# jspenmar/slowtv_monodepth

Measured on AMD Instinct MI355X. Metric: training images/sec (640×192, 3-frame) at 1/2/4/8 MI355X; warp+SSIM HBM GB/s, higher is better.
Workload: dtype f32

## Files before the change

### slowtv_monodepth_amd/csrc/smd_api.hip

```cpp
#include <limits.h>
#include <stdarg.h>
#include <stdio.h>
#include <stdlib.h>
#include <string.h>
#include <algorithm>

#include "smd_kernels.h"
#include "smd_smooth_dev.h"

namespace {

thread_local char g_err[512] = "";

int fail(int code, const char* fmt, ...) {
  va_list ap;
  va_start(ap, fmt);
  vsnprintf(g_err, sizeof(g_err), fmt, ap);
  va_end(ap);
  return code;
}

int check_launch(hipError_t e, const char* what) {
  if (e != hipSuccess) return fail(SMD_E_LAUNCH, "%s: %s", what, hipGetErrorString(e));
  return SMD_OK;
// ... 494 lines not shown
  if (int rc = fill_scales(sc, disp, g_disp, hs, ws, scale_keys, S)) return rc;
  for (int s = 0; s < S; ++s) if (!disp[s] || !g_disp[s]) return fail(SMD_E_INVALID, "null pointer for scale %d", s);
  int direct = -1;
  if (const char* why = loss_path_unsupported(sc, n, h, w, flags, &direct)) return fail(SMD_E_UNSUPPORTED, "the fused loss path does not serve %s", why);
  const size_t need = smd_loss_path_workspace_bytes(hs, ws, S, b, n, h, w);
  if (!need || workspace_bytes < need) return fail(SMD_E_WORKSPACE, "workspace %zu < %zu bytes", workspace_bytes, need);
  const size_t base = align256(smd_image_recon_workspace_bytes(b, n, S, h, w));
  float* g_depth = (float*)((char*)workspace + base);
  float* k0_tmp = (float*)((char*)workspace + base + align256((size_t)S*b*h*w*sizeof(float)));
  float a_scale = 1.f;
  if (min_depth > 0.f || max_depth > 0.f) a_scale = 1.f/min_depth - (max_depth > 0.f ? 1.f/max_depth : 0.f);
  const bool guests = knob("loss_path_guests", 1) != 0;
  smd::PoseFinJob job;
  memset(&job, 0, sizeof(job));
  job.chain.aa = aa; job.chain.t = t; job.chain.invert = invert; job.chain.g_aa = g_aa; job.chain.g_t = g_t;
  job.chain.fs = fs; job.chain.cs = cs; job.chain.g_fs = g_fs; job.chain.g_cs = g_cs; job.chain.h = h; job.chain.w = w;
  job.sm.stats = stats; job.sm.edge_w = edge_weights; job.sm.g_loss = g_loss; job.sm.g_scale = w_smooth; job.sm.accumulate_scale = direct;
  job.sm.blocks_per_sample = guests ? smd::smooth_bwd_blocks_per_sample(sc) : 0;
  const int rflags = flags & (SMD_USE_MIN | SMD_USE_AUTOMASK | SMD_NEED_K_GRAD | SMD_BWD_SKIP_DEAD_ROWS | SMD_BWD_NO_LIVE);
  if (int rc = recon_bwd_impl(depth_up, supp_packed, T, K, K_inv, sel, g_loss, nullptr, a_scale, g_depth, g_T, g_K, g_Kinv, workspace, base,
                              b, n, S, h, w, rflags, stream, &job, direct >= 0 ? g_disp[direct] : nullptr, direct, w_recon)) return rc;
  if (!guests) {
    if (int rc = check_launch(smd::launch_smooth_bwd(sc, b, nullptr, h, w, SMD_USE_EDGES, stats, g_loss, edge_weights, (hipStream_t)stream, w_smooth, direct), "loss_path smoothness adjoint")) return rc;
  }
  return check_launch(smd::launch_disp_to_depth_bwd(sc, b, h, w, min_depth, max_depth, depth_up, g_depth, k0_tmp, true, (hipStream_t)stream, &job, direct, true), "loss_path K0 adjoint");
}

static int smooth_chunks(const int* hs, const int* ws, int S) {
  int mx = 1;
  for (int s = 0; s < S; ++s) {
    const int u = smd::smooth_units_of(hs[s], ws[s]), p = smd::ceil_div(hs[s]*ws[s], 256);
    mx = (u > p ? u : p) > mx ? (u > p ? u : p) : mx;
  }
  return mx;
}

size_t smd_disp_smooth_workspace_bytes(const int* hs, const int* ws, int S, int b) {
  if (!hs || !ws || S < 1 || S > SMD_MAX_SCALES || b < 1) return 0;
  return align256((size_t)S*b*smooth_chunks(hs, ws, S)*2*sizeof(float) + (size_t)S*b*sizeof(double));
}

size_t smd_disp_smooth_edge_weight_bytes(const int* hs, const int* ws, int S, int b) {
  smd::ScaleSet sc;
  if (b < 1 || fill_scales(sc, nullptr, nullptr, hs, ws, nullptr, S)) return 0;
  return smd::smooth_edge_bytes(sc, b);
}

int smd_gaussian_blur3x3(const float* x, float* out, int planes, int h, int w, int adjoint, void* stream) {
  if (!x || !out) return fail(SMD_E_INVALID, "null pointer");
  if (x == out) return fail(SMD_E_INVALID, "in-place blur is not supported");
  if (planes < 1) return fail(SMD_E_INVALID, "invalid sizes");
  if (h < 2 || w < 2) return fail(SMD_E_INVALID, "reflect padding by one needs at least 2 x 2 pixels (got %d x %d)", h, w);
  return check_launch(smd::launch_blur3(x, out, planes, h, w, adjoint != 0, (hipStream_t)stream), "gaussian_blur3x3");
}

int smd_disp_smooth_prep(const float* img, const int* hs, const int* ws, int S, int b, int h, int w, int flags, float* edge_weights, void* stream) {
  if (!img || !edge_weights) return fail(SMD_E_INVALID, "null pointer");
  if (b < 1 || h < 1 || w < 1 || b > 65535) return fail(SMD_E_INVALID, "invalid sizes");
  if (!(flags & SMD_USE_EDGES) || (flags & SMD_USE_LAPLACIAN)) return fail(SMD_E_INVALID, "smd_disp_smooth_prep serves SmoothReg(use_edges=True) without use_laplacian");
  smd::ScaleSet sc;
  if (int rc = fill_scales(sc, nullptr, nullptr, hs, ws, nullptr, S)) return rc;
  return check_launch(smd::launch_smooth_edges(sc, b, img, h, w, edge_weights, (hipStream_t)stream), "disp_smooth_prep");
}

int smd_disp_smooth_fwd(const float* const* disp, const int* hs, const int* ws, const int* scale_keys, int S, int b,
                        const float* img, int h, int w, int flags, float* loss, float* stats, float* disp_grad, float* image_grad,
                        float* edge_weights, void* workspace, size_t workspace_bytes, void* stream) {
  if (!disp || !img || !loss || !stats || !workspace) return fail(SMD_E_INVALID, "null pointer");
  if (b < 1 || h < 1 || w < 1 || b > 65535) return fail(SMD_E_INVALID, "invalid sizes");
  smd::ScaleSet sc;
  if (int rc = fill_scales(sc, disp, nullptr, hs, ws, scale_keys, S)) return rc;
  for (int s = 0; s < S; ++s) if (!disp[s]) return fail(SMD_E_INVALID, "null disparity pointer for scale %d", s);
  const size_t need = smd_disp_smooth_workspace_bytes(hs, ws, S, b);
  if (workspace_bytes < need) return fail(SMD_E_WORKSPACE, "workspace %zu < %zu bytes", workspace_bytes, need);
  if ((flags & SMD_USE_EDGES) && !edge_weights) return fail(SMD_E_INVALID, "SMD_USE_EDGES needs the edge_weights buffer (smd_disp_smooth_edge_weight_bytes)");
  if ((flags & SMD_EDGES_READY) && (!(flags & SMD_USE_EDGES) || (flags & SMD_USE_LAPLACIAN))) return fail(SMD_E_INVALID, "SMD_EDGES_READY goes with SMD_USE_EDGES (first-order form)");
  return check_launch(smd::launch_smooth_fwd(sc, b, img, h, w, flags, loss, stats, disp_grad, image_grad, (float*)workspace,
                                             edge_weights, (flags & SMD_EDGES_READY) != 0, (hipStream_t)stream), "disp_smooth_fwd");
}

int smd_disp_smooth_bwd(const float* const* disp, const int* hs, const int* ws, const int* scale_keys, int S, int b,
                        const float* img, int h, int w, int flags, const float* stats, const float* edge_weights, const float* g_loss,
                        float* const* g_disp, void* stream) {
  if (!disp || !img || !stats || !g_loss || !g_disp) return fail(SMD_E_INVALID, "null pointer");
  if (b < 1 || h < 1 || w < 1 || b > 65535) return fail(SMD_E_INVALID, "invalid sizes");
  smd::ScaleSet sc;
  if (int rc = fill_scales(sc, disp, g_disp, hs, ws, scale_keys, S)) return rc;
  for (int s = 0; s < S; ++s) if (!disp[s] || !g_disp[s]) return fail(SMD_E_INVALID, "null pointer for scale %d", s);
  if ((flags & SMD_USE_LAPLACIAN) && (flags & SMD_USE_EDGES) && !edge_weights) return fail(SMD_E_INVALID, "the second-order adjoint needs the edge weights the forward cached");
  return check_launch(smd::launch_smooth_bwd(sc, b, img, h, w, flags, stats, g_loss, edge_weights, (hipStream_t)stream), "disp_smooth_bwd");
}

size_t smd_view_synth_workspace_bytes(int B, int h, int w) {
  if (B < 1 || h < 2 || w < 2) return 0;
  return align256((size_t)B*smd::ceil_div(h*w, 256)*smd::kPoseSums*sizeof(float));
}

int smd_view_synth_fwd(const float* input, const float* depth, const float* T, const float* K, const float* K_inv,
                       float* warp, float* depth_warp, uint8_t* mask_valid, int B, int C, int h, int w, void* stream) {
  if (!input || !depth || !T || !K || !K_inv || !warp) return fail(SMD_E_INVALID, "null pointer");
  if (B < 1 || B > 65535 || C < 1 || h < 2 || w < 2) return fail(SMD_E_INVALID, "invalid sizes B=%d C=%d h=%d w=%d", B, C, h, w);
  return check_launch(smd::launch_view_synth_fwd(input, depth, T, K, K_inv, warp, depth_warp, mask_valid, B, C, h, w, (hipStream_t)stream), "view_synth_fwd");
}

int smd_view_synth_bwd(const float* input, const float* depth, const float* T, const float* K, const float* K_inv,
                       const float* g_warp, const float* g_depth_warp, float* g_input, float* g_depth, float* g_T, float* g_K, float* g_Kinv,
                       void* workspace, size_t workspace_bytes, int B, int C, int h, int w, void* stream) {
  if (!input || !depth || !T || !K || !K_inv || !g_warp || !g_depth || !g_T || !workspace) return fail(SMD_E_INVALID, "null pointer");
  if (B < 1 || B > 65535 || C < 1 || h < 2 || w < 2) return fail(SMD_E_INVALID, "invalid sizes B=%d C=%d h=%d w=%d", B, C, h, w);
  if (workspace_bytes < smd_view_synth_workspace_bytes(B, h, w)) return fail(SMD_E_WORKSPACE, "workspace too small");
  return check_launch(smd::launch_view_synth_bwd(input, depth, T, K, K_inv, g_warp, g_depth_warp, g_input, g_depth, g_T, g_K, g_Kinv,
                                                 (float*)workspace, B, C, h, w, (hipStream_t)stream), "view_synth_bwd");
}

size_t smd_photo_error_workspace_bytes(int N, int C, int h, int w) {
  if (N < 1 || C < 1 || h < 2 || w < 2) return 0;
  return align256((size_t)N*3*C*h*w*sizeof(float));
}

int smd_photo_error_fwd(const float* pred, const float* target, float* err, int N, int C, int h, int w, int flags, float weight_ssim, void* stream) {
  if (!pred || !target || !err) return fail(SMD_E_INVALID, "null pointer");
  if (N < 1 || N > 65535 || C < 1 || h < 2 || w < 2) return fail(SMD_E_INVALID, "invalid sizes N=%d C=%d h=%d w=%d", N, C, h, w);
  if (!(weight_ssim >= 0.f && weight_ssim <= 1.f)) return fail(SMD_E_INVALID, "Invalid SSIM weight. (%g vs. [0, 1])", weight_ssim);
  return check_launch(smd::launch_photo_error_fwd(pred, target, err, N, C, h, w, flags, weight_ssim, (hipStream_t)stream), "photo_error_fwd");
}

int smd_photo_error_bwd(const float* pred, const float* target, const float* g_err, float* g_pred, void* workspace, size_t workspace_bytes,
                        int N, int C, int h, int w, int flags, float weight_ssim, void* stream) {
  if (!pred || !target || !g_err || !g_pred || !workspace) return fail(SMD_E_INVALID, "null pointer");
  if (N < 1 || N > 65535 || C < 1 || h < 2 || w < 2) return fail(SMD_E_INVALID, "invalid sizes N=%d C=%d h=%d w=%d", N, C, h, w);
  if (workspace_bytes < smd_photo_error_workspace_bytes(N, C, h, w)) return fail(SMD_E_WORKSPACE, "workspace too small");
  if (!(weight_ssim >= 0.f && weight_ssim <= 1.f)) return fail(SMD_E_INVALID, "Invalid SSIM weight. (%g vs. [0, 1])", weight_ssim);
  return check_launch(smd::launch_photo_error_bwd(pred, target, g_err, g_pred, (float*)workspace, N, C, h, w, flags, weight_ssim, (hipStream_t)stream), "photo_error_bwd");
}

size_t smd_regression_workspace_bytes(size_t N) {
  if (N < 1) return 0;
  return align256((size_t)smd::regr_blocks(N)*3*sizeof(float));
}

int smd_regression_fwd(const float* pred, const float* target, const uint8_t* mask, size_t N, int flags, float* loss, float* err, float* stats,
                       void* workspace, size_t workspace_bytes, void* stream) {
  if (!pred || !target || !loss || !stats || !workspace) return fail(SMD_E_INVALID, "null pointer");
  if (N < 1 || N > ((size_t)1 << 40)) return fail(SMD_E_INVALID, "invalid size N=%zu", N);
  if (workspace_bytes < smd_regression_workspace_bytes(N)) return fail(SMD_E_WORKSPACE, "workspace too small");
  return check_launch(smd::launch_regression_fwd(pred, target, mask, N, flags, loss, err, stats, (float*)workspace, (hipStream_t)stream), "regression_fwd");
}

int smd_regression_bwd(const float* pred, const float* target, const uint8_t* mask, size_t N, int flags, float* stats, const float* g_loss,
                       float* g_pred, float* g_target, void* workspace, size_t workspace_bytes, void* stream) {
  if (!pred || !target || !stats || !g_loss || !workspace || (!g_pred && !g_target)) return fail(SMD_E_INVALID, "null pointer");
  if (N < 1 || N > ((size_t)1 << 40)) return fail(SMD_E_INVALID, "invalid size N=%zu", N);
  if (workspace_bytes < smd_regression_workspace_bytes(N)) return fail(SMD_E_WORKSPACE, "workspace too small");
  return check_launch(smd::launch_regression_bwd(pred, target, mask, N, flags, stats, g_loss, g_pred, g_target, (float*)workspace, (hipStream_t)stream),
                      "regression_bwd");
}

size_t smd_recon_reduce_workspace_bytes(int B, int h, int w) {
  if (B < 1 || h < 1 || w < 1) return 0;
  return align256((size_t)smd::ceil_div(B*h*w, 256)*sizeof(float));
}

int smd_recon_reduce_fwd(const float* err_warp, const float* err_static, const float* mask, const float* noise, uint64_t seed, float* err, uint8_t* sel,
                         float* loss, void* workspace, size_t workspace_bytes, int n, int B, int h, int w, int flags, void* stream) {
  if (!err_warp || !err || !sel || !loss || !workspace) return fail(SMD_E_INVALID, "null pointer");
  if ((flags & (SMD_MASK_EXPLAINABILITY | SMD_MASK_UNCERTAINTY)) && !mask) return fail(SMD_E_INVALID, "Must provide a 'mask' when masking...");
  if ((flags & SMD_USE_AUTOMASK) && !err_static) return fail(SMD_E_INVALID, "Must provide the original 'source' images when automasking...");
  if (n < 1 || n >= SMD_SEL_MASKED || B < 1 || h < 1 || w < 1) return fail(SMD_E_INVALID, "invalid sizes");
  if (workspace_bytes < smd_recon_reduce_workspace_bytes(B, h, w)) return fail(SMD_E_WORKSPACE, "workspace too small");
  return check_launch(smd::launch_recon_reduce_fwd(err_warp, err_static, mask, noise, seed, err, sel, loss, (float*)workspace, n, B, h, w, flags,
                                                   (hipStream_t)stream), "recon_reduce_fwd");
}

int smd_recon_reduce_bwd(const uint8_t* sel, const float* g_loss, float* g_err_warp, const float* err_warp, const float* err_static,
                         const float* mask, float* g_mask, int n, int B, int h, int w, int flags, void* stream) {
  if (!sel || !g_loss || !g_err_warp) return fail(SMD_E_INVALID, "null pointer");
  if (n < 1 || B < 1 || h < 1 || w < 1) return fail(SMD_E_INVALID, "invalid sizes");
  if (mask && (!g_mask || !err_warp || ((flags & SMD_USE_AUTOMASK) && !err_static))) return fail(SMD_E_INVALID, "a masked reduction needs err_warp, err_static (with automask) and g_mask");
  return check_launch(smd::launch_recon_reduce_bwd(sel, g_loss, g_err_warp, err_warp, err_static, mask, g_mask, n, B, h, w, flags, (hipStream_t)stream), "recon_reduce_bwd");
}

static bool dec_sizes_ok(long long planes, int h, int w) {
  return planes >= 1 && h >= 2 && w >= 2 && (long long)(h + 2)*(w + 2) < (1ll << 30) && planes*(((long long)(h + 2)*(w + 2) + 255)/256) < (1ll << 31);
}
size_t smd_decoder_glue_workspace_bytes(int B, int C, int h, int w) {
  if (B < 1 || C < 1 || h < 1 || w < 1) return 0;
  return align256(smd::decoder_bias_partials(B, C, h, w)*sizeof(float));
}
int smd_elu_pad_fwd(const void* x, const float* bias, void* out, int B, int C, int h, int w, int apply_elu, int dtypes, void* stream) {
  if (!x || !out) return fail(SMD_E_INVALID, "null pointer");
  if (B < 1 || C < 1 || !dec_sizes_ok((long long)B*C, h, w)) return fail(SMD_E_INVALID, "invalid sizes B=%d C=%d h=%d w=%d", B, C, h, w);
  return check_launch(smd::launch_elu_pad_fwd(x, bias, out, B, C, h, w, apply_elu, dtypes, (hipStream_t)stream), "elu_pad_fwd");
}
int smd_elu_pad_bwd(const void* x, const float* bias, const void* g_out, void* g_x, float* g_bias, void* workspace, size_t workspace_bytes,
                    int B, int C, int h, int w, int apply_elu, int dtypes, void* stream) {
  if (!x || !g_out || !g_x || (g_bias && !workspace)) return fail(SMD_E_INVALID, "null pointer");
  if (B < 1 || C < 1 || !dec_sizes_ok((long long)B*C, h, w)) return fail(SMD_E_INVALID, "invalid sizes B=%d C=%d h=%d w=%d", B, C, h, w);
  if (g_bias && workspace_bytes < smd_decoder_glue_workspace_bytes(B, C, h, w)) return fail(SMD_E_WORKSPACE, "workspace too small");
  return check_launch(smd::launch_elu_pad_bwd(x, bias, g_out, g_x, g_bias, (float*)workspace, B, C, h, w, apply_elu, dtypes, (hipStream_t)stream), "elu_pad_bwd");
}
static bool head_sizes_ok(int B, int C, int h, int w) {
  return B >= 1 && C >= 1 && C < 65535 && dec_sizes_ok((long long)B*C, h, w) && (long long)B*((h + 47)/48) < 65536 && h < 65536 && (long long)B*C*(h + 2)*(w + 2) < (1ll << 40);
}
size_t smd_conv3x3_head_workspace_bytes(int B, int C, int h, int w) {
  if (!head_sizes_ok(B, C, h, w)) return 0;
  return align256(smd::conv_head_partials(B, C, h, w)*sizeof(float));
}
int smd_conv3x3_head_fwd(const void* xp, const float* weight, const float* bias, float* y, int B, int C, int h, int w, int act, void* stream) {
  if (!xp || !weight || !y) return fail(SMD_E_INVALID, "null pointer");
  if (!head_sizes_ok(B, C, h, w) || (act & ~(1 | SMD_HEAD_X_BF16))) return fail(SMD_E_INVALID, "invalid sizes B=%d C=%d h=%d w=%d act=%d", B, C, h, w, act);
  return check_launch(smd::launch_conv_head_fwd(xp, (act & SMD_HEAD_X_BF16) != 0, weight, bias, y, B, C, h, w, act & 1, (hipStream_t)stream), "conv3x3_head_fwd");
}
int smd_conv3x3_head_bwd(const void* xp, const float* weight, const float* y, const float* g_y, void* g_xp, float* g_weight, float* g_bias,
                         void* workspace, size_t workspace_bytes, int B, int C, int h, int w, int act, void* stream) {
  if (!weight || !y || !g_y || (!g_xp && !g_weight) || (g_weight && (!xp || !workspace)) || (g_bias && !g_weight)) return fail(SMD_E_INVALID, "null pointer");
  if (!head_sizes_ok(B, C, h, w) || (act & ~(1 | SMD_HEAD_X_BF16))) return fail(SMD_E_INVALID, "invalid sizes B=%d C=%d h=%d w=%d act=%d", B, C, h, w, act);
  if (g_weight && workspace_bytes < smd_conv3x3_head_workspace_bytes(B, C, h, w)) return fail(SMD_E_WORKSPACE, "workspace too small");
  return check_launch(smd::launch_conv_head_bwd(xp, (act & SMD_HEAD_X_BF16) != 0, weight, y, g_y, g_xp, g_weight, g_bias, (float*)workspace, B, C, h, w, act & 1, (hipStream_t)stream), "conv3x3_head_bwd");
}
static bool thin_sizes_ok(int B, int C, int h, int w) { return (C == 16 || C == 32) && head_sizes_ok(B, C, h, w) && dec_sizes_ok((long long)B*16, h, w) && B < 65536 && h + 2 < 4*65536; }
size_t smd_conv3x3_thin_workspace_bytes(int B, int C, int h, int w) {
  if (!thin_sizes_ok(B, C, h, w)) return 0;
  return align256(smd::conv_thin_partials(B, C, h, w)*sizeof(float));
}
int smd_conv3x3_thin_bwd(const float* xp, const float* weight, const float* g_y, float* g_xp, float* g_weight, void* workspace, size_t workspace_bytes,
                         int B, int C, int h, int w, void* stream) {
  if (!g_y || (!g_xp && !g_weight) || (g_xp && !weight) || (g_weight && (!xp || !workspace))) return fail(SMD_E_INVALID, "null pointer");
  if (C != 16 && C != 32 && C >= 1) return fail(SMD_E_UNSUPPORTED, "the thin convolution serves 16 or 32 input channels, not %d", C);
  if (!thin_sizes_ok(B, C, h, w)) return fail(SMD_E_INVALID, "invalid sizes B=%d C=%d h=%d w=%d", B, C, h, w);
  if (g_weight && workspace_bytes < smd_conv3x3_thin_workspace_bytes(B, C, h, w)) return fail(SMD_E_WORKSPACE, "workspace too small");
  hipStream_t st = (hipStream_t)stream;
  if (g_xp) { if (int rc = check_launch(smd::launch_conv_thin_bwd_data(g_y, weight, g_xp, B, C, h, w, st), "conv3x3_thin_bwd (data)")) return rc; }
  if (g_weight) { if (int rc = check_launch(smd::launch_conv_thin_bwd_wgt(xp, g_y, g_weight, (float*)workspace, B, C, h, w, st), "conv3x3_thin_bwd (weights)")) return rc; }
  return SMD_OK;
}
int smd_conv3x3_thin_fwd(const float* xp, const float* weight, float* y, int B, int C, int h, int w, void* stream) {
  if (!xp || !weight || !y) return fail(SMD_E_INVALID, "null pointer");
  if (C != 16 && C != 32 && C >= 1) return fail(SMD_E_UNSUPPORTED, "the thin convolution serves 16 or 32 input channels, not %d", C);
  if (!thin_sizes_ok(B, C, h, w)) return fail(SMD_E_INVALID, "invalid sizes B=%d C=%d h=%d w=%d", B, C, h, w);
  return check_launch(smd::launch_conv_thin_fwd(xp, weight, y, B, C, h, w, (hipStream_t)stream), "conv3x3_thin_fwd");
}
static bool mfma_sizes_ok(int B, int C, int CO, int h, int w) {
  return B >= 1 && C >= 1 && CO >= 1 && C <= 4096 && CO <= 4096 && h >= 1 && w >= 1 && h < 32768 && w < 32768 && (long long)(h + 2)*(w + 2) < (1ll << 30) &&
         (long long)B*((C + 31)/32)*((CO + 31)/32) < 65536 && (long long)C*(h + 2)*(w + 2) < (1ll << 29) && (long long)CO*h*w < (1ll << 29);
}
static bool mfma_fwd_served(int C, int CO) { return (C % 16 == 0 && CO % 32 == 0) || (CO == 16 && (C == 16 || C == 32)); }
static bool mfma_wgt_served(int C, int CO) { return CO % 32 == 0 || (CO == 16 && (C == 16 || C == 32)); }
static bool mfma_data_served(int C, int CO) { return (CO % 16 == 0 && C % 32 == 0) || (C == 16 && CO == 16); }
size_t smd_conv3x3_mfma_packed_bytes(int C, int CO, int pieces) {
  if (C < 1 || CO < 1 || pieces < 1 || pieces > 3) return 0;
  return align256(smd::conv_mfma_packed_elems(C, CO, pieces)*2);
}
size_t smd_conv3x3_mfma_workspace_bytes(int B, int C, int CO, int h, int w) {
  if (!mfma_sizes_ok(B, C, CO, h, w)) return 0;
  smd::set_conv_two_tiles(knob("conv_two_tiles", 0));
  size_t n = 64;
  if (mfma_fwd_served(C, CO)) n = std::max(n, smd::conv_mfma_fwd_split_elems(B, C, CO, h, w));
  if (mfma_data_served(C, CO)) n = std::max(n, smd::conv_mfma_bwd_split_elems(B, C, CO, h, w));
  if (mfma_wgt_served(C, CO)) n = std::max(n, smd::conv_mfma_wgrad_partials(B, C, CO, h, w));
  return align256(n*sizeof(float));
}
int smd_conv3x3_mfma_pack(const float* weight, void* wp_fwd, void* wp_bwd, int C, int CO, int pieces, void* stream) {
  if (!weight || (!wp_fwd && !wp_bwd)) return fail(SMD_E_INVALID, "null pointer");
  if (pieces < 1 || pieces > 3) return fail(SMD_E_UNSUPPORTED, "pieces must be 1 (bfloat16 tensors), 2 or 3 (float tensors), not %d", pieces);
  if (C < 1 || CO < 1 || C > 4096 || CO > 4096) return fail(SMD_E_INVALID, "invalid sizes C=%d CO=%d", C, CO);
  if (wp_fwd && !mfma_fwd_served(C, CO)) return fail(SMD_E_UNSUPPORTED, "the forward form serves C %% 16 == 0 with CO %% 32 == 0, or CO == 16 with C == 16 | 32, not C=%d CO=%d", C, CO);
  if (wp_bwd && !mfma_data_served(C, CO)) return fail(SMD_E_UNSUPPORTED, "the data-gradient form serves CO %% 16 == 0 with C %% 32 == 0, or C == CO == 16, not C=%d CO=%d", C, CO);
  return check_launch(smd::launch_conv_mfma_pack(weight, wp_fwd, wp_bwd, C, CO, pieces, (hipStream_t)stream), "conv3x3_mfma_pack");
}
int smd_conv3x3_mfma_fwd(const void* xp, const void* wp_fwd, void* y, void* workspace, size_t workspace_bytes,
                         int B, int C, int CO, int h, int w, int pieces, void* stream) {
  if (!xp || !wp_fwd || !y || !workspace) return fail(SMD_E_INVALID, "null pointer");
  if (pieces < 1 || pieces > 3) return fail(SMD_E_UNSUPPORTED, "pieces must be 1 (bfloat16 tensors), 2 or 3 (float tensors), not %d", pieces);
  if (!mfma_sizes_ok(B, C, CO, h, w)) return fail(SMD_E_INVALID, "invalid sizes B=%d C=%d CO=%d h=%d w=%d", B, C, CO, h, w);
  if (!mfma_fwd_served(C, CO)) return fail(SMD_E_UNSUPPORTED, "the forward serves C %% 16 == 0 with CO %% 32 == 0, or CO == 16 with C == 16 | 32, not C=%d CO=%d", C, CO);
  if (workspace_bytes < smd_conv3x3_mfma_workspace_bytes(B, C, CO, h, w)) return fail(SMD_E_WORKSPACE, "workspace too small");
  smd::set_conv_two_tiles(knob("conv_two_tiles", 0));
  return check_launch(smd::launch_conv_mfma_fwd(xp, wp_fwd, y, (float*)workspace, B, C, CO, h, w, pieces, (hipStream_t)stream), "conv3x3_mfma_fwd");
}
int smd_conv3x3_mfma_bwd_data(const void* g_y, const void* wp_bwd, void* g_xp, void* workspace, size_t workspace_bytes,
                              int B, int C, int CO, int h, int w, int pieces, void* stream) {
  if (!g_y || !wp_bwd || !g_xp || !workspace) return fail(SMD_E_INVALID, "null pointer");
  if (pieces < 1 || pieces > 3) return fail(SMD_E_UNSUPPORTED, "pieces must be 1 (bfloat16 tensors), 2 or 3 (float tensors), not %d", pieces);
  if (!mfma_sizes_ok(B, C, CO, h, w)) return fail(SMD_E_INVALID, "invalid sizes B=%d C=%d CO=%d h=%d w=%d", B, C, CO, h, w);
  if (!mfma_data_served(C, CO)) return fail(SMD_E_UNSUPPORTED, "the data gradient serves CO %% 16 == 0 with C %% 32 == 0, or C == CO == 16, not C=%d CO=%d", C, CO);
  if (workspace_bytes < smd_conv3x3_mfma_workspace_bytes(B, C, CO, h, w)) return fail(SMD_E_WORKSPACE, "workspace too small");
  smd::set_conv_two_tiles(knob("conv_two_tiles", 0));
  return check_launch(smd::launch_conv_mfma_bwd_data(g_y, wp_bwd, g_xp, (float*)workspace, B, C, CO, h, w, pieces, (hipStream_t)stream), "conv3x3_mfma_bwd_data");
}
int smd_conv3x3_mfma_bwd_weight(const void* xp, const void* g_y, float* g_weight, void* workspace, size_t workspace_bytes,
                                int B, int C, int CO, int h, int w, int pieces, void* stream) {
  if (!xp || !g_y || !g_weight || !workspace) return fail(SMD_E_INVALID, "null pointer");
  if (pieces < 1 || pieces > 3) return fail(SMD_E_UNSUPPORTED, "pieces must be 1 (bfloat16 tensors), 2 or 3 (float tensors), not %d", pieces);
  if (!mfma_sizes_ok(B, C, CO, h, w)) return fail(SMD_E_INVALID, "invalid sizes B=%d C=%d CO=%d h=%d w=%d", B, C, CO, h, w);
  if (!mfma_wgt_served(C, CO)) return fail(SMD_E_UNSUPPORTED, "the weight gradient serves CO %% 32 == 0, or CO == 16 with C == 16 | 32, not C=%d CO=%d", C, CO);
  if (workspace_bytes < smd_conv3x3_mfma_workspace_bytes(B, C, CO, h, w)) return fail(SMD_E_WORKSPACE, "workspace too small");
  return check_launch(smd::launch_conv_mfma_bwd_wgt(xp, g_y, g_weight, (float*)workspace, B, C, CO, h, w, pieces, (hipStream_t)stream), "conv3x3_mfma_bwd_weight");
}
static bool mfmaz_pieces_ok(int pieces) { return pieces == 2 || pieces == 3; }
size_t smd_conv3x3z_mfma_workspace_bytes(int B, int C, int CO, int h, int w) {
  if (!mfma_sizes_ok(B, C, CO, h, w)) return 0;
  smd::set_conv_two_tiles(knob("conv_two_tiles", 0));
  size_t n = std::max((size_t)64, smd::conv_mfma_z_split_elems(B, C, CO, h, w));
  if (CO % 32 == 0) n = std::max(n, smd::conv_mfma_wgrad_partials(B, C, CO, h, w));
  return align256(n*sizeof(float));
}
int smd_conv3x3z_mfma_fwd(const float* x, const void* wp_fwd, float* y, void* workspace, size_t workspace_bytes,
                          int B, int C, int CO, int h, int w, int pieces, void* stream) {
  if (!x || !wp_fwd || !y || !workspace) return fail(SMD_E_INVALID, "null pointer");
  if (!mfmaz_pieces_ok(pieces)) return fail(SMD_E_UNSUPPORTED, "the zero-padded forms take float tensors: pieces 2 or 3, not %d", pieces);
  if (!mfma_sizes_ok(B, C, CO, h, w)) return fail(SMD_E_INVALID, "invalid sizes B=%d C=%d CO=%d h=%d w=%d", B, C, CO, h, w);
  if (C % 16 || CO % 32) return fail(SMD_E_UNSUPPORTED, "the zero-padded forward serves C %% 16 == 0 with CO %% 32 == 0, not C=%d CO=%d", C, CO);
  if (workspace_bytes < smd_conv3x3z_mfma_workspace_bytes(B, C, CO, h, w)) return fail(SMD_E_WORKSPACE, "workspace too small");
  return check_launch(smd::launch_conv_mfma_z_fwd(x, wp_fwd, y, (float*)workspace, B, C, CO, h, w, pieces, (hipStream_t)stream), "conv3x3z_mfma_fwd");
}
int smd_conv3x3z_mfma_bwd_data(const float* g_y, const void* wp_bwd, float* g_x, void* workspace, size_t workspace_bytes,
                               int B, int C, int CO, int h, int w, int pieces, void* stream) {
  if (!g_y || !wp_bwd || !g_x || !workspace) return fail(SMD_E_INVALID, "null pointer");
  if (!mfmaz_pieces_ok(pieces)) return fail(SMD_E_UNSUPPORTED, "the zero-padded forms take float tensors: pieces 2 or 3, not %d", pieces);
  if (!mfma_sizes_ok(B, C, CO, h, w)) return fail(SMD_E_INVALID, "invalid sizes B=%d C=%d CO=%d h=%d w=%d", B, C, CO, h, w);
  if (CO % 16 || C % 32) return fail(SMD_E_UNSUPPORTED, "the zero-padded data gradient serves CO %% 16 == 0 with C %% 32 == 0, not C=%d CO=%d", C, CO);
  if (workspace_bytes < smd_conv3x3z_mfma_workspace_bytes(B, C, CO, h, w)) return fail(SMD_E_WORKSPACE, "workspace too small");
  return check_launch(smd::launch_conv_mfma_z_bwd_data(g_y, wp_bwd, g_x, (float*)workspace, B, C, CO, h, w, pieces, (hipStream_t)stream), "conv3x3z_mfma_bwd_data");
}
int smd_conv3x3z_mfma_bwd_weight(const float* x, const float* g_y, float* g_weight, void* workspace, size_t workspace_bytes,
                                 int B, int C, int CO, int h, int w, int pieces, void* stream) {
  if (!x || !g_y || !g_weight || !workspace) return fail(SMD_E_INVALID, "null pointer");
  if (!mfmaz_pieces_ok(pieces)) return fail(SMD_E_UNSUPPORTED, "the zero-padded forms take float tensors: pieces 2 or 3, not %d", pieces);
  if (!mfma_sizes_ok(B, C, CO, h, w)) return fail(SMD_E_INVALID, "invalid sizes B=%d C=%d CO=%d h=%d w=%d", B, C, CO, h, w);
  if (CO % 32) return fail(SMD_E_UNSUPPORTED, "the zero-padded weight gradient serves CO %% 32 == 0, not C=%d CO=%d", C, CO);
  if (workspace_bytes < smd_conv3x3z_mfma_workspace_bytes(B, C, CO, h, w)) return fail(SMD_E_WORKSPACE, "workspace too small");
  return check_launch(smd::launch_conv_mfma_z_bwd_wgt(x, g_y, g_weight, (float*)workspace, B, C, CO, h, w, pieces, (hipStream_t)stream), "conv3x3z_mfma_bwd_weight");
}
int smd_elu_up_cat_pad_fwd(const void* a, const float* bias, const void* skip, void* out, int B, int Ca, int Cs, int h, int w, int dtypes, void* stream) {
  if (!a || !out || (Cs > 0 && !skip)) return fail(SMD_E_INVALID, "null pointer");
  if (B < 1 || Ca < 1 || Cs < 0 || h < 1 || w < 1 || !dec_sizes_ok((long long)B*(Ca + Cs), 2*h, 2*w))
    return fail(SMD_E_INVALID, "invalid sizes B=%d Ca=%d Cs=%d h=%d w=%d", B, Ca, Cs, h, w);
  return check_launch(smd::launch_elu_up_cat_pad_fwd(a, bias, skip, out, B, Ca, Cs, h, w, dtypes, (hipStream_t)stream), "elu_up_cat_pad_fwd");
}
int smd_elu_up_cat_pad_bwd(const void* a, const float* bias, const void* g_out, void* g_a, void* g_skip, float* g_bias,
                           void* workspace, size_t workspace_bytes, int B, int Ca, int Cs, int h, int w, int dtypes, void* stream) {
  if (!a || !g_out || (!g_a && !g_skip) || (g_bias && (!workspace || !g_a))) return fail(SMD_E_INVALID, "null pointer");
  if (B < 1 || Ca < 1 || Cs < 0 || h < 1 || w < 1 || !dec_sizes_ok((long long)B*(Ca + Cs), 2*h, 2*w))
    return fail(SMD_E_INVALID, "invalid sizes B=%d Ca=%d Cs=%d h=%d w=%d", B, Ca, Cs, h, w);
  if (g_bias && workspace_bytes < smd_decoder_glue_workspace_bytes(B, Ca, h, w)) return fail(SMD_E_WORKSPACE, "workspace too small");
  return check_launch(smd::launch_elu_up_cat_pad_bwd(a, bias, g_out, g_a, g_skip, g_bias, (float*)workspace, B, Ca, Cs, h, w, dtypes, (hipStream_t)stream),
                      "elu_up_cat_pad_bwd");
}

size_t smd_bn_workspace_bytes(int N, int C, int HW) {
  if (N < 1 || C < 1 || HW < 1) return 0;
  return align256(((size_t)C*smd::bn_chunks(N, HW)*2 + (size_t)C*3)*sizeof(float));
}
int smd_bn_fwd(const float* x, const float* residual, const float* gamma, const float* beta, float* running_mean, float* running_var,
               float momentum, float eps, int relu, float* y, float* save_mean, float* save_invstd, void* workspace, size_t workspace_bytes,
               int N, int C, int HW, void* stream) {
  if (!x || !gamma || !beta || !y || !save_mean || !save_invstd || !workspace) return fail(SMD_E_INVALID, "null pointer");
  if (N < 1 || C < 1 || C > 65535 || HW < 1 || (long long)N*HW < 2) return fail(SMD_E_INVALID, "invalid sizes N=%d C=%d HW=%d", N, C, HW);
  if (workspace_bytes < smd_bn_workspace_bytes(N, C, HW)) return fail(SMD_E_WORKSPACE, "workspace too small");
  return check_launch(smd::launch_bn_fwd(x, residual, gamma, beta, running_mean, running_var, momentum, eps, relu, y, save_mean, save_invstd,
                                         (float*)workspace, N, C, HW, (hipStream_t)stream), "bn_fwd");
}
int smd_bn_bwd(const float* x, const float* y, const float* g_y, const float* gamma, const float* save_mean, const float* save_invstd, int relu,
               float* g_x, float* g_residual, float* g_gamma, float* g_beta, void* workspace, size_t workspace_bytes, int N, int C, int HW,
               void* stream) {
  if (!x || !g_y || !gamma || !save_mean || !save_invstd || !g_x || !g_gamma || !g_beta || !workspace || (relu && !y))
    return fail(SMD_E_INVALID, "null pointer");
  if (N < 1 || C < 1 || C > 65535 || HW < 1) return fail(SMD_E_INVALID, "invalid sizes N=%d C=%d HW=%d", N, C, HW);
  if (workspace_bytes < smd_bn_workspace_bytes(N, C, HW)) return fail(SMD_E_WORKSPACE, "workspace too small");
  return check_launch(smd::launch_bn_bwd(x, y, g_y, gamma, save_mean, save_invstd, relu, g_x, g_residual, g_gamma, g_beta, (float*)workspace,
                                         N, C, HW, (hipStream_t)stream), "bn_bwd");
}

int smd_maxpool3x3s2_fwd(const float* x, float* y, uint8_t* idx, int N, int C, int H, int W, void* stream) {
  if (!x || !y || !idx) return fail(SMD_E_INVALID, "null pointer");
  if (N < 1 || C < 1 || H < 1 || W < 1 || (long long)N*C*(((long long)H*W + 1023)/1024) >= (1ll << 31)) return fail(SMD_E_INVALID, "invalid sizes");
  return check_launch(smd::launch_maxpool_fwd(x, y, idx, (size_t)N*C, H, W, (hipStream_t)stream), "maxpool_fwd");
}
int smd_maxpool3x3s2_bwd(const float* g_y, const uint8_t* idx, float* g_x, int N, int C, int H, int W, void* stream) {
  if (!g_y || !idx || !g_x) return fail(SMD_E_INVALID, "null pointer");
  if (N < 1 || C < 1 || H < 1 || W < 1 || (long long)N*C*(((long long)H*W + 1023)/1024) >= (1ll << 31)) return fail(SMD_E_INVALID, "invalid sizes");
  return check_launch(smd::launch_maxpool_bwd(g_y, idx, g_x, (size_t)N*C, H, W, (hipStream_t)stream), "maxpool_bwd");
}

static bool dw_sizes_ok(int N, int C, int H, int W) {
  return N >= 1 && C >= 1 && H >= 1 && W >= 1 && (long long)N*C*smd::dwconv_tiles(H, W) < (1ll << 31) && (long long)H*W < (1ll << 30);
}
size_t smd_dwconv7x7_workspace_bytes(int C, int H, int W) {
  if (C < 1 || H < 1 || W < 1) return 0;
  return align256((size_t)C*smd::dwconv_tiles(H, W)*50*sizeof(float));
}
int smd_dwconv7x7_fwd(const float* x, const float* weight, const float* bias, float* y, int N, int C, int H, int W, int flip, void* stream) {
  if (!x || !weight || !y) return fail(SMD_E_INVALID, "null pointer");
  if (!dw_sizes_ok(N, C, H, W)) return fail(SMD_E_INVALID, "invalid sizes N=%d C=%d H=%d W=%d", N, C, H, W);
  return check_launch(smd::launch_dwconv7(x, weight, bias, y, N, C, H, W, flip, (hipStream_t)stream), "dwconv7x7_fwd");
}
int smd_dwconv7x7_wrw(const float* x, const float* g_y, float* g_weight, float* g_bias, void* workspace, size_t workspace_bytes,
                      int N, int C, int H, int W, void* stream) {
  if (!x || !g_y || !g_weight || !workspace) return fail(SMD_E_INVALID, "null pointer");
  if (!dw_sizes_ok(N, C, H, W)) return fail(SMD_E_INVALID, "invalid sizes N=%d C=%d H=%d W=%d", N, C, H, W);
  if (workspace_bytes < smd_dwconv7x7_workspace_bytes(C, H, W)) return fail(SMD_E_WORKSPACE, "workspace too small");
  return check_launch(smd::launch_dwconv7_wrw(x, g_y, g_weight, g_bias, (float*)workspace, N, C, H, W, (hipStream_t)stream), "dwconv7x7_wrw");
}

size_t smd_layernorm_cf_workspace_bytes(int N, int C, int HW) {
  if (N < 1 || C < 1 || HW < 1) return 0;
  return align256((size_t)smd::ln_cf_chunks((size_t)N*HW)*C*2*sizeof(float));
}
int smd_layernorm_cf_fwd(const float* x, const float* gamma, const float* beta, void* y, int y_is_bf16, float* mean, float* rstd, int N, int C, int HW,
                         float eps, void* stream) {
  if (!x || !gamma || !beta || !y || !mean || !rstd) return fail(SMD_E_INVALID, "null pointer");
  if (N < 1 || C < 1 || HW < 1 || (long long)N*HW >= (1ll << 38)) return fail(SMD_E_INVALID, "invalid sizes N=%d C=%d HW=%d", N, C, HW);
  return check_launch(smd::launch_ln_cf_fwd(x, gamma, beta, y, y_is_bf16, mean, rstd, N, C, HW, eps, (hipStream_t)stream), "layernorm_cf_fwd");
}
int smd_layernorm_cf_bwd(const float* x, const void* g_y, int g_y_is_bf16, const float* gamma, const float* mean, const float* rstd, float* g_x, float* g_gamma,
                         float* g_beta, void* workspace, size_t workspace_bytes, int N, int C, int HW, void* stream) {
  if (!x || !g_y || !gamma || !mean || !rstd || !g_x || !g_gamma || !g_beta || !workspace) return fail(SMD_E_INVALID, "null pointer");
  if (N < 1 || C < 1 || C > 32767 || HW < 1) return fail(SMD_E_INVALID, "invalid sizes N=%d C=%d HW=%d", N, C, HW);
  if (workspace_bytes < smd_layernorm_cf_workspace_bytes(N, C, HW)) return fail(SMD_E_WORKSPACE, "workspace too small");
  return check_launch(smd::launch_ln_cf_bwd(x, g_y, g_y_is_bf16, gamma, mean, rstd, g_x, g_gamma, g_beta, (float*)workspace, N, C, HW, (hipStream_t)stream),
                      "layernorm_cf_bwd");
}

int smd_pose_fwd(const float* aa, const float* t, const uint8_t* invert, int N, float* T, void* stream) {
  if (!aa || !t || !T) return fail(SMD_E_INVALID, "null pointer");
  if (N < 1) return fail(SMD_E_INVALID, "invalid size N=%d", N);
  return check_launch(smd::launch_pose_fwd(aa, t, invert, N, T, (hipStream_t)stream), "pose_fwd");
}
int smd_pose_bwd(const float* aa, const float* t, const uint8_t* invert, int N, const float* g_T, float* g_aa, float* g_t, void* stream) {
  if (!aa || !t || !g_T || !g_aa || !g_t) return fail(SMD_E_INVALID, "null pointer");
  if (N < 1) return fail(SMD_E_INVALID, "invalid size N=%d", N);
  return check_launch(smd::launch_pose_bwd(aa, t, invert, N, g_T, g_aa, g_t, (hipStream_t)stream), "pose_bwd");
}
int smd_intrinsics_fwd(const float* fs, const float* cs, const float* K_in, int b, int h, int w, float* K, float* K_inv, void* stream) {
  if (!K_inv || (fs && (!cs || !K)) || (!fs && !K_in)) return fail(SMD_E_INVALID, "null pointer");
  if (b < 1 || h < 1 || w < 1) return fail(SMD_E_INVALID, "invalid sizes");
  return check_launch(smd::launch_intrinsics_fwd(fs, cs, K_in, b, h, w, K, K_inv, (hipStream_t)stream), "intrinsics_fwd");
}
int smd_intrinsics_bwd(const float* fs, const float* cs, int b, int h, int w, const float* g_K, const float* g_Kinv,
                       float* g_fs, float* g_cs, void* stream) {
  if (!fs || !cs || !g_K || !g_Kinv || !g_fs || !g_cs) return fail(SMD_E_INVALID, "null pointer");
  if (b < 1 || h < 1 || w < 1) return fail(SMD_E_INVALID, "invalid sizes");
  return check_launch(smd::launch_intrinsics_bwd(fs, cs, b, h, w, g_K, g_Kinv, g_fs, g_cs, (hipStream_t)stream), "intrinsics_bwd");
}

int smd_crop_resize(const float* const* src, float* const* dst, const int* planes, int nseg, int H, int W, int crop_h, int crop_w,
                    int out_h, int out_w, const float* K_in, float* K_out, int nK, void* stream) {
  if (!src || !dst || !planes) return fail(SMD_E_INVALID, "null pointer");
  if (nseg < 1 || nseg > smd::SMD_MAX_AR_SEGMENTS) return fail(SMD_E_INVALID, "nseg=%d outside [1, %d]", nseg, smd::SMD_MAX_AR_SEGMENTS);
  if (H < 2 || W < 2 || crop_h < 1 || crop_w < 1 || crop_h > H || crop_w > W || out_h < 1 || out_w < 1)
    return fail(SMD_E_INVALID, "invalid sizes: input %dx%d, crop %dx%d, output %dx%d", H, W, crop_h, crop_w, out_h, out_w);
  if ((K_in != nullptr) != (K_out != nullptr) || (K_in && nK < 1)) return fail(SMD_E_INVALID, "K_in / K_out / nK must be given together");
  smd::CropResizeArgs a;
  memset(&a, 0, sizeof(a));
  long long total = 0;
  for (int k = 0; k < nseg; ++k) {
    if (!src[k] || !dst[k] || planes[k] < 1) return fail(SMD_E_INVALID, "segment %d: null pointer or no planes", k);
    a.src[k] = src[k]; a.dst[k] = dst[k]; a.planes[k] = planes[k]; a.first_plane[k] = (int)total;
    total += planes[k];
  }
  if (total + 1 > 65535) return fail(SMD_E_INVALID, "too many image planes for one launch (%lld)", total);
  a.nseg = nseg; a.H = H; a.W = W; a.ch = crop_h; a.cw = crop_w; a.oh = out_h; a.ow = out_w;
  a.y0 = (int)((double)H/2.0 - (double)crop_h/2.0); a.x0 = (int)((double)W/2.0 - (double)crop_w/2.0);
  a.resample = (crop_h != H || crop_w != W) ? 1 : 0;
  a.K_in = K_in; a.K_out = K_out; a.nK = nK;
  return check_launch(smd::launch_crop_resize(a, (hipStream_t)stream), "crop_resize");
}

int smd_profile_enable(int which, int capacity) {
  if (which < 0 || which > 4 || capacity < 0) return fail(SMD_E_INVALID, "bad profile slot");
  ProfSlot& p = g_prof[which];
  for (int i = 0; i < 2*p.cap; ++i) (void)hipEventDestroy(p.ev[i]);
  delete[] p.ev;
  p = ProfSlot();
  if (capacity == 0) return SMD_OK;
  p.ev = new hipEvent_t[2*capacity];
  for (int i = 0; i < 2*capacity; ++i)
    if (hipEventCreate(&p.ev[i]) != hipSuccess) return fail(SMD_E_LAUNCH, "hipEventCreate failed");
  p.cap = capacity;
  return SMD_OK;
}

int smd_profile_collect(int which, float* ms_out, int max_out, int* n_out) {
  if (which < 0 || which > 4 || !ms_out || !n_out) return fail(SMD_E_INVALID, "bad profile arguments");
  ProfSlot& p = g_prof[which];
  int n = 0;
  for (int i = 0; i < p.used && n < max_out; ++i) {
    if (hipEventSynchronize(p.ev[2*i + 1]) != hipSuccess) return fail(SMD_E_LAUNCH, "hipEventSynchronize failed");
    float ms = 0.f;
    if (hipEventElapsedTime(&ms, p.ev[2*i], p.ev[2*i + 1]) != hipSuccess) return fail(SMD_E_LAUNCH, "hipEventElapsedTime failed");
    ms_out[n++] = ms;
  }
  p.used = 0;
  *n_out = n;
  return SMD_OK;
}

int smd_debug_stream_copy(const void* src, void* dst, size_t nbytes, int mode, void* stream) {
  if (!src || !dst) return fail(SMD_E_INVALID, "null pointer");
  if (nbytes < 16 || (nbytes & 15) || ((uintptr_t)src & 15) || ((uintptr_t)dst & 15)) return fail(SMD_E_INVALID, "size and pointers must be multiples of 16");
  return check_launch(smd::launch_stream_copy(src, dst, nbytes, mode, (hipStream_t)stream), "stream_copy");
}

int smd_debug_lane_shift(float* out_left, float* out_right, void* stream) {
  if (!out_left || !out_right) return fail(SMD_E_INVALID, "null pointer");
  return check_launch(smd::launch_debug_lane_shift(out_left, out_right, (hipStream_t)stream), "debug_lane_shift");
}

}
```

### slowtv_monodepth_amd/csrc/smd_conv_mfma.hip

```cpp
#include "smd_common.h"
#include "smd_kernels.h"
#include <algorithm>
#include <type_traits>

namespace smd {

typedef __bf16 bf16x8 __attribute__((ext_vector_type(8)));
typedef __bf16 bf16x2v __attribute__((ext_vector_type(2)));
typedef float f32x2v __attribute__((ext_vector_type(2)));
typedef float f32x16 __attribute__((ext_vector_type(16)));

__host__ __device__ constexpr int n_products(int P) { return P == 3 ? 6 : P == 2 ? 3 : 1; }
__host__ __device__ constexpr int prod_a(int P, int t) { return P == 3 ? (t == 0 ? 2 : t == 1 ? 1 : t == 2 ? 0 : t == 3 ? 1 : 0) : P == 2 ? (t == 0 ? 1 : 0) : 0; }
__host__ __device__ constexpr int prod_b(int P, int t) { return P == 3 ? (t == 0 ? 0 : t == 1 ? 1 : t == 2 ? 2 : t == 3 ? 0 : t == 4 ? 1 : 0) : P == 2 ? (t == 1 ? 1 : 0) : 0; }

__device__ __forceinline__ unsigned pack_bf16_rne(float a, float b) { const f32x2v v = {a, b}; return __builtin_bit_cast(unsigned, __builtin_convertvector(v, bf16x2v)); }
__device__ __forceinline__ float bf16_lo(unsigned u) { return __builtin_bit_cast(float, u << 16); }
__device__ __forceinline__ float bf16_hi(unsigned u) { return __builtin_bit_cast(float, u & 0xffff0000u); }
template <int P> __device__ __forceinline__ void split_pair(float a, float b, unsigned (&p)[P]) {
  p[0] = pack_bf16_rne(a, b);
  if constexpr (P > 1) { a -= bf16_lo(p[0]); b -= bf16_hi(p[0]); p[1] = pack_bf16_rne(a, b); }
  if constexpr (P > 2) { a -= bf16_lo(p[1]); b -= bf16_hi(p[1]); p[2] = pack_bf16_rne(a, b); }
}
__device__ __forceinline__ bf16x8 as_frag(const uint4& u) { return __builtin_bit_cast(bf16x8, u); }
template <int P> __device__ __forceinline__ void split_pair(unsigned short a, unsigned short b, unsigned (&p)[P]) {
  static_assert(P == 1, "bfloat16 operands have one piece");
  p[0] = (unsigned)a | ((unsigned)b << 16);
}
template <typename T> struct RawOf { typedef float type; };
template <> struct RawOf<bf16> { typedef unsigned short type; };
template <typename T> __device__ __forceinline__ void store_out(T* p, size_t i, float v);
template <> __device__ __forceinline__ void store_out<float>(float* p, size_t i, float v) { p[i] = v; }
template <> __device__ __forceinline__ void store_out<bf16>(bf16* p, size_t i, float v) { p[i] = __float2bfloat16(v); }

template <int P>
__global__ __launch_bounds__(256) void k_conv_pack_w(const float* __restrict__ w, unsigned short* __restrict__ wp_fwd, unsigned short* __restrict__ wp_bwd, int CO, int C) {
  const int idx = blockIdx.x*256 + threadIdx.x;
  if (idx >= CO*C*9) return;
  const int tap = idx % 9, c = (idx/9) % C, co = idx/(9*C);
  unsigned pk[P];
  split_pair<P>(w[idx], 0.f, pk);
  if (wp_fwd) {
    const size_t base = ((((size_t)(co >> 5)*(C >> 4) + (c >> 4))*9 + tap)*P)*512 + (((c >> 3) & 1)*32 + (co & 31))*8 + (c & 7);
#pragma unroll
    for (int p = 0; p < P; ++p) wp_fwd[base + (size_t)p*512] = (unsigned short)(pk[p] & 0xffffu);
  }
  if (wp_bwd) {
    const size_t base = ((((size_t)(c >> 5)*(CO >> 4) + (co >> 4))*9 + (8 - tap))*P)*512 + (((co >> 3) & 1)*32 + (c & 31))*8 + (co & 7);
#pragma unroll
    for (int p = 0; p < P; ++p) wp_bwd[base + (size_t)p*512] = (unsigned short)(pk[p] & 0xffffu);
  }
}

#ifdef SMD_CONV_TRACE
__device__ unsigned long long g_conv_trace[8192][40];
#define SMD_CT(slot) do { if (wall == 0 && lid < 8192u && (slot) < 40) { const unsigned long long t_ = __builtin_amdgcn_s_memtime(); if (lane == 0) g_conv_trace[lid][(slot)] = t_; } } while (0)
#else
#define SMD_CT(slot) do { } while (0)
#endif
template <int TC> struct ConvTile {
  static constexpr int TRB = (TC == 64) ? 4 : 8;
  static constexpr int PW = TC + 2, PH = TRB + 2, NPIX = PW*PH;
};

template <int TC, int P, int OFF, typename TI, typename TO, int NM>
__global__ __launch_bounds__(256*NM, 2/NM) void k_conv_mfma(const TI* __restrict__ in_, const uint4* __restrict__ wp, TO* __restrict__ out,
                                                   int CK, int M, int hi, int wi, int ho, int wo, int KS, int kc_per_split, size_t split_stride,
                                                   unsigned gx, unsigned gy, unsigned gz) {
  using T = ConvTile<TC>;
  constexpr int NPIX = T::NPIX, PW = T::PW, off = OFF, NPROD = n_products(P);
  constexpr bool ZERO = OFF != 0;
  constexpr int kBuf = P*NPIX*2;
  __shared__ uint4 tile[2*kBuf];
  const int lane = threadIdx.x & 63, wall = __builtin_amdgcn_readfirstlane(threadIdx.x >> 6), wv = wall & 3, mt = wall >> 2, j = lane & 31, g = lane >> 5;
  constexpr int NT = 256*NM;
  const int MG = M/(32*NM);
  const unsigned nblk = (unsigned)(MG*KS)*gx*gy*gz, per = (nblk + 7)/8;
  const unsigned lid = (blockIdx.x & 7)*per + (blockIdx.x >> 3);
  if (lid >= nblk) return;
  const int mg = (int)(lid % MG)*NM + mt, ks = (lid/MG) % KS;
  const unsigned tl = lid/(MG*KS);
  const int x0 = (int)(tl % gx)*TC, y0 = (int)((tl/gx) % gy)*T::TRB, b = (int)(tl/(gx*gy));
  const int KC = CK >> 4, kc0 = ks*kc_per_split, kc1 = min(KC, kc0 + kc_per_split);
  const size_t plane = (size_t)hi*wi;
  typedef typename RawOf<TI>::type R;
  const R* src = reinterpret_cast<const R*>(in_) + (size_t)b*CK*plane;

  constexpr int ITEMS = 2*NPIX, TRIPS = (ITEMS + NT - 1)/NT;
  int pofs[TRIPS];
#pragma unroll
  for (int t = 0; t < TRIPS; ++t) {
    const int item = min(t*NT + (int)threadIdx.x, ITEMS - 1);
    const int half = item >= NPIX ? 1 : 0, pix = item - half*NPIX;
    const int r = pix/PW, cc = pix - r*PW;
    const int yy = y0 + r - off, xx = x0 + cc - off;
    if (ZERO) pofs[t] = (yy >= 0 && yy < hi && xx >= 0 && xx < wi) ? yy*wi + xx : -1;
    else pofs[t] = min(yy, hi - 1)*wi + min(xx, wi - 1);
  }
  R v[TRIPS][8];
  auto request = [&](int kc) {
#pragma unroll
    for (int t = 0; t < TRIPS; ++t) {
      const int item = min(t*NT + (int)threadIdx.x, ITEMS - 1);
      const int half = item >= NPIX ? 1 : 0;
      const R* p = src + (size_t)(kc*16 + half*8)*plane + (size_t)max(pofs[t], 0);
#pragma unroll
      for (int e = 0; e < 8; ++e) v[t][e] = (!ZERO || pofs[t] >= 0) ? p[(size_t)e*plane] : R(0);
    }
  };
  auto file_trip = [&](int buf, int t) {
    {
      const int item = t*NT + (int)threadIdx.x;
      if (item < ITEMS) {
        const int half = item >= NPIX ? 1 : 0, pix = item - half*NPIX;
        unsigned pk[4][P];
#pragma unroll
        for (int q = 0; q < 4; ++q) split_pair<P>(v[t][2*q], v[t][2*q + 1], pk[q]);
        const int slot = pix*2 + (half ^ ((pix >> 3) & 1));
#pragma unroll
        for (int p = 0; p < P; ++p) tile[buf*kBuf + p*NPIX*2 + slot] = uint4{pk[0][p], pk[1][p], pk[2][p], pk[3][p]};
      }
    }
  };
  auto file = [&](int buf) {
#pragma unroll
    for (int t = 0; t < TRIPS; ++t) file_trip(buf, t);
  };

  f32x16 acc[2], lo[2];
#pragma unroll
  for (int nt = 0; nt < 2; ++nt)
#pragma unroll
    for (int r = 0; r < 16; ++r) { acc[nt][r] = 0.f; lo[nt][r] = 0.f; }

  bf16x8 A[5][P], Bf[2][2][P];
  const uint4* wq = wp + ((size_t)mg*KC*9*P)*64 + lane;
  auto fetch_a = [&](bf16x8 (&dst)[P], int kc, int tap) {
#pragma unroll
    for (int p = 0; p < P; ++p) dst[p] = as_frag(wq[(size_t)((kc*9 + tap)*P + p)*64]);
  };
  auto read_b = [&](bf16x8 (&dst)[2][P], int buf, int tap) {
    const int ky = tap/3, kx = tap % 3;
#pragma unroll
    for (int nt = 0; nt < 2; ++nt) {
      const int r = (TC == 64) ? wv : 2*wv + nt, cb = (TC == 64) ? nt*32 : 0;
      const int pix = (r + ky)*PW + cb + j + kx;
      const int slot = pix*2 + (g ^ ((pix >> 3) & 1));
#pragma unroll
      for (int p = 0; p < P; ++p) dst[nt][p] = as_frag(tile[buf*kBuf + p*NPIX*2 + slot]);
    }
  };
  auto chunk = [&](int kc, int cur, auto more_tag) {
    constexpr bool MORE = decltype(more_tag)::value;
    [[maybe_unused]] const int cslot = 3 + 4*(kc - kc0);
    SMD_CT(cslot);
    read_b(Bf[0], cur, 0);
#pragma unroll
    for (int tap = 0; tap < 9; ++tap) {
      if (tap < 8) read_b(Bf[(tap + 1) & 1], cur, tap + 1);
#pragma unroll
      for (int t = 0; t < NPROD; ++t)
#pragma unroll
        for (int nt = 0; nt < 2; ++nt) {
          if (t == NPROD - 1) acc[nt] = __builtin_amdgcn_mfma_f32_32x32x16_bf16(A[tap % 5][0], Bf[tap & 1][nt][0], acc[nt], 0, 0, 0);
          else lo[nt] = __builtin_amdgcn_mfma_f32_32x32x16_bf16(A[tap % 5][prod_a(P, t)], Bf[tap & 1][nt][prod_b(P, t)], lo[nt], 0, 0, 0);
        }
      if (tap <= 4) fetch_a(A[(tap + 4) % 5], kc, tap + 4);
      else if (MORE && tap >= 6) fetch_a(A[tap - 6], kc + 1, tap - 6);
      if (MORE && tap == 8) fetch_a(A[3], kc + 1, 3);
      if (MORE && tap == 4) request(kc + 1);
      if (MORE && tap >= 6) {
#pragma unroll
        for (int t = 0; t < TRIPS; ++t) if (t*3/TRIPS == tap - 6) file_trip(cur ^ 1, t);
      }
      __builtin_amdgcn_sched_barrier(0);
    }
    SMD_CT(cslot + 1);
    SMD_CT(cslot + 2);
    __syncthreads();
    SMD_CT(cslot + 3);
  };

  SMD_CT(0);
  if (kc0 < kc1) {
    request(kc0);
#pragma unroll
    for (int tap = 0; tap < 4; ++tap) fetch_a(A[tap], kc0, tap);
    file(0);
  }
  SMD_CT(1);
  __syncthreads();
  SMD_CT(2);
  int kc = kc0;
  for (; kc + 1 < kc1; ++kc) chunk(kc, (kc - kc0) & 1, std::true_type{});
  if (kc < kc1) chunk(kc, (kc - kc0) & 1, std::false_type{});
  float* dstf = reinterpret_cast<float*>(out) + (size_t)ks*split_stride;
#pragma unroll
  for (int nt = 0; nt < 2; ++nt) {
    const int r = (TC == 64) ? wv : 2*wv + nt, cb = (TC == 64) ? nt*32 : 0;
    const int y = y0 + r, x = x0 + cb + j;
    if (y < ho && x < wo) {
#pragma unroll
      for (int rr = 0; rr < 16; ++rr) {
        const int m = mg*32 + (rr & 3) + 8*(rr >> 2) + 4*g;
        const size_t o = (((size_t)b*M + m)*ho + y)*wo + x;
        if (KS > 1) dstf[o] = acc[nt][rr] + lo[nt][rr];
        else store_out<TO>(out, o, acc[nt][rr] + lo[nt][rr]);
      }
    }
  }
  SMD_CT(39);
}

typedef float f32x4v __attribute__((ext_vector_type(4)));
typedef float f32x4u __attribute__((ext_vector_type(4), aligned(4)));

template <int P>
__global__ __launch_bounds__(256) void k_conv_pack_w16(const float* __restrict__ w, unsigned short* __restrict__ wp_fwd, unsigned short* __restrict__ wp_bwd, int C) {
  const int idx = blockIdx.x*256 + threadIdx.x;
  const int nslots = (C >> 4)*5*64*8;
  if (idx < nslots && wp_fwd) {
    const int e = idx & 7, lane = (idx >> 3) & 63, s = (idx >> 9) % 5, ch = idx/(512*5);
    const int j = lane & 15, q = lane >> 4, tap = 2*s + (q >> 1), k = 16*ch + 8*(q & 1) + e;
    unsigned pk[P];
    split_pair<P>(tap < 9 ? w[((size_t)j*C + k)*9 + tap] : 0.f, 0.f, pk);
#pragma unroll
    for (int p = 0; p < P; ++p) wp_fwd[(((size_t)(ch*5 + s)*P + p)*64 + lane)*8 + e] = (unsigned short)(pk[p] & 0xffffu);
  }
  if (idx < 5*64*8 && wp_bwd && C == 16) {
    const int e = idx & 7, lane = (idx >> 3) & 63, s = idx >> 9;
    const int j = lane & 15, q = lane >> 4, tap = 2*s + (q >> 1), k = 8*(q & 1) + e;
    unsigned pk[P];
    split_pair<P>(tap < 9 ? w[((size_t)k*C + j)*9 + (8 - tap)] : 0.f, 0.f, pk);
#pragma unroll
    for (int p = 0; p < P; ++p) wp_bwd[(((size_t)s*P + p)*64 + lane)*8 + e] = (unsigned short)(pk[p] & 0xffffu);
  }
}

template <int NCH, int P, bool BWD, typename TI, typename TO>
__global__ __launch_bounds__(256) void k_conv16_mfma(const TI* __restrict__ in_, const uint4* __restrict__ wp, TO* __restrict__ out,
                                                     int hi, int wi, int ho, int wo, unsigned gx, unsigned gy, unsigned gz) {
  using T = ConvTile<64>;
  constexpr int NPIX = T::NPIX, PW = T::PW, off = BWD ? 2 : 0, NPROD = n_products(P), CK = 16*NCH;
  __shared__ uint4 tile[P*NPIX*2];
  const int lane = threadIdx.x & 63, wv = __builtin_amdgcn_readfirstlane(threadIdx.x >> 6), i = lane & 15, q = lane >> 4;
  const unsigned nblk = gx*gy*gz, per = (nblk + 7)/8;
  const unsigned lid = (blockIdx.x & 7)*per + (blockIdx.x >> 3);
  if (lid >= nblk) return;
  const int x0 = (int)(lid % gx)*64, y0 = (int)((lid/gx) % gy)*4, b = (int)(lid/(gx*gy));
  const size_t plane = (size_t)hi*wi;
  typedef typename RawOf<TI>::type R;
  const R* src = reinterpret_cast<const R*>(in_) + (size_t)b*CK*plane;

  bf16x8 Wr[NCH][5][P];
#pragma unroll
  for (int ch = 0; ch < NCH; ++ch)
#pragma unroll
    for (int s = 0; s < 5; ++s)
#pragma unroll
      for (int p = 0; p < P; ++p) Wr[ch][s][p] = as_frag(wp[((ch*5 + s)*P + p)*64 + lane]);

  constexpr int ITEMS = 2*NPIX, TRIPS = (ITEMS + 255)/256;
  int pofs[TRIPS];
#pragma unroll
  for (int t = 0; t < TRIPS; ++t) {
    const int item = min(t*256 + (int)threadIdx.x, ITEMS - 1);
    const int half = item >= NPIX ? 1 : 0, pix = item - half*NPIX;
    const int r = pix/PW, cc = pix - r*PW;
    const int yy = y0 + r - off, xx = x0 + cc - off;
    if (BWD) pofs[t] = (yy >= 0 && yy < hi && xx >= 0 && xx < wi) ? yy*wi + xx : -1;
    else pofs[t] = min(yy, hi - 1)*wi + min(xx, wi - 1);
  }
  int dpix[5];
#pragma unroll
  for (int s = 0; s < 5; ++s) { const int tq = min(2*s + (q >> 1), 8); dpix[s] = (tq/3)*PW + tq % 3; }

  f32x4v acc[4], lo[4];
#pragma unroll
  for (int r = 0; r < 4; ++r) { acc[r] = f32x4v{0.f, 0.f, 0.f, 0.f}; lo[r] = f32x4v{0.f, 0.f, 0.f, 0.f}; }

#pragma unroll
  for (int ch = 0; ch < NCH; ++ch) {
    R v[TRIPS][8];
#pragma unroll
    for (int t = 0; t < TRIPS; ++t) {
      const int item = min(t*256 + (int)threadIdx.x, ITEMS - 1);
      const int half = item >= NPIX ? 1 : 0;
      const R* p = src + (size_t)(ch*16 + half*8)*plane + (size_t)max(pofs[t], 0);
#pragma unroll
      for (int e = 0; e < 8; ++e) v[t][e] = (!BWD || pofs[t] >= 0) ? p[(size_t)e*plane] : R(0);
    }
    if (ch > 0) __syncthreads();
#pragma unroll
    for (int t = 0; t < TRIPS; ++t) {
      const int item = t*256 + (int)threadIdx.x;
      if (item < ITEMS) {
        const int half = item >= NPIX ? 1 : 0, pix = item - half*NPIX;
        unsigned pk[4][P];
#pragma unroll
        for (int k = 0; k < 4; ++k) split_pair<P>(v[t][2*k], v[t][2*k + 1], pk[k]);
        const int slot = pix*2 + (half ^ ((pix >> 3) & 1));
#pragma unroll
        for (int p = 0; p < P; ++p) tile[p*NPIX*2 + slot] = uint4{pk[0][p], pk[1][p], pk[2][p], pk[3][p]};
      }
    }
    __syncthreads();
#pragma unroll
    for (int s = 0; s < 5; ++s) {
#pragma unroll
      for (int r = 0; r < 4; ++r) {
        const int pix = r*PW + 16*wv + i + dpix[s];
        const int slot = pix*2 + ((q & 1) ^ ((pix >> 3) & 1));
        bf16x8 A[P];
#pragma unroll
        for (int p = 0; p < P; ++p) A[p] = as_frag(tile[p*NPIX*2 + slot]);
#pragma unroll
        for (int t = 0; t < NPROD; ++t) {
          if (t == NPROD - 1) acc[r] = __builtin_amdgcn_mfma_f32_16x16x32_bf16(A[0], Wr[ch][s][0], acc[r], 0, 0, 0);
          else lo[r] = __builtin_amdgcn_mfma_f32_16x16x32_bf16(A[prod_a(P, t)], Wr[ch][s][prod_b(P, t)], lo[r], 0, 0, 0);
        }
      }
    }
  }
  const int x = x0 + 16*wv + 4*q;
#pragma unroll
  for (int r = 0; r < 4; ++r) {
    const int y = y0 + r;
    if (y >= ho || x >= wo) continue;
    TO* dstp = out + (((size_t)b*16 + i)*ho + y)*wo + x;
    const f32x4v o = acc[r] + lo[r];
    if constexpr (sizeof(TO) == 4) {
      if (x + 3 < wo) *reinterpret_cast<f32x4u*>(dstp) = o;
      else { dstp[0] = o[0]; if (x + 1 < wo) dstp[1] = o[1]; if (x + 2 < wo) dstp[2] = o[2]; }
    } else {
      const unsigned lo2 = pack_bf16_rne(o[0], o[1]), hi2 = pack_bf16_rne(o[2], o[3]);
      if (x + 3 < wo && (wo & 1) == 0) { reinterpret_cast<unsigned*>(dstp)[0] = lo2; reinterpret_cast<unsigned*>(dstp)[1] = hi2; }
      else {
        unsigned short* d16 = reinterpret_cast<unsigned short*>(dstp);
        d16[0] = (unsigned short)(lo2 & 0xffffu);
        if (x + 1 < wo) d16[1] = (unsigned short)(lo2 >> 16);
        if (x + 2 < wo) d16[2] = (unsigned short)(hi2 & 0xffffu);
        if (x + 3 < wo) d16[3] = (unsigned short)(hi2 >> 16);
      }
    }
  }
}

template <typename TO>
__global__ __launch_bounds__(256) void k_conv_split_sum(const float* __restrict__ part, TO* __restrict__ out, size_t n4, int KS) {
  const size_t i = (size_t)blockIdx.x*256 + threadIdx.x;
  if (i >= n4) return;
  const f4* p = reinterpret_cast<const f4*>(part);
  f4 s = p[i];
  for (int k = 1; k < KS; ++k) s += p[(size_t)k*n4 + i];
  if constexpr (sizeof(TO) == 4) reinterpret_cast<f4*>(out)[i] = s;
  else { unsigned* o = reinterpret_cast<unsigned*>(out) + 2*i; o[0] = pack_bf16_rne(s.x, s.y); o[1] = pack_bf16_rne(s.z, s.w); }
}

struct WgradTile {
  static constexpr int COB = 32, CB = 64;
  static constexpr int XROW = 20, XCH = 2*XROW + 4;
  static constexpr int GROW = 16, GCH = 4*GROW + 4;
};

template <int P, typename TI>
__global__ __launch_bounds__(256, 2) void k_conv_wgrad_mfma(const TI* __restrict__ xp, const TI* __restrict__ gy, float* __restrict__ partial,
                                                         int C, int CO, int h, int w, int rows_per_block) {
  using T = WgradTile;
  constexpr int COB = T::COB, CB = T::CB, XROW = T::XROW, XCH = T::XCH, GROW = T::GROW, GCH = T::GCH, NPROD = n_products(P);
  constexpr int kXs = P*CB*XCH, kGs = P*COB*GCH;
  constexpr int kRed = 2*144*64;
  __shared__ __attribute__((aligned(16))) unsigned lds[(kXs + kGs) > kRed ? (kXs + kGs) : kRed];
  unsigned* const xs = lds;
  unsigned* const gs = lds + kXs;
  const int lane = threadIdx.x & 63, wv = __builtin_amdgcn_readfirstlane(threadIdx.x >> 6), j = lane & 31, g = lane >> 5;
  const int ct = wv & 1, ks = wv >> 1;
  const int CGRP = (C + CB - 1)/CB, COGRP = CO/COB;
  const int cg = blockIdx.z % CGRP, cog = (blockIdx.z/CGRP) % COGRP, b = blockIdx.z/(CGRP*COGRP);
  const int x0 = blockIdx.x*32, ybeg = blockIdx.y*rows_per_block, nrows = min(rows_per_block, h - ybeg);
  const int W = w + 2, H = h + 2;
  typedef typename RawOf<TI>::type R;
  const R* xsrc = reinterpret_cast<const R*>(xp) + (size_t)b*C*H*W;
  const R* gsrc = reinterpret_cast<const R*>(gy) + ((size_t)b*CO + (size_t)cog*COB)*h*w;

  constexpr int XITEMS = CB*17, XTRIPS = (XITEMS + 255)/256;
  constexpr int GITEMS = COB*16, GTRIPS = GITEMS/256;
  static_assert(GITEMS % 256 == 0, "g_y items per thread");
  R xv[XTRIPS][2], gv[GTRIPS][2];
  auto load_x = [&](int yy) {
    yy = min(yy, H - 1);
#pragma unroll
    for (int t = 0; t < XTRIPS; ++t) {
      const int item = t*256 + (int)threadIdx.x;
      const int ch = min(item/17, CB - 1), pr = item % 17;
      const int c = min(cg*CB + ch, C - 1);
      const R* rowp = xsrc + ((size_t)c*H + yy)*W;
      xv[t][0] = rowp[min(x0 + 2*pr, W - 1)];
      xv[t][1] = rowp[min(x0 + 2*pr + 1, W - 1)];
    }
  };
  auto file_x = [&](int slot) {
#pragma unroll
    for (int t = 0; t < XTRIPS; ++t) {
      const int item = t*256 + (int)threadIdx.x;
      if (item < XITEMS) {
        const int ch = item/17, pr = item % 17;
        unsigned pk[P];
        split_pair<P>(xv[t][0], xv[t][1], pk);
#pragma unroll
        for (int p = 0; p < P; ++p) xs[(p*CB + ch)*XCH + slot*XROW + pr] = pk[p];
      }
    }
  };
  auto load_g = [&](int y) {
#pragma unroll
    for (int t = 0; t < GTRIPS; ++t) {
      const int item = t*256 + (int)threadIdx.x;
      const int co = item >> 4, pr = item & 15;
      const int xa = x0 + 2*pr;
      const bool yok = y < ybeg + nrows;
      const R* rowp = gsrc + ((size_t)co*h + (yok ? y : 0))*w;
      gv[t][0] = (yok && xa < w) ? rowp[xa] : R(0);
      gv[t][1] = (yok && xa + 1 < w) ? rowp[xa + 1] : R(0);
    }
  };
  auto file_g = [&](int slot) {
#pragma unroll
    for (int t = 0; t < GTRIPS; ++t) {
      const int item = t*256 + (int)threadIdx.x;
      const int co = item >> 4, pr = item & 15;
      unsigned pk[P];
      split_pair<P>(gv[t][0], gv[t][1], pk);
#pragma unroll
      for (int p = 0; p < P; ++p) gs[(p*COB + co)*GCH + slot*GROW + pr] = pk[p];
    }
  };

  f32x16 acc[9];
#pragma unroll
  for (int t = 0; t < 9; ++t)
#pragma unroll
    for (int r = 0; r < 16; ++r) acc[t][r] = 0.f;

  load_x(ybeg); file_x(0);
  load_g(ybeg); file_g(0);
  __syncthreads();
  for (int i = 0; i < nrows + 2; ++i) {
    load_x(ybeg + i + 1);
    load_g(ybeg + i + 1);
    bf16x8 Bx[3][P];
#pragma unroll
    for (int p = 0; p < P; ++p) {
      const uint4* q = reinterpret_cast<const uint4*>(&xs[(p*CB + ct*32 + j)*XCH + (i & 1)*XROW + ks*8 + g*4]);
      const uint4 d = q[0];
      const unsigned d4 = q[1].x;
      Bx[0][p] = as_frag(d);
      Bx[1][p] = as_frag(uint4{__builtin_amdgcn_alignbit(d.y, d.x, 16), __builtin_amdgcn_alignbit(d.z, d.y, 16), __builtin_amdgcn_alignbit(d.w, d.z, 16), __builtin_amdgcn_alignbit(d4, d.w, 16)});
      Bx[2][p] = as_frag(uint4{d.y, d.z, d.w, d4});
    }
#pragma unroll
    for (int ky = 0; ky < 3; ++ky) {
      if (i - ky < 0) continue;
      bf16x8 A[P];
#pragma unroll
      for (int p = 0; p < P; ++p) A[p] = as_frag(*reinterpret_cast<const uint4*>(&gs[(p*COB + j)*GCH + ((i - ky) & 3)*GROW + ks*8 + g*4]));
#pragma unroll
      for (int t = 0; t < NPROD; ++t)
#pragma unroll
        for (int kx = 0; kx < 3; ++kx) acc[ky*3 + kx] = __builtin_amdgcn_mfma_f32_32x32x16_bf16(A[prod_a(P, t)], Bx[kx][prod_b(P, t)], acc[ky*3 + kx], 0, 0, 0);
    }
    file_x((i + 1) & 1);
    file_g((i + 1) & 3);
    __syncthreads();
  }

  float* red = reinterpret_cast<float*>(lds);
  if (ks == 1) {
#pragma unroll
    for (int t = 0; t < 9; ++t)
#pragma unroll
      for (int r = 0; r < 16; ++r) red[(ct*144 + t*16 + r)*64 + lane] = acc[t][r];
  }
  __syncthreads();
  if (ks == 0) {
#pragma unroll
    for (int t = 0; t < 9; ++t)
#pragma unroll
      for (int r = 0; r < 16; ++r) acc[t][r] += red[(ct*144 + t*16 + r)*64 + lane];
    const size_t blk = ((size_t)b*gridDim.y + blockIdx.y)*gridDim.x + blockIdx.x;
    const int c = (cg*2 + ct)*32 + j;
    if (c < C) {
#pragma unroll
      for (int t = 0; t < 9; ++t)
#pragma unroll
        for (int r = 0; r < 16; ++r) {
          const int co = cog*32 + (r & 3) + 8*(r >> 2) + 4*g;
          partial[((blk*9 + t)*CO + co)*C + c] = acc[t][r];
        }
    }
  }
}

template <int P, bool ZP>
__global__ __launch_bounds__(256, 2) void k_conv_wgrad_dma(const float* __restrict__ xp, const float* __restrict__ gy, float* __restrict__ partial,
                                                        int C, int CO, int h, int w, int rows_per_block) {
  constexpr int COB = 32, CB = 64, NW = 4, NPROD = n_products(P), CS = 36, D = 4;
  constexpr int XDW = CB*CS, GDW = COB*CS, NPX = XDW/64, NPG = GDW/64, NX = (NPX + NW - 1)/NW, NG = (NPG + NW - 1)/NW, NDMA = NX + NG, SLOT = XDW + GDW + 64;
  static_assert(XDW % 64 == 0 && GDW % 64 == 0 && (D - 2)*NDMA < 64 && D == 4, "DMA pieces and waits");
  constexpr int kRing = D*SLOT, kTab = NW*NDMA*64, kRed = 2*144*64;
  __shared__ __attribute__((aligned(16))) unsigned lds[(kRing + kTab) > kRed ? (kRing + kTab) : kRed];
  const int lane = threadIdx.x & 63, wv = __builtin_amdgcn_readfirstlane(threadIdx.x >> 6), j = lane & 31, g = lane >> 5;
  const int ct = wv & 1, ks = wv >> 1;
  const int CGRP = (C + CB - 1)/CB, COGRP = CO/COB;
  const int cg = blockIdx.z % CGRP, cog = (blockIdx.z/CGRP) % COGRP, b = blockIdx.z/(CGRP*COGRP);
  const int x0 = blockIdx.x*32, ybeg = blockIdx.y*rows_per_block, nrows = min(rows_per_block, h - ybeg), nsteps = nrows + 2;
  const int W = w + 2, H = h + 2;
  const rsrc_t rs_x = ZP ? make_rsrc(xp + (size_t)b*C*h*w, (size_t)C*h*w*4) : make_rsrc(xp + (size_t)b*C*H*W, (size_t)C*H*W*4);
  const rsrc_t rs_g = make_rsrc(gy + ((size_t)b*CO + (size_t)cog*COB)*h*w, (size_t)COB*h*w*4);
  [[maybe_unused]] const rsrc_t rs_0 = make_rsrc(xp, 0);
  const unsigned lds0 = (unsigned)__builtin_amdgcn_readfirstlane((int)(unsigned)(unsigned long long)(__attribute__((address_space(3))) unsigned*)lds);
  auto dma = [&](const rsrc_t& rs, unsigned v, unsigned so, unsigned dst) {
    unsigned keep;
    asm volatile("s_mov_b32 %0, m0\n\ts_mov_b32 m0, %4\n\ts_nop 0\n\tbuffer_load_dword %1, %2, %3 offen lds\n\ts_mov_b32 m0, %0"
                 : "=&s"(keep) : "v"(v), "s"(rs), "s"(so), "s"(dst) : "memory");
  };
  unsigned* const tab = lds + kRing + wv*(NDMA*64) + lane;
#pragma unroll
  for (int n = 0; n < NX; ++n) {
    const int k = n*NW + wv, d = k*64 + lane, ch = d/CS, col = d - ch*CS, c = cg*CB + ch;
    if constexpr (ZP) tab[n*64] = (k < NPX && col < 34 && x0 + col >= 1 && x0 + col <= w && c < C) ? (unsigned)((c*h)*w + x0 + col - 1)*4u : 0x80000000u;
    else tab[n*64] = (k < NPX && col < 34 && x0 + col < W && c < C) ? (unsigned)((c*H)*W + x0 + col)*4u : 0x80000000u;
  }
#pragma unroll
  for (int n = 0; n < NG; ++n) {
    const int k = n*NW + wv, d = k*64 + lane, co = d/CS, col = d - co*CS;
    tab[(NX + n)*64] = (k < NPG && col < 32 && x0 + col < w) ? (unsigned)((co*h)*w + x0 + col)*4u : 0x80000000u;
  }
  auto issue = [&](int r) {
    const unsigned base = lds0 + (unsigned)((r % D)*SLOT*4);
    rsrc_t rx = rs_x;
    unsigned sx;
    if constexpr (ZP) {
      const int yx = ybeg + r - 1;
      const bool xin = yx >= 0 && yx < h;
      rx = xin ? rs_x : rs_0; sx = xin ? (unsigned)yx*(unsigned)w*4u : 0u;
    } else sx = (unsigned)min(ybeg + r, H - 1)*(unsigned)W*4u;
    const unsigned sg = (unsigned)min(ybeg + r, h - 1)*(unsigned)w*4u;
    unsigned v[NDMA];
#pragma unroll
    for (int n = 0; n < NDMA; ++n) v[n] = tab[n*64];
#pragma unroll
    for (int n = 0; n < NX; ++n) { const int k = n*NW + wv; dma(rx, v[n], sx, base + (unsigned)(k < NPX ? k*256 : (XDW + GDW)*4)); }
#pragma unroll
    for (int n = 0; n < NG; ++n) { const int k = n*NW + wv; dma(rs_g, v[NX + n], sg, base + (unsigned)(k < NPG ? XDW*4 + k*256 : (XDW + GDW)*4)); }
  };

  f32x16 acc[9];
#pragma unroll
  for (int t = 0; t < 9; ++t)
#pragma unroll
    for (int r = 0; r < 16; ++r) acc[t][r] = 0.f;
  bf16x8 A[3][P];
#pragma unroll
  for (int r = 0; r < 3; ++r)
#pragma unroll
    for (int p = 0; p < P; ++p) A[r][p] = as_frag(uint4{0u, 0u, 0u, 0u});

  auto step = [&](int i, bf16x8 (&a0)[P], const bf16x8 (&a1)[P], const bf16x8 (&a2)[P]) {
    const int after = min(D - 2, nsteps - 1 - i);
    if (after >= 2) asm volatile("s_waitcnt vmcnt(%0)" :: "n"(2*NDMA) : "memory");
    else if (after == 1) asm volatile("s_waitcnt vmcnt(%0)" :: "n"(NDMA) : "memory");
    else asm volatile("s_waitcnt vmcnt(0)" ::: "memory");
    __builtin_amdgcn_s_barrier();
    asm volatile("" ::: "memory");
    if (i + D - 1 < nsteps) issue(i + D - 1);
    const float* slot = reinterpret_cast<const float*>(lds) + (i % D)*SLOT;
    const float* xr = slot + (ct*32 + j)*CS + ks*16 + g*8;
    const float* gr = slot + XDW + j*CS + ks*16 + g*8;
    const float4 x0v = *reinterpret_cast<const float4*>(xr), x1v = *reinterpret_cast<const float4*>(xr + 4);
    const float2 x2v = *reinterpret_cast<const float2*>(xr + 8);
    const float4 g0v = *reinterpret_cast<const float4*>(gr), g1v = *reinterpret_cast<const float4*>(gr + 4);
    unsigned px[5][P], pg[4][P];
    split_pair<P>(x0v.x, x0v.y, px[0]); split_pair<P>(x0v.z, x0v.w, px[1]); split_pair<P>(x1v.x, x1v.y, px[2]); split_pair<P>(x1v.z, x1v.w, px[3]); split_pair<P>(x2v.x, x2v.y, px[4]);
    split_pair<P>(g0v.x, g0v.y, pg[0]); split_pair<P>(g0v.z, g0v.w, pg[1]); split_pair<P>(g1v.x, g1v.y, pg[2]); split_pair<P>(g1v.z, g1v.w, pg[3]);
    bf16x8 Bx[3][P];
#pragma unroll
    for (int p = 0; p < P; ++p) {
      Bx[0][p] = as_frag(uint4{px[0][p], px[1][p], px[2][p], px[3][p]});
      Bx[1][p] = as_frag(uint4{__builtin_amdgcn_alignbit(px[1][p], px[0][p], 16), __builtin_amdgcn_alignbit(px[2][p], px[1][p], 16),
                               __builtin_amdgcn_alignbit(px[3][p], px[2][p], 16), __builtin_amdgcn_alignbit(px[4][p], px[3][p], 16)});
      Bx[2][p] = as_frag(uint4{px[1][p], px[2][p], px[3][p], px[4][p]});
      a0[p] = as_frag(i < nrows ? uint4{pg[0][p], pg[1][p], pg[2][p], pg[3][p]} : uint4{0u, 0u, 0u, 0u});
    }
#pragma unroll
    for (int ky = 0; ky < 3; ++ky) {
      const bf16x8 (&a)[P] = ky == 0 ? a0 : ky == 1 ? a1 : a2;
#pragma unroll
      for (int t = 0; t < NPROD; ++t)
#pragma unroll
        for (int kx = 0; kx < 3; ++kx) acc[ky*3 + kx] = __builtin_amdgcn_mfma_f32_32x32x16_bf16(a[prod_a(P, t)], Bx[kx][prod_b(P, t)], acc[ky*3 + kx], 0, 0, 0);
    }
  };
#pragma unroll
  for (int r = 0; r < D - 1; ++r) issue(r);
  for (int i = 0; i < nsteps; i += 3) {
    step(i, A[0], A[2], A[1]);
    if (i + 1 < nsteps) step(i + 1, A[1], A[0], A[2]);
    if (i + 2 < nsteps) step(i + 2, A[2], A[1], A[0]);
  }
  __syncthreads();
  float* red = reinterpret_cast<float*>(lds);
  if (ks == 1) {
#pragma unroll
    for (int t = 0; t < 9; ++t)
#pragma unroll
      for (int r = 0; r < 16; ++r) red[(ct*144 + t*16 + r)*64 + lane] = acc[t][r];
  }
  __syncthreads();
  if (ks == 0) {
#pragma unroll
    for (int t = 0; t < 9; ++t)
#pragma unroll
      for (int r = 0; r < 16; ++r) acc[t][r] += red[(ct*144 + t*16 + r)*64 + lane];
    const size_t blk = ((size_t)b*gridDim.y + blockIdx.y)*gridDim.x + blockIdx.x;
    const int c = (cg*2 + ct)*32 + j;
    if (c < C) {
#pragma unroll
      for (int t = 0; t < 9; ++t)
#pragma unroll
        for (int r = 0; r < 16; ++r) {
          const int co = cog*32 + (r & 3) + 8*(r >> 2) + 4*g;
          partial[((blk*9 + t)*CO + co)*C + c] = acc[t][r];
        }
    }
  }
}

template <int NC, int P, typename TI>
__global__ __launch_bounds__(128*NC) void k_conv16_wgrad_mfma(const TI* __restrict__ xp, const TI* __restrict__ gy, float* __restrict__ partial, int h, int w, int rows_per_block) {
  constexpr int C = 16*NC, NT = 128*NC, NPROD = n_products(P);
  constexpr int XROW = 36, XCH = 2*XROW + 4;
  constexpr int GROW = 32, GCH = 4*GROW + 4;
  constexpr int kXs = P*C*XCH, kGs = P*16*GCH, kRed = NC*36*64;
  __shared__ __attribute__((aligned(16))) unsigned lds[(kXs + kGs) > kRed ? (kXs + kGs) : kRed];
  unsigned* const xs = lds;
  unsigned* const gs = lds + kXs;
  const int lane = threadIdx.x & 63, wv = __builtin_amdgcn_readfirstlane(threadIdx.x >> 6), j = lane & 15, q = lane >> 4;
  const int nc = wv >> 1, ks = wv & 1;
  const int x0 = blockIdx.x*64, ybeg = blockIdx.y*rows_per_block, nrows = min(rows_per_block, h - ybeg), b = blockIdx.z;
  const int W = w + 2, H = h + 2;
  typedef typename RawOf<TI>::type R;
  const R* xsrc = reinterpret_cast<const R*>(xp) + (size_t)b*C*H*W;
  const R* gsrc = reinterpret_cast<const R*>(gy) + (size_t)b*16*h*w;

  constexpr int XITEMS = C*33, XTRIPS = (XITEMS + NT - 1)/NT;
  constexpr int GITEMS = 16*32, GTRIPS = GITEMS/NT;
  static_assert(GITEMS % NT == 0, "g_y items per thread");
  R xv[XTRIPS][2], gv[GTRIPS][2];
  auto load_x = [&](int yy) {
    yy = min(yy, H - 1);
#pragma unroll
    for (int t = 0; t < XTRIPS; ++t) {
      const int item = min(t*NT + (int)threadIdx.x, XITEMS - 1);
      const int c = item/33, pr = item - c*33;
      const R* rowp = xsrc + ((size_t)c*H + yy)*W;
      xv[t][0] = rowp[min(x0 + 2*pr, W - 1)];
      xv[t][1] = rowp[min(x0 + 2*pr + 1, W - 1)];
    }
  };
  auto file_x = [&](int slot) {
#pragma unroll
    for (int t = 0; t < XTRIPS; ++t) {
      const int item = t*NT + (int)threadIdx.x;
      if (item < XITEMS) {
        const int c = item/33, pr = item - c*33;
        unsigned pk[P];
        split_pair<P>(xv[t][0], xv[t][1], pk);
#pragma unroll
        for (int p = 0; p < P; ++p) xs[(p*C + c)*XCH + slot*XROW + pr] = pk[p];
      }
    }
  };
  auto load_g = [&](int y) {
#pragma unroll
    for (int t = 0; t < GTRIPS; ++t) {
      const int item = t*NT + (int)threadIdx.x;
      const int co = item >> 5, pr = item & 31;
      const int xa = x0 + 2*pr;
      const bool yok = y < ybeg + nrows;
      const R* rowp = gsrc + ((size_t)co*h + (yok ? y : 0))*w;
      gv[t][0] = (yok && xa < w) ? rowp[xa] : R(0);
      gv[t][1] = (yok && xa + 1 < w) ? rowp[xa + 1] : R(0);
    }
  };
  auto file_g = [&](int slot) {
#pragma unroll
    for (int t = 0; t < GTRIPS; ++t) {
      const int item = t*NT + (int)threadIdx.x;
      const int co = item >> 5, pr = item & 31;
      unsigned pk[P];
      split_pair<P>(gv[t][0], gv[t][1], pk);
#pragma unroll
      for (int p = 0; p < P; ++p) gs[(p*16 + co)*GCH + slot*GROW + pr] = pk[p];
    }
  };

  f32x4v acc[9];
#pragma unroll
  for (int t = 0; t < 9; ++t) acc[t] = f32x4v{0.f, 0.f, 0.f, 0.f};

  load_x(ybeg); file_x(0);
  load_g(ybeg); file_g(0);
  __syncthreads();
  for (int i = 0; i < nrows + 2; ++i) {
    load_x(ybeg + i + 1);
    load_g(ybeg + i + 1);
    bf16x8 Bx[3][P];
#pragma unroll
    for (int p = 0; p < P; ++p) {
      const uint4* qp = reinterpret_cast<const uint4*>(&xs[(p*C + nc*16 + j)*XCH + (i & 1)*XROW + ks*16 + q*4]);
      const uint4 d = qp[0];
      const unsigned d4 = qp[1].x;
      Bx[0][p] = as_frag(d);
      Bx[1][p] = as_frag(uint4{__builtin_amdgcn_alignbit(d.y, d.x, 16), __builtin_amdgcn_alignbit(d.z, d.y, 16), __builtin_amdgcn_alignbit(d.w, d.z, 16), __builtin_amdgcn_alignbit(d4, d.w, 16)});
      Bx[2][p] = as_frag(uint4{d.y, d.z, d.w, d4});
    }
#pragma unroll
    for (int ky = 0; ky < 3; ++ky) {
      if (i - ky < 0) continue;
      bf16x8 A[P];
#pragma unroll
      for (int p = 0; p < P; ++p) A[p] = as_frag(*reinterpret_cast<const uint4*>(&gs[(p*16 + j)*GCH + ((i - ky) & 3)*GROW + ks*16 + q*4]));
#pragma unroll
      for (int t = 0; t < NPROD; ++t)
#pragma unroll
        for (int kx = 0; kx < 3; ++kx) acc[ky*3 + kx] = __builtin_amdgcn_mfma_f32_16x16x32_bf16(A[prod_a(P, t)], Bx[kx][prod_b(P, t)], acc[ky*3 + kx], 0, 0, 0);
    }
    file_x((i + 1) & 1);
    file_g((i + 1) & 3);
    __syncthreads();
  }
  float* red = reinterpret_cast<float*>(lds);
  if (ks == 1) {
#pragma unroll
    for (int t = 0; t < 9; ++t)
#pragma unroll
      for (int v = 0; v < 4; ++v) red[(nc*36 + t*4 + v)*64 + lane] = acc[t][v];
  }
  __syncthreads();
  if (ks == 0) {
    const size_t blk = ((size_t)b*gridDim.y + blockIdx.y)*gridDim.x + blockIdx.x;
#pragma unroll
    for (int t = 0; t < 9; ++t)
#pragma unroll
      for (int v = 0; v < 4; ++v) {
        const int co = 4*q + v, c = nc*16 + j;
        partial[((blk*9 + t)*16 + co)*C + c] = acc[t][v] + red[(nc*36 + t*4 + v)*64 + lane];
      }
  }
}

template <int NC, int P>
__global__ __launch_bounds__(128*NC) void k_conv16_wgrad_dma(const float* __restrict__ xp, const float* __restrict__ gy, float* __restrict__ partial, int h, int w, int rows_per_block) {
  constexpr int C = 16*NC, NW = 2*NC, NPROD = n_products(P), CS = 68, D = 4;
  constexpr int XDW = C*CS, GDW = 16*CS, NPX = XDW/64, NPG = GDW/64, NX = (NPX + NW - 1)/NW, NG = (NPG + NW - 1)/NW, NDMA = NX + NG, SLOT = XDW + GDW + 64;
  static_assert(XDW % 64 == 0 && GDW % 64 == 0, "whole DMA pieces per region");
  static_assert((D - 2)*NDMA < 64, "the waits below are immediates of six bits");
  constexpr int kRed = NC*36*64;
  __shared__ __attribute__((aligned(16))) unsigned lds[(D*SLOT) > kRed ? (D*SLOT) : kRed];
  const int lane = threadIdx.x & 63, wv = __builtin_amdgcn_readfirstlane(threadIdx.x >> 6), j = lane & 15, q = lane >> 4;
  const int nc = wv >> 1, ks = wv & 1;
  const int x0 = blockIdx.x*64, ybeg = blockIdx.y*rows_per_block, nrows = min(rows_per_block, h - ybeg), b = blockIdx.z;
  const int W = w + 2, H = h + 2, nsteps = nrows + 2;
  const rsrc_t rs_x = make_rsrc(xp + (size_t)b*C*H*W, (size_t)C*H*W*4), rs_g = make_rsrc(gy + (size_t)b*16*h*w, (size_t)16*h*w*4);
  const unsigned lds0 = (unsigned)__builtin_amdgcn_readfirstlane((int)(unsigned)(unsigned long long)(__attribute__((address_space(3))) unsigned*)lds);

  unsigned vx[NX], vg[NG];
#pragma unroll
  for (int n = 0; n < NX; ++n) {
    const int k = n*NW + wv, d = k*64 + lane, c = d/CS, col = d - c*CS;
    vx[n] = (k < NPX && col < 66 && x0 + col < W) ? (unsigned)((c*H)*W + x0 + col)*4u : 0x80000000u;
  }
#pragma unroll
  for (int n = 0; n < NG; ++n) {
    const int k = n*NW + wv, d = k*64 + lane, co = d/CS, col = d - co*CS;
    vg[n] = (k < NPG && col < 64 && x0 + col < w) ? (unsigned)((co*h)*w + x0 + col)*4u : 0x80000000u;
  }
  auto dma = [&](const rsrc_t& rs, unsigned v, unsigned so, unsigned dst) {
    unsigned keep;
    asm volatile("s_mov_b32 %0, m0\n\ts_mov_b32 m0, %4\n\ts_nop 0\n\tbuffer_load_dword %1, %2, %3 offen lds\n\ts_mov_b32 m0, %0"
                 : "=&s"(keep) : "v"(v), "s"(rs), "s"(so), "s"(dst) : "memory");
  };
  auto issue = [&](int r) {
    const unsigned base = lds0 + (unsigned)((r % D)*SLOT*4);
    const unsigned sx = (unsigned)min(ybeg + r, H - 1)*(unsigned)W*4u, sg = (unsigned)min(ybeg + r, h - 1)*(unsigned)w*4u;
#pragma unroll
    for (int n = 0; n < NX; ++n) { const int k = n*NW + wv; dma(rs_x, vx[n], sx, base + (unsigned)(k < NPX ? k*256 : (XDW + GDW)*4)); }
#pragma unroll
    for (int n = 0; n < NG; ++n) { const int k = n*NW + wv; dma(rs_g, vg[n], sg, base + (unsigned)(k < NPG ? XDW*4 + k*256 : (XDW + GDW)*4)); }
  };

  f32x4v acc[9];
#pragma unroll
  for (int t = 0; t < 9; ++t) acc[t] = f32x4v{0.f, 0.f, 0.f, 0.f};
  bf16x8 A[3][P];
#pragma unroll
  for (int r = 0; r < 3; ++r)
#pragma unroll
    for (int p = 0; p < P; ++p) A[r][p] = as_frag(uint4{0u, 0u, 0u, 0u});

  auto step = [&](int i, bf16x8 (&a0)[P], const bf16x8 (&a1)[P], const bf16x8 (&a2)[P]) {
    const int after = min(D - 2, nsteps - 1 - i);
    if (after >= 2) asm volatile("s_waitcnt vmcnt(%0)" :: "n"(2*NDMA) : "memory");
    else if (after == 1) asm volatile("s_waitcnt vmcnt(%0)" :: "n"(NDMA) : "memory");
    else asm volatile("s_waitcnt vmcnt(0)" ::: "memory");
    __builtin_amdgcn_s_barrier();
    asm volatile("" ::: "memory");
    if (i + D - 1 < nsteps) issue(i + D - 1);
    const float* slot = reinterpret_cast<const float*>(lds) + (i % D)*SLOT;
    const float* xr = slot + (nc*16 + j)*CS + ks*32 + q*8;
    const float* gr = slot + XDW + j*CS + ks*32 + q*8;
    const float4 x0v = *reinterpret_cast<const float4*>(xr), x1v = *reinterpret_cast<const float4*>(xr + 4);
    const float2 x2v = *reinterpret_cast<const float2*>(xr + 8);
    const float4 g0v = *reinterpret_cast<const float4*>(gr), g1v = *reinterpret_cast<const float4*>(gr + 4);
    unsigned px[5][P], pg[4][P];
    split_pair<P>(x0v.x, x0v.y, px[0]); split_pair<P>(x0v.z, x0v.w, px[1]); split_pair<P>(x1v.x, x1v.y, px[2]); split_pair<P>(x1v.z, x1v.w, px[3]); split_pair<P>(x2v.x, x2v.y, px[4]);
    split_pair<P>(g0v.x, g0v.y, pg[0]); split_pair<P>(g0v.z, g0v.w, pg[1]); split_pair<P>(g1v.x, g1v.y, pg[2]); split_pair<P>(g1v.z, g1v.w, pg[3]);
    bf16x8 Bx[3][P];
#pragma unroll
    for (int p = 0; p < P; ++p) {
      Bx[0][p] = as_frag(uint4{px[0][p], px[1][p], px[2][p], px[3][p]});
      Bx[1][p] = as_frag(uint4{__builtin_amdgcn_alignbit(px[1][p], px[0][p], 16), __builtin_amdgcn_alignbit(px[2][p], px[1][p], 16),
                               __builtin_amdgcn_alignbit(px[3][p], px[2][p], 16), __builtin_amdgcn_alignbit(px[4][p], px[3][p], 16)});
      Bx[2][p] = as_frag(uint4{px[1][p], px[2][p], px[3][p], px[4][p]});
      a0[p] = as_frag(i < nrows ? uint4{pg[0][p], pg[1][p], pg[2][p], pg[3][p]} : uint4{0u, 0u, 0u, 0u});
    }
#pragma unroll
    for (int ky = 0; ky < 3; ++ky) {
      const bf16x8 (&a)[P] = ky == 0 ? a0 : ky == 1 ? a1 : a2;
#pragma unroll
      for (int t = 0; t < NPROD; ++t)
#pragma unroll
        for (int kx = 0; kx < 3; ++kx) acc[ky*3 + kx] = __builtin_amdgcn_mfma_f32_16x16x32_bf16(a[prod_a(P, t)], Bx[kx][prod_b(P, t)], acc[ky*3 + kx], 0, 0, 0);
    }
  };

  static_assert(D == 4, "the waits above");
#pragma unroll
  for (int r = 0; r < D - 1; ++r) issue(r);
  for (int i = 0; i < nsteps; i += 3) {
    step(i, A[0], A[2], A[1]);
    if (i + 1 < nsteps) step(i + 1, A[1], A[0], A[2]);
    if (i + 2 < nsteps) step(i + 2, A[2], A[1], A[0]);
  }
  __syncthreads();
  float* red = reinterpret_cast<float*>(lds);
  if (ks == 1) {
#pragma unroll
    for (int t = 0; t < 9; ++t)
#pragma unroll
      for (int v = 0; v < 4; ++v) red[(nc*36 + t*4 + v)*64 + lane] = acc[t][v];
  }
  __syncthreads();
  if (ks == 0) {
    const size_t blk = ((size_t)b*gridDim.y + blockIdx.y)*gridDim.x + blockIdx.x;
#pragma unroll
    for (int t = 0; t < 9; ++t)
#pragma unroll
      for (int v = 0; v < 4; ++v) {
        const int co = 4*q + v, c = nc*16 + j;
        partial[((blk*9 + t)*16 + co)*C + c] = acc[t][v] + red[(nc*36 + t*4 + v)*64 + lane];
      }
  }
}

template <bool DIRECT>
__global__ __launch_bounds__(256) void k_conv_wgrad_finalize(const float* __restrict__ partial, unsigned T, unsigned G, int CO, int C, double* __restrict__ slice, float* __restrict__ g_w) {
  __shared__ double part[4][64];
  const int lane = threadIdx.x & 63, wv = threadIdx.x >> 6;
  const int n = CO*C*9, i = blockIdx.x*64 + lane;
  const unsigned g = blockIdx.y, t0 = (unsigned)(((unsigned long long)T*g)/G), t1 = (unsigned)(((unsigned long long)T*(g + 1))/G);
  double s = 0.0;
  if (i < n) for (unsigned t = t0 + wv; t < t1; t += 4) s += (double)partial[(size_t)t*n + i];
  part[wv][lane] = s;
  __syncthreads();
  if (wv == 0 && i < n) {
    const double tot = (part[0][lane] + part[1][lane]) + (part[2][lane] + part[3][lane]);
    if (DIRECT) { const int c = i % C, co = (i/C) % CO, tap = i/(C*CO); g_w[((size_t)co*C + c)*9 + tap] = (float)tot; }
    else slice[(size_t)g*n + i] = tot;
  }
}
__global__ __launch_bounds__(256) void k_conv_wgrad_finalize2(const double* __restrict__ slice, unsigned G, int CO, int C, float* __restrict__ g_w) {
  const int n = CO*C*9, i = blockIdx.x*256 + threadIdx.x;
  if (i >= n) return;
  double tot = 0.0;
  unsigned g = 0;
  for (; g + 8 <= G; g += 8) {
    double v[8];
#pragma unroll
    for (int k = 0; k < 8; ++k) v[k] = slice[(size_t)(g + k)*n + i];
#pragma unroll
    for (int k = 0; k < 8; ++k) tot += v[k];
  }
  for (; g < G; ++g) tot += slice[(size_t)g*n + i];
  const int c = i % C, co = (i/C) % CO, tap = i/(C*CO);
  g_w[((size_t)co*C + c)*9 + tap] = (float)tot;
}
static unsigned wgrad_slices(unsigned T) { return T < 64 ? 1u : std::min(32u, T/16); }

static void wgrad_shape(int B, int C, int CO, int h, int w, dim3& grid, int& rows) {
  const int strips = ceil_div(w, 32), base = strips*B*ceil_div(C, 64)*(CO/32);
  const int groups = std::max(1, std::min(512/std::max(base, 1), ceil_div(h, 12)));
  rows = ceil_div(h, groups);
  grid = dim3(strips, ceil_div(h, rows), B*ceil_div(C, 64)*(CO/32));
}
static void wgrad16_shape(int B, int C, int h, int w, dim3& grid, int& rows) {
  const int strips = ceil_div(w, 64);
  const long long units = (long long)strips*B, slots = C == 16 ? 1024 : 768;
  const int groups = (int)std::max(1ll, std::min<long long>(ceil_div(h, 12), slots/units));
  rows = ceil_div(h, groups);
  grid = dim3(strips, ceil_div(h, rows), B);
}
size_t conv_mfma_wgrad_partials(int B, int C, int CO, int h, int w) {
  dim3 grid; int rows;
  if (CO == 16) wgrad16_shape(B, C, h, w, grid, rows); else wgrad_shape(B, C, CO, h, w, grid, rows);
  const size_t T = (size_t)grid.x*grid.y*B, n = (size_t)9*CO*C;
  return T*n + 2*(size_t)wgrad_slices((unsigned)T)*n;
}
static size_t thin_packed_elems(int C, int pieces) { return (size_t)(C >> 4)*5*pieces*512; }
size_t conv_mfma_packed_elems(int C, int CO, int pieces) { return std::max((size_t)CO*C*9*pieces, CO == 16 ? thin_packed_elems(C, pieces) : (size_t)0); }

#define SMD_BY_PIECES(pieces, CALL) do { if ((pieces) == 3) { CALL(3, float); } else if ((pieces) == 2) { CALL(2, float); } else { CALL(1, bf16); } } while (0)

template <int P, typename T>
static void launch_conv16(const void* in, const void* wp, void* out, int B, int CK, bool bwd, int hi, int wi, int ho, int wo, hipStream_t st) {
  const unsigned gx = ceil_div(wo, 64), gy = ceil_div(ho, 4), gz = B;
  const dim3 grid(8*(unsigned)ceil_div((long long)gx*gy*gz, 8ll));
  const uint4* wq = (const uint4*)wp;
  const T* i_ = (const T*)in; T* o_ = (T*)out;
  if (bwd) hipLaunchKernelGGL((k_conv16_mfma<1, P, true, T, T>), grid, dim3(256), 0, st, i_, wq, o_, hi, wi, ho, wo, gx, gy, gz);
  else if (CK == 16) hipLaunchKernelGGL((k_conv16_mfma<1, P, false, T, T>), grid, dim3(256), 0, st, i_, wq, o_, hi, wi, ho, wo, gx, gy, gz);
  else hipLaunchKernelGGL((k_conv16_mfma<2, P, false, T, T>), grid, dim3(256), 0, st, i_, wq, o_, hi, wi, ho, wo, gx, gy, gz);
}

hipError_t launch_conv_mfma_pack(const float* w, void* wp_fwd, void* wp_bwd, int C, int CO, int pieces, hipStream_t st) {
  if (CO == 16) {
    void* thin_bwd = (C == 16) ? wp_bwd : nullptr;
    if (wp_fwd || thin_bwd) {
      const dim3 g16(ceil_div((C >> 4)*5*512, 256));
#define SMD_CALL(P, T) hipLaunchKernelGGL((k_conv_pack_w16<P>), g16, dim3(256), 0, st, w, (unsigned short*)wp_fwd, (unsigned short*)thin_bwd, C)
      SMD_BY_PIECES(pieces, SMD_CALL);
#undef SMD_CALL
    }
    if (C == 16 || !wp_bwd) return hipGetLastError();
    wp_fwd = nullptr;
  }
  const dim3 grid(ceil_div(CO*C*9, 256));
#define SMD_CALL(P, T) hipLaunchKernelGGL((k_conv_pack_w<P>), grid, dim3(256), 0, st, w, (unsigned short*)wp_fwd, (unsigned short*)wp_bwd, CO, C)
  SMD_BY_PIECES(pieces, SMD_CALL);
#undef SMD_CALL
  return hipGetLastError();
}

static int g_conv_two_tiles = 0;
void set_conv_two_tiles(int v) { g_conv_two_tiles = v; }
static bool conv_two_tiles() { return g_conv_two_tiles != 0; }
struct ConvShape { int TC, TRB, NM, KS, kcs; unsigned gx, gy, gz; dim3 grid; size_t out_elems; };
static ConvShape conv_shape(int B, int CK, int M, int ho, int wo) {
  ConvShape s;
  s.TC = wo >= 48 ? 64 : 32; s.TRB = wo >= 48 ? 4 : 8;
  const long long tiles = (long long)ceil_div(wo, s.TC)*ceil_div(ho, s.TRB)*B;
  s.NM = (M % 64 == 0 && tiles*(M/64) >= 256 && conv_two_tiles()) ? 2 : 1;
  const long long base = tiles*(M/(32*s.NM));
  const int KC = CK >> 4;
  int ks = 1;
  if (base < 384) ks = (int)std::min<long long>(std::max(KC/2, 1), (512 + base - 1)/base);
  s.kcs = ceil_div(KC, ks); s.KS = ceil_div(KC, s.kcs);
  s.gx = ceil_div(wo, s.TC); s.gy = ceil_div(ho, s.TRB); s.gz = B;
  s.grid = dim3(8*(unsigned)ceil_div((long long)s.gx*s.gy*s.gz*(M/(32*s.NM))*s.KS, 8ll));
  s.out_elems = (size_t)B*M*ho*wo;
  return s;
}
size_t conv_mfma_split_elems(int B, int CK, int M, int ho, int wo) {
  const ConvShape s = conv_shape(B, CK, M, ho, wo);
  return s.KS > 1 ? (size_t)s.KS*s.out_elems : 0;
}

template <int P, int OFF, typename T>
static void launch_conv_form(const void* in, const void* wp, void* out, float* split_ws, int B, int CK, int M, int hi, int wi, int ho, int wo, hipStream_t st) {
  const ConvShape s = conv_shape(B, CK, M, ho, wo);
  const uint4* wq = (const uint4*)wp;
  const T* i_ = (const T*)in;
  T* dst = s.KS > 1 ? reinterpret_cast<T*>(split_ws) : (T*)out;
  if (s.NM == 2) {
    if (s.TC == 64) hipLaunchKernelGGL((k_conv_mfma<64, P, OFF, T, T, 2>), s.grid, dim3(512), 0, st, i_, wq, dst, CK, M, hi, wi, ho, wo, s.KS, s.kcs, s.out_elems, s.gx, s.gy, s.gz);
    else hipLaunchKernelGGL((k_conv_mfma<32, P, OFF, T, T, 2>), s.grid, dim3(512), 0, st, i_, wq, dst, CK, M, hi, wi, ho, wo, s.KS, s.kcs, s.out_elems, s.gx, s.gy, s.gz);
  } else if (s.TC == 64) hipLaunchKernelGGL((k_conv_mfma<64, P, OFF, T, T, 1>), s.grid, dim3(256), 0, st, i_, wq, dst, CK, M, hi, wi, ho, wo, s.KS, s.kcs, s.out_elems, s.gx, s.gy, s.gz);
  else hipLaunchKernelGGL((k_conv_mfma<32, P, OFF, T, T, 1>), s.grid, dim3(256), 0, st, i_, wq, dst, CK, M, hi, wi, ho, wo, s.KS, s.kcs, s.out_elems, s.gx, s.gy, s.gz);
  if (s.KS > 1) {
    const size_t n4 = s.out_elems/4;
    hipLaunchKernelGGL((k_conv_split_sum<T>), dim3((unsigned)((n4 + 255)/256)), dim3(256), 0, st, split_ws, (T*)out, n4, s.KS);
  }
}

size_t conv_mfma_fwd_split_elems(int B, int C, int CO, int h, int w) { return CO % 32 ? 0 : conv_mfma_split_elems(B, C, CO, h, w); }
size_t conv_mfma_bwd_split_elems(int B, int C, int CO, int h, int w) { return C % 32 ? 0 : conv_mfma_split_elems(B, CO, C, h + 2, w + 2); }
hipError_t launch_conv_mfma_fwd(const void* xp, const void* wp_fwd, void* y, float* split_ws, int B, int C, int CO, int h, int w, int pieces, hipStream_t st) {
  if (CO == 16) {
#define SMD_CALL(P, T) launch_conv16<P, T>(xp, wp_fwd, y, B, C, false, h + 2, w + 2, h, w, st)
    SMD_BY_PIECES(pieces, SMD_CALL);
#undef SMD_CALL
    return hipGetLastError();
  }
#define SMD_CALL(P, T) launch_conv_form<P, 0, T>(xp, wp_fwd, y, split_ws, B, C, CO, h + 2, w + 2, h, w, st)
  SMD_BY_PIECES(pieces, SMD_CALL);
#undef SMD_CALL
  return hipGetLastError();
}
hipError_t launch_conv_mfma_bwd_data(const void* gy, const void* wp_bwd, void* g_xp, float* split_ws, int B, int C, int CO, int h, int w, int pieces, hipStream_t st) {
  if (CO == 16 && C == 16) {
#define SMD_CALL(P, T) launch_conv16<P, T>(gy, wp_bwd, g_xp, B, 16, true, h, w, h + 2, w + 2, st)
    SMD_BY_PIECES(pieces, SMD_CALL);
#undef SMD_CALL
    return hipGetLastError();
  }
#define SMD_CALL(P, T) launch_conv_form<P, 2, T>(gy, wp_bwd, g_xp, split_ws, B, CO, C, h, w, h + 2, w + 2, st)
  SMD_BY_PIECES(pieces, SMD_CALL);
#undef SMD_CALL
  return hipGetLastError();
}
template <int P, typename T>
static void launch_wgrad(const void* xp_, const void* gy_, float* partial, int B, int C, int CO, int h, int w, hipStream_t st) {
  const T* xp = (const T*)xp_; const T* gy = (const T*)gy_;
  dim3 grid; int rows;
  if (CO == 16) {
    wgrad16_shape(B, C, h, w, grid, rows);
    if constexpr (std::is_same<T, float>::value) {
      if (C == 16) hipLaunchKernelGGL((k_conv16_wgrad_dma<1, P>), grid, dim3(128), 0, st, xp, gy, partial, h, w, rows);
      else hipLaunchKernelGGL((k_conv16_wgrad_dma<2, P>), grid, dim3(256), 0, st, xp, gy, partial, h, w, rows);
    } else {
      if (C == 16) hipLaunchKernelGGL((k_conv16_wgrad_mfma<1, P, T>), grid, dim3(128), 0, st, xp, gy, partial, h, w, rows);
      else hipLaunchKernelGGL((k_conv16_wgrad_mfma<2, P, T>), grid, dim3(256), 0, st, xp, gy, partial, h, w, rows);
    }
    return;
  }
  wgrad_shape(B, C, CO, h, w, grid, rows);
  if constexpr (std::is_same<T, float>::value) hipLaunchKernelGGL((k_conv_wgrad_dma<P, false>), grid, dim3(256), 0, st, xp, gy, partial, C, CO, h, w, rows);
  else hipLaunchKernelGGL((k_conv_wgrad_mfma<P, T>), grid, dim3(256), 0, st, xp, gy, partial, C, CO, h, w, rows);
}
static hipError_t wgrad_finalize(float* g_w, float* partial, int B, int C, int CO, int h, int w, hipStream_t st) {
  dim3 grid; int rows;
  if (CO == 16) wgrad16_shape(B, C, h, w, grid, rows); else wgrad_shape(B, C, CO, h, w, grid, rows);
  const unsigned T = grid.x*grid.y*(unsigned)B, G = wgrad_slices(T);
  const int n = CO*C*9;
  double* slice = reinterpret_cast<double*>(partial + (size_t)T*n);
  if (G == 1) hipLaunchKernelGGL(k_conv_wgrad_finalize<true>, dim3(ceil_div(n, 64), 1), dim3(256), 0, st, partial, T, 1u, CO, C, slice, g_w);
  else {
    hipLaunchKernelGGL(k_conv_wgrad_finalize<false>, dim3(ceil_div(n, 64), G), dim3(256), 0, st, partial, T, G, CO, C, slice, g_w);
    hipLaunchKernelGGL(k_conv_wgrad_finalize2, dim3(ceil_div(n, 256)), dim3(256), 0, st, slice, G, CO, C, g_w);
  }
  return hipGetLastError();
}
hipError_t launch_conv_mfma_bwd_wgt(const void* xp, const void* gy, float* g_w, float* partial, int B, int C, int CO, int h, int w, int pieces, hipStream_t st) {
#define SMD_CALL(P, T) launch_wgrad<P, T>(xp, gy, partial, B, C, CO, h, w, st)
  SMD_BY_PIECES(pieces, SMD_CALL);
#undef SMD_CALL
  return wgrad_finalize(g_w, partial, B, C, CO, h, w, st);
}

#define SMD_BY_PIECES_F32(pieces, CALL) do { if ((pieces) == 3) { CALL(3); } else { CALL(2); } } while (0)
size_t conv_mfma_z_split_elems(int B, int C, int CO, int h, int w) {
  size_t n = 0;
  if (C % 16 == 0 && CO % 32 == 0) n = std::max(n, conv_mfma_split_elems(B, C, CO, h, w));
  if (CO % 16 == 0 && C % 32 == 0) n = std::max(n, conv_mfma_split_elems(B, CO, C, h, w));
  return n;
}
hipError_t launch_conv_mfma_z_fwd(const float* x, const void* wp_fwd, float* y, float* split_ws, int B, int C, int CO, int h, int w, int pieces, hipStream_t st) {
#define SMD_CALL(P) launch_conv_form<P, 1, float>(x, wp_fwd, y, split_ws, B, C, CO, h, w, h, w, st)
  SMD_BY_PIECES_F32(pieces, SMD_CALL);
#undef SMD_CALL
  return hipGetLastError();
}
hipError_t launch_conv_mfma_z_bwd_data(const float* gy, const void* wp_bwd, float* g_x, float* split_ws, int B, int C, int CO, int h, int w, int pieces, hipStream_t st) {
#define SMD_CALL(P) launch_conv_form<P, 1, float>(gy, wp_bwd, g_x, split_ws, B, CO, C, h, w, h, w, st)
  SMD_BY_PIECES_F32(pieces, SMD_CALL);
#undef SMD_CALL
  return hipGetLastError();
}
hipError_t launch_conv_mfma_z_bwd_wgt(const float* x, const float* gy, float* g_w, float* partial, int B, int C, int CO, int h, int w, int pieces, hipStream_t st) {
  dim3 grid; int rows;
  wgrad_shape(B, C, CO, h, w, grid, rows);
#define SMD_CALL(P) hipLaunchKernelGGL((k_conv_wgrad_dma<P, true>), grid, dim3(256), 0, st, x, gy, partial, C, CO, h, w, rows)
  SMD_BY_PIECES_F32(pieces, SMD_CALL);
#undef SMD_CALL
  return wgrad_finalize(g_w, partial, B, C, CO, h, w, st);
}

}

#ifdef SMD_CONV_TRACE
extern "C" int smd_debug_conv_trace(unsigned long long* host_out, int blocks) {
  return (int)hipMemcpyFromSymbol(host_out, HIP_SYMBOL(smd::g_conv_trace), (size_t)blocks*40*sizeof(unsigned long long), 0, hipMemcpyDeviceToHost);
}
#endif
```

### slowtv_monodepth_amd/csrc/smd_kernels.h

```cpp
#pragma once
#include <hip/hip_runtime.h>
#include <stddef.h>
#include <stdint.h>

#include "../../include/smd_hotpath.h"

namespace smd {

constexpr int kFwdCols = 62;
constexpr int kBwdCols = 60;
#ifndef SMD_WAVES_PER_BLOCK
#define SMD_WAVES_PER_BLOCK 4
#endif
constexpr int kWavesPerBlock = SMD_WAVES_PER_BLOCK;
#ifndef SMD_SMOOTH_CHUNK
#define SMD_SMOOTH_CHUNK 1024
#endif
constexpr int kSmoothChunk = SMD_SMOOTH_CHUNK;
__host__ __device__ inline int smooth_chunk_px(int n) { return n > 32768 ? kSmoothChunk : 256; }
__host__ __device__ inline int smooth_chunks_of(int n) { return (n + smooth_chunk_px(n) - 1)/smooth_chunk_px(n); }
constexpr int kSmoothCols = 63, kSmoothRows = 8;
__host__ __device__ inline int smooth_units_of(int hs, int ws) { return ((ws + kSmoothCols - 1)/kSmoothCols)*((hs + kSmoothRows - 1)/kSmoothRows); }
constexpr int kSmoothRowsMain = 16;
__host__ __device__ inline int smooth_units_main(int hs, int ws) { return ((ws + kSmoothCols - 1)/kSmoothCols)*((hs + kSmoothRowsMain - 1)/kSmoothRowsMain); }
constexpr int kPoseSums = 12;

struct ScaleSet {
  const float* p[SMD_MAX_SCALES];
  float* g[SMD_MAX_SCALES];
  int hs[SMD_MAX_SCALES];
  int ws[SMD_MAX_SCALES];
  int key[SMD_MAX_SCALES];
  int S;
};

__host__ __device__ inline size_t packed_texel_floats(int b, int n, int h, int w) { return (size_t)n*b*(size_t)(h + 1)*(size_t)(w + 1)*3; }
__host__ __device__ inline size_t packed_ypix_floats(int b, int h, int w) { return (size_t)b*(size_t)h*(size_t)w*3; }
__host__ __device__ inline size_t packed_tpix_floats(int b, int h, int w) { return (size_t)b*(size_t)h*(size_t)w*4; }
__host__ __device__ inline size_t packed_image_floats(int b, int n, int h, int w) {
  return packed_texel_floats(b, n, h, w) + packed_ypix_floats(b, h, w) + 2*packed_tpix_floats(b, h, w);
}
__host__ __device__ inline size_t packed_rowtab_offset_floats(int b, int n, int h, int w) { return (packed_image_floats(b, n, h, w) + 3) & ~(size_t)3; }
__host__ __device__ inline size_t packed_arrive_offset_floats(int b, int n, int h, int w) { return packed_rowtab_offset_floats(b, n, h, w) + (size_t)SMD_MAX_SCALES*(size_t)(h + 4)*4; }
constexpr int kLiveSupports = 4;
__host__ __device__ inline size_t live_max_strips(int h, int w) { return (size_t)((w + kFwdCols - 1)/kFwdCols)*(size_t)((h + 3)/4); }
__host__ __device__ inline size_t packed_live_offset_floats(int b, int n, int h, int w) { return (packed_arrive_offset_floats(b, n, h, w) + (((size_t)b + 1 + 3) & ~(size_t)3) + 63) & ~(size_t)63; }
__host__ __device__ inline size_t live_header_floats(int b) { return ((size_t)b + 63) & ~(size_t)63; }
__host__ __device__ inline size_t live_table_floats(int b, int h, int w) { return live_header_floats(b) + (size_t)SMD_MAX_SCALES*b*live_max_strips(h, w)*kLiveSupports*2; }
__host__ __device__ inline size_t packed_total_floats(int b, int n, int h, int w) { return packed_live_offset_floats(b, n, h, w) + live_table_floats(b, h, w); }

struct LossCombine { float* out3; unsigned* arrive; float w_rec, w_sm; };
struct SmoothFwdJob {
  const float* edge_w;
  float* partial; int max_units; float* stats; float* loss;
  unsigned* arrive;
  double* contrib;
  LossCombine comb;
};

struct ReconPrepArgs {
  const float* tgt;
  const float* supp;
  float* packed;
  int b, n, h, w;
  int i0, ni;
  int flags;
  int rh, nsx, nsy;
  int first_pass, last_pass;
  uint4* rowtab;
  unsigned* arrive;
  int sc_S, sc_hs[SMD_MAX_SCALES], sc_ws[SMD_MAX_SCALES];
};

struct ReconMainArgs {
  const float* depth;
  float* depth_out;
  ScaleSet sc;
  float a_scale, a_off;
  const uint4* rowtab;
  const float* packed;
  const float* T;
  const float* K;
  const float* Kinv;
  const float* noise;
  float* err;
  uint8_t* sel;
  float* partial;
  unsigned* arrive;
  float* loss;
  double loss_scale;
  float* warp0;
  int b, n, S, h, w;
  int i0, ni;
  int flags;
  int rh;
  int nsx, nsy;
  int b1, rh2, nsy2;
  float wscale, hscale;
  float inv_n;
  uint32_t seed_lo, seed_hi;
  int first_pass, last_pass;
  int lookahead;
  int share;
  int main_blocks, guest_blocks;
  SmoothFwdJob sm;
  LossCombine comb;
  unsigned* live;
};

struct ReconBwdArgs {
  const float* depth; const float* packed; const float* T; const float* K; const float* Kinv;
  const uint8_t* sel;
  const float* g_loss;
  float g_scale;
  float* g_depth;
  const float* g_in;
  float k0_scale;
  float* pose_partial;
  unsigned* arrive;
  float* g_T; float* g_K; float* g_Kinv;
  int b, n, S, h, w;
  int flags;
  int rh, nsx, nsy;
  int b1, rh2, nsy2;
  int pose_stride;
  int wps;
  int scales_block;
  float wscale, hscale;
  int skip_level;
  int pair;
  const unsigned* live;
  int fwd_rh, fwd_b1, fwd_rh2;
  float* g_direct;
  int direct_scale;
};

__host__ __device__ inline int ceil_div(int a, int b) { return (a + b - 1)/b; }

constexpr int SMD_MAX_AR_SEGMENTS = 8;
struct CropResizeArgs {
  const float* src[SMD_MAX_AR_SEGMENTS]; float* dst[SMD_MAX_AR_SEGMENTS];
  int planes[SMD_MAX_AR_SEGMENTS], first_plane[SMD_MAX_AR_SEGMENTS];
  int nseg;
  int H, W;
  int y0, x0, ch, cw;
  int resample;
  int oh, ow;
  const float* K_in; float* K_out; int nK;
};
hipError_t launch_crop_resize(const CropResizeArgs& a, hipStream_t st);

__device__ __forceinline__ void decode_tile(unsigned p, int nbx, int b, int S, int& xb, int& bi, int& s) {
  const unsigned nq = (unsigned)nbx*(unsigned)b, full = nq & ~7u;
  unsigned q;
  if (p < full*(unsigned)S) { const unsigned slot = p >> 3; q = (slot/(unsigned)S)*8u + (p & 7u); s = (int)(slot % (unsigned)S); }
  else { const unsigned r = p - full*(unsigned)S; q = full + r/(unsigned)S; s = (int)(r % (unsigned)S); }
  bi = (int)(q/(unsigned)nbx); xb = (int)(q - (unsigned)bi*(unsigned)nbx);
}

__host__ __device__ inline unsigned recon_grid_blocks(int nstrips, int b, int S, int spb = kWavesPerBlock) {
  return (unsigned)ceil_div(nstrips, spb)*(unsigned)b*(unsigned)S;
}
__device__ __forceinline__ void decode_wave(unsigned p, int wid, int nstrips, int b, int S, int& strip, int& bi, int& s) {
  int xb;
  decode_tile(p, ceil_div(nstrips, kWavesPerBlock), b, S, xb, bi, s);
  strip = xb*kWavesPerBlock + wid;
}

void note_variant(int which, const char* fmt, ...);
hipError_t launch_recon_prep(const ReconPrepArgs& a, hipStream_t st);
hipError_t launch_recon_main(const ReconMainArgs& a, hipStream_t st);
hipError_t launch_recon_bwd(const ReconBwdArgs& a, hipStream_t st);
hipError_t launch_sum_partials(const float* partial, int count, double scale, float* out, hipStream_t st);
hipError_t launch_pose_finalize(const float* pose_partial, int entries, int stride, const float* T, const float* K, const float* Kinv,
                                float* g_T, float* g_K, float* g_Kinv, int b, int n, hipStream_t st);

hipError_t launch_disp_to_depth_fwd(const ScaleSet& sc, int b, int h, int w, float min_depth, float max_depth,
                                    float* depth_up, float* disp_up, hipStream_t st);
struct BwdMap;
size_t disp_to_depth_bwd_tmp_floats(const ScaleSet& sc, int b, int h, int w, BwdMap* map);
struct PoseChain {
  const float* aa; const float* t; const uint8_t* invert; float* g_aa; float* g_t;
  const float* fs; const float* cs; float* g_fs; float* g_cs;
  int h, w;
};
struct SmoothBwdJob { const float* stats; const float* edge_w; const float* g_loss; float g_scale; int blocks_per_sample; int accumulate_scale; };
struct PoseFinJob { ReconBwdArgs a; int entries1, entries2, b1; PoseChain chain; SmoothBwdJob sm; };
hipError_t launch_disp_to_depth_bwd(const ScaleSet& sc, int b, int h, int w, float min_depth, float max_depth,
                                    const float* depth_up, const float* g_depth_up, float* tmp, bool premultiplied, hipStream_t st,
                                    const PoseFinJob* job = nullptr, int skip_scale = -1, bool accumulate = false);

hipError_t launch_smooth_fwd(const ScaleSet& sc, int b, const float* img, int h, int w, int flags, float* loss, float* stats,
                             float* disp_grad, float* image_grad, float* ws_sums, float* edge_w, bool edges_ready, hipStream_t st);
hipError_t launch_blur3(const float* x, float* out, int planes, int h, int w, bool adjoint, hipStream_t st);
hipError_t launch_smooth_edges(const ScaleSet& sc, int b, const float* img, int h, int w, float* edge_w, hipStream_t st);
size_t smooth_edge_bytes(const ScaleSet& sc, int b);
hipError_t launch_smooth_bwd(const ScaleSet& sc, int b, const float* img, int h, int w, int flags, const float* stats,
                             const float* g_loss, const float* edge_w, hipStream_t st, float g_scale = 1.f, int accumulate_scale = -1);
hipError_t launch_smooth_main(const ScaleSet& sc, int b, const SmoothFwdJob& job, hipStream_t st);
void smooth_fwd_job(const ScaleSet& sc, int b, float* loss, float* stats, float* ws_sums, float* edge_w, SmoothFwdJob* job);

hipError_t launch_view_synth_fwd(const float* input, const float* depth, const float* T, const float* K, const float* Kinv,
                                 float* warp, float* depth_warp, uint8_t* mask_valid, int B, int C, int h, int w, hipStream_t st);
hipError_t launch_view_synth_bwd(const float* input, const float* depth, const float* T, const float* K, const float* Kinv,
                                 const float* g_warp, const float* g_depth_warp, float* g_input, float* g_depth,
                                 float* g_T, float* g_K, float* g_Kinv, float* ws, int B, int C, int h, int w, hipStream_t st);
hipError_t launch_photo_error_fwd(const float* pred, const float* target, float* err, int N, int C, int h, int w, int flags, float w_ssim, hipStream_t st);
hipError_t launch_photo_error_bwd(const float* pred, const float* target, const float* g_err, float* g_pred, float* ws,
                                  int N, int C, int h, int w, int flags, float w_ssim, hipStream_t st);
hipError_t launch_recon_reduce_fwd(const float* err_warp, const float* err_static, const float* mask, const float* noise, uint64_t seed,
                                   float* err, uint8_t* sel, float* loss, float* ws, int n, int B, int h, int w, int flags,
                                   hipStream_t st);
hipError_t launch_recon_reduce_bwd(const uint8_t* sel, const float* g_loss, float* g_err_warp, const float* err_warp, const float* err_static,
                                   const float* mask, float* g_mask, int n, int B, int h, int w, int flags, hipStream_t st);
hipError_t launch_debug_lane_shift(float* out_left, float* out_right, hipStream_t st);
hipError_t launch_stream_copy(const void* src, void* dst, size_t nbytes, int mode, hipStream_t st);
size_t conv_head_partials(int B, int C, int h, int w);
hipError_t launch_conv_head_fwd(const void* xp, int x_bf16, const float* wgt, const float* bias, float* y, int B, int C, int h, int w, int act, hipStream_t st);
hipError_t launch_conv_head_bwd(const void* xp, int x_bf16, const float* wgt, const float* y, const float* gy, void* g_xp, float* g_w, float* g_bias, float* partial,
                                int B, int C, int h, int w, int act, hipStream_t st);
hipError_t launch_conv_thin_fwd(const float* xp, const float* wgt, float* y, int B, int C, int h, int w, hipStream_t st);
size_t conv_thin_partials(int B, int C, int h, int w);
hipError_t launch_conv_thin_bwd_wgt(const float* xp, const float* gy, float* g_w, float* partial, int B, int C, int h, int w, hipStream_t st);
hipError_t launch_conv_thin_bwd_data(const float* gy, const float* wgt, float* g_xp, int B, int C, int h, int w, hipStream_t st);
size_t conv_mfma_packed_elems(int C, int CO, int pieces);
void set_conv_two_tiles(int v);
size_t conv_mfma_wgrad_partials(int B, int C, int CO, int h, int w);
hipError_t launch_conv_mfma_pack(const float* w, void* wp_fwd, void* wp_bwd, int C, int CO, int pieces, hipStream_t st);
size_t conv_mfma_fwd_split_elems(int B, int C, int CO, int h, int w);
size_t conv_mfma_bwd_split_elems(int B, int C, int CO, int h, int w);
hipError_t launch_conv_mfma_fwd(const void* xp, const void* wp_fwd, void* y, float* split_ws, int B, int C, int CO, int h, int w, int pieces, hipStream_t st);
hipError_t launch_conv_mfma_bwd_data(const void* gy, const void* wp_bwd, void* g_xp, float* split_ws, int B, int C, int CO, int h, int w, int pieces, hipStream_t st);
hipError_t launch_conv_mfma_bwd_wgt(const void* xp, const void* gy, float* g_w, float* partial, int B, int C, int CO, int h, int w, int pieces, hipStream_t st);
size_t conv_mfma_z_split_elems(int B, int C, int CO, int h, int w);
hipError_t launch_conv_mfma_z_fwd(const float* x, const void* wp_fwd, float* y, float* split_ws, int B, int C, int CO, int h, int w, int pieces, hipStream_t st);
hipError_t launch_conv_mfma_z_bwd_data(const float* gy, const void* wp_bwd, float* g_x, float* split_ws, int B, int C, int CO, int h, int w, int pieces, hipStream_t st);
hipError_t launch_conv_mfma_z_bwd_wgt(const float* x, const float* gy, float* g_w, float* partial, int B, int C, int CO, int h, int w, int pieces, hipStream_t st);
size_t decoder_bias_partials(int B, int C, int h, int w);
hipError_t launch_elu_pad_fwd(const void* x, const float* bias, void* out, int B, int C, int h, int w, int apply_elu, int dt, hipStream_t st);
hipError_t launch_elu_pad_bwd(const void* x, const float* bias, const void* g_out, void* g_x, float* g_bias, float* ws, int B, int C, int h, int w,
                              int apply_elu, int dt, hipStream_t st);
hipError_t launch_elu_up_cat_pad_fwd(const void* a, const float* bias, const void* skip, void* out, int B, int Ca, int Cs, int h, int w, int dt,
                                     hipStream_t st);
hipError_t launch_elu_up_cat_pad_bwd(const void* a, const float* bias, const void* g_out, void* g_a, void* g_skip, float* g_bias, float* ws,
                                     int B, int Ca, int Cs, int h, int w, int dt, hipStream_t st);
int bn_chunks(int N, int HW);
hipError_t launch_bn_fwd(const float* x, const float* residual, const float* gamma, const float* beta, float* running_mean, float* running_var,
                         float momentum, float eps, int relu, float* y, float* save_mean, float* save_invstd, float* ws, int N, int C, int HW,
                         hipStream_t st);
hipError_t launch_bn_bwd(const float* x, const float* y, const float* g_y, const float* gamma, const float* save_mean, const float* save_invstd,
                         int relu, float* g_x, float* g_res, float* g_gamma, float* g_beta, float* ws, int N, int C, int HW, hipStream_t st);
hipError_t launch_maxpool_fwd(const float* x, float* y, uint8_t* idx, size_t planes, int H, int W, hipStream_t st);
hipError_t launch_maxpool_bwd(const float* g_y, const uint8_t* idx, float* g_x, size_t planes, int H, int W, hipStream_t st);
int dwconv_tiles(int H, int W);
hipError_t launch_dwconv7(const float* x, const float* w, const float* bias, float* y, int N, int C, int H, int W, int flip, hipStream_t st);
hipError_t launch_dwconv7_wrw(const float* x, const float* gy, float* gw, float* gb, float* ws, int N, int C, int H, int W, hipStream_t st);
int ln_cf_chunks(size_t npix);
hipError_t launch_ln_cf_fwd(const float* x, const float* gamma, const float* beta, void* y, int y_bf16, float* mean, float* rstd, int N, int C, int HW,
                            float eps, hipStream_t st);
hipError_t launch_ln_cf_bwd(const float* x, const void* g_y, int g_bf16, const float* gamma, const float* mean, const float* rstd, float* g_x, float* g_gamma,
                            float* g_beta, float* ws, int N, int C, int HW, hipStream_t st);
int regr_blocks(size_t N);
hipError_t launch_regression_fwd(const float* pred, const float* target, const uint8_t* mask, size_t N, int flags, float* loss, float* err,
                                 float* stats, float* ws, hipStream_t st);
hipError_t launch_regression_bwd(const float* pred, const float* target, const uint8_t* mask, size_t N, int flags, float* stats,
                                 const float* g_loss, float* g_pred, float* g_target, float* ws, hipStream_t st);
hipError_t launch_pose_fwd(const float* aa, const float* t, const uint8_t* invert, int N, float* T, hipStream_t st);
hipError_t launch_pose_bwd(const float* aa, const float* t, const uint8_t* invert, int N, const float* g_T, float* g_aa, float* g_t, hipStream_t st);
hipError_t launch_intrinsics_fwd(const float* fs, const float* cs, const float* Kin, int b, int h, int w, float* K, float* Kinv, hipStream_t st);
hipError_t launch_intrinsics_bwd(const float* fs, const float* cs, int b, int h, int w, const float* g_K, const float* g_Kinv,
                                 float* g_fs, float* g_cs, hipStream_t st);



inline int pick_rows_per_strip(int b, int S, int h, int w, int cols, int halo) {
  const int nsx = ceil_div(w, cols);
  const long target_waves = 6144;
  const int rh_max = 16;
  (void)cols;
  int best = 8;
  for (int rh = rh_max; rh >= 8; rh -= 4) {
    long waves = (long)nsx*ceil_div(h, rh)*b*S;
    best = rh;
    if (waves >= target_waves) break;
  }
  (void)halo;
  return best;
}

}
```

### slowtv_monodepth_amd/functional.py

```python
from __future__ import annotations

import os
import threading

import torch

from . import _lib
from ._lib import FLAGS, REGR_FLAGS, SEL_MASKED, int_array, ptr_array
from ._lib import call as _raw_call

__all__ = ['conv3x3_mfma', 'conv3x3_wide', 'conv3x3_same', 'set_conv_route', 'conv_routes', 'loss_path_fused', 'crop_resize', 'disp_to_depth', 'image_recon_prep', 'PreparedFrames', 'image_recon_fused', 'image_recon_fused_disp', 'disp_smooth_fused', 'view_synth', 'photo_error', 'recon_reduce',
           'lane_shift_selftest', 'recon_flags', 'regression_loss', 'elu_pad', 'elu_up_cat_pad', 'batch_norm_act', 'max_pool3x3s2', 'dwconv7x7', 'layer_norm_cf', 'pose_matrices', 'intrinsics', 'inv_intrinsics']


_tls = threading.local()


def _on(t: torch.Tensor) -> torch.device:
    _tls.device = t.device
    return t.device


def call(name: str, *args):
    dev = getattr(_tls, 'device', None)
# ... 490 lines not shown
    return _LossPath.apply(imgs, supp_imgs, Ts, Ks, K_inv, aa, t, inv, fs, cs, seed, flags, min_depth, max_depth, keys, prepared, w_recon, w_smooth, *disps.values())


class _ViewSynth(torch.autograd.Function):

    @staticmethod
    def forward(ctx, inp, depth, T, K, K_inv):
        B, Cc, h, w = inp.shape
        inp = _check('input', inp, (B, Cc, h, w)); depth = _check('depth', depth, (B, 1, h, w))
        T = _check('T', T, (B, 4, 4)); K = _check('K', K, (B, 4, 4)); K_inv = _check('K_inv', K_inv, (B, 4, 4))
        warp = torch.empty_like(inp)
        dwarp = torch.empty((B, 1, h, w), device=inp.device, dtype=torch.float32)
        valid = torch.empty((B, 1, h, w), device=inp.device, dtype=torch.uint8)
        call('smd_view_synth_fwd', inp.data_ptr(), depth.data_ptr(), T.data_ptr(), K.data_ptr(), K_inv.data_ptr(), warp.data_ptr(),
             dwarp.data_ptr(), valid.data_ptr(), B, Cc, h, w, _stream())
        ctx.save_for_backward(inp, depth, T, K, K_inv)
        ctx.mark_non_differentiable(valid)
        return warp, dwarp, valid

    @staticmethod
    def backward(ctx, g_warp, g_dwarp, _g_valid):
        inp, depth, T, K, K_inv = ctx.saved_tensors
        B, Cc, h, w = inp.shape
        dev = _on(inp)
        g_warp = _check('grad(warp)', g_warp if g_warp is not None else torch.zeros_like(inp))
        g_dwarp = _check('grad(depth_warp)', g_dwarp) if g_dwarp is not None else None
        need_in, need_k = ctx.needs_input_grad[0], (ctx.needs_input_grad[3] or ctx.needs_input_grad[4])
        g_in = torch.empty_like(inp) if need_in else None
        g_depth = torch.empty_like(depth)
        g_T = torch.empty((B, 4, 4), device=dev, dtype=torch.float32)
        g_K = torch.empty((B, 4, 4), device=dev, dtype=torch.float32) if need_k else None
        g_Ki = torch.empty((B, 4, 4), device=dev, dtype=torch.float32) if need_k else None
        nbytes = _lib.lib.smd_view_synth_workspace_bytes(B, h, w)
        ws = torch.empty(nbytes, device=dev, dtype=torch.uint8)
        call('smd_view_synth_bwd', inp.data_ptr(), depth.data_ptr(), T.data_ptr(), K.data_ptr(), K_inv.data_ptr(), g_warp.data_ptr(),
             g_dwarp.data_ptr() if g_dwarp is not None else None, g_in.data_ptr() if need_in else None, g_depth.data_ptr(), g_T.data_ptr(),
             g_K.data_ptr() if need_k else None, g_Ki.data_ptr() if need_k else None, ws.data_ptr(), nbytes, B, Cc, h, w, _stream())
        return g_in, g_depth, g_T, (g_K if ctx.needs_input_grad[3] else None), (g_Ki if ctx.needs_input_grad[4] else None)


def view_synth(inp, depth, T, K, K_inv=None):
    if K_inv is None: K_inv = torch.linalg.inv(K)
    warp, dwarp, valid = _ViewSynth.apply(inp, depth, T, K, K_inv)
    return warp, dwarp, valid.bool()


class _PhotoError(torch.autograd.Function):
    @staticmethod
    def forward(ctx, pred, target, flags, weight_ssim):
        if pred.ndim != 4: raise ValueError(f'photometric error expects (N,C,h,w) tensors, got {tuple(pred.shape)}')
        N, c, h, w = pred.shape
        pred = _check('pred', pred, (N, c, h, w)); target = _check('target', target, (N, c, h, w))
        err = torch.empty((N, 1, h, w), device=pred.device, dtype=torch.float32)
        call('smd_photo_error_fwd', pred.data_ptr(), target.data_ptr(), err.data_ptr(), N, c, h, w, int(flags), float(weight_ssim), _stream())
        ctx.save_for_backward(pred, target); ctx.flags, ctx.weight_ssim = int(flags), float(weight_ssim)
        return err

    @staticmethod
    def backward(ctx, g_err):
        pred, target = ctx.saved_tensors
        _on(pred)
        N, c, h, w = pred.shape
        g_err = _check('grad(err)', g_err)
        g_pred = torch.empty_like(pred)
        nbytes = _lib.lib.smd_photo_error_workspace_bytes(N, c, h, w)
        ws = torch.empty(nbytes, device=pred.device, dtype=torch.uint8)
        call('smd_photo_error_bwd', pred.data_ptr(), target.data_ptr(), g_err.data_ptr(), g_pred.data_ptr(), ws.data_ptr(), nbytes, N, c, h, w,
             ctx.flags, ctx.weight_ssim, _stream())
        return g_pred, None, None, None


def photo_error(pred, target, loss_name: str = 'ssim', weight_ssim: float = 0.85):
    if loss_name not in ('ssim', 'l1', 'l2'): raise KeyError(loss_name)
    if not (0 <= weight_ssim <= 1): raise ValueError(f'Invalid SSIM weight. ({weight_ssim} vs. [0, 1])')
    return _PhotoError.apply(pred, target, {'ssim': 0, 'l1': FLAGS['loss_l1'], 'l2': FLAGS['loss_l2']}[loss_name], weight_ssim)


class _Regression(torch.autograd.Function):

    @staticmethod
    def forward(ctx, pred, target, mask, flags):
        pred = _check('pred', pred); target = _check('target', target, pred.shape)
        if mask is not None:
            if tuple(mask.shape) != tuple(pred.shape): raise ValueError(f'mask: expected shape {tuple(pred.shape)}, got {tuple(mask.shape)}')
            if mask.dtype.is_floating_point: raise TypeError('RegressionLoss: pass a bool (or uint8 0/1) mask; weighting masks are not part of the accelerated path')
            mask = (mask if mask.dtype == torch.bool else mask != 0).contiguous().view(torch.uint8)
        N, dev = pred.numel(), pred.device
        loss = torch.empty((), device=dev, dtype=torch.float32); err = torch.empty_like(pred)
        stats = torch.zeros(8, device=dev, dtype=torch.float32)
        nbytes = _lib.lib.smd_regression_workspace_bytes(N)
        ws = torch.empty(nbytes, device=dev, dtype=torch.uint8)
        call('smd_regression_fwd', pred.data_ptr(), target.data_ptr(), mask.data_ptr() if mask is not None else None, N, int(flags),
             loss.data_ptr(), err.data_ptr(), stats.data_ptr(), ws.data_ptr(), nbytes, _stream())
        ctx.save_for_backward(pred, target, mask, stats); ctx.flags = int(flags)
        ctx.mark_non_differentiable(err)
        return loss, err

    @staticmethod
    def backward(ctx, g_loss, _g_err):
        pred, target, mask, stats = ctx.saved_tensors
        _on(pred)
        N = pred.numel()
        g_pred = torch.empty_like(pred) if ctx.needs_input_grad[0] else None
        g_target = torch.empty_like(target) if ctx.needs_input_grad[1] else None
        if g_pred is None and g_target is None: return None, None, None, None
        nbytes = _lib.lib.smd_regression_workspace_bytes(N)
        ws = torch.empty(nbytes, device=pred.device, dtype=torch.uint8)
        call('smd_regression_bwd', pred.data_ptr(), target.data_ptr(), mask.data_ptr() if mask is not None else None, N, ctx.flags,
             stats.data_ptr(), g_loss.to(torch.float32).contiguous().data_ptr(), g_pred.data_ptr() if g_pred is not None else None,
             g_target.data_ptr() if g_target is not None else None, ws.data_ptr(), nbytes, _stream())
        return g_pred, g_target, None, None


def regression_loss(pred, target, mask=None, *, loss_name: str = 'berhu', invert: bool = False):
    if loss_name not in ('l1', 'log_l1', 'berhu'): raise KeyError(loss_name)
    return _Regression.apply(pred, target, mask, REGR_FLAGS[loss_name] | (REGR_FLAGS['invert'] if invert else 0))


class _ReconReduce(torch.autograd.Function):
    @staticmethod
    def forward(ctx, err_warp, err_static, mask, noise, seed, flags):
        n, B, h, w = err_warp.shape
        err_warp = _check('err_warp', err_warp, (n, B, h, w))
        if err_static is not None: err_static = _check('err_static', err_static, (n, B, h, w))
        if mask is not None: mask = _check('mask', mask, (B, n, h, w))
        if noise is not None: noise = _check('noise', noise.reshape(B, h, w), (B, h, w))
        dev = err_warp.device
        err = torch.empty((B, h, w), device=dev, dtype=torch.float32)
        sel = torch.empty((B, h, w), device=dev, dtype=torch.uint8)
        loss = torch.empty((), device=dev, dtype=torch.float32)
        nbytes = _lib.lib.smd_recon_reduce_workspace_bytes(B, h, w)
        ws = torch.empty(nbytes, device=dev, dtype=torch.uint8)
        call('smd_recon_reduce_fwd', err_warp.data_ptr(), err_static.data_ptr() if err_static is not None else None,
             mask.data_ptr() if mask is not None else None, noise.data_ptr() if noise is not None else None, int(seed) & (2**64 - 1),
             err.data_ptr(), sel.data_ptr(), loss.data_ptr(), ws.data_ptr(), nbytes, n, B, h, w, int(flags), _stream())
        if mask is not None: ctx.save_for_backward(sel, err_warp, err_static, mask)
        else: ctx.save_for_backward(sel, None, None, None)
        ctx.meta = (n, B, h, w, int(flags))
        ctx.mark_non_differentiable(err, sel)
        return loss, err, sel

    @staticmethod
    def backward(ctx, g_loss, *_):
        sel, err_warp, err_static, mask = ctx.saved_tensors
        _on(sel)
        n, B, h, w, flags = ctx.meta
        g = torch.empty((n, B, h, w), device=sel.device, dtype=torch.float32)
        g_mask = torch.empty_like(mask) if mask is not None else None
        call('smd_recon_reduce_bwd', sel.data_ptr(), g_loss.to(torch.float32).contiguous().data_ptr(), g.data_ptr(),
             err_warp.data_ptr() if err_warp is not None else None, err_static.data_ptr() if err_static is not None else None,
             mask.data_ptr() if mask is not None else None, g_mask.data_ptr() if g_mask is not None else None, n, B, h, w, flags, _stream())
        return g, None, g_mask, None, None, None


def recon_reduce(err_warp, err_static=None, *, use_min: bool = False, noise=None, seed: int = 0, mask=None, mask_name: str | None = None):
    if mask_name not in {'explainability', 'uncertainty', None}: raise ValueError(f'Invalid mask type: {mask_name}')
    if mask_name and mask is None: raise ValueError("Must provide a 'mask' when masking...")
    flags = (FLAGS['use_min'] if use_min else 0) | (FLAGS['use_automask'] if err_static is not None else 0)
    if mask_name:
        flags |= FLAGS['mask_' + mask_name]
        if mask.shape[1] == 1 and err_warp.shape[0] > 1: mask = mask.expand(-1, err_warp.shape[0], -1, -1)
    return _ReconReduce.apply(err_warp, err_static, mask if mask_name else None, noise, seed, flags)


def _glue_ws(B, C, h, w, device):
    nbytes = _lib.lib.smd_decoder_glue_workspace_bytes(B, C, h, w)
    return torch.empty(nbytes, device=device, dtype=torch.uint8), nbytes


def _check_fb(name: str, t: torch.Tensor, shape=None) -> torch.Tensor:
    if not isinstance(t, torch.Tensor): raise TypeError(f'{name} must be a Tensor, got {type(t)}')
    if not t.is_cuda: raise RuntimeError(f'{name} must live on the GPU')
    if t.dtype not in (torch.float32, torch.bfloat16): raise TypeError(f'{name} must be float32 or bfloat16, got {t.dtype}')
    if shape is not None and tuple(t.shape) != tuple(shape): raise ValueError(f'{name}: expected shape {tuple(shape)}, got {tuple(t.shape)}')
    return t.contiguous()


_BF = torch.bfloat16


class _EluPad(torch.autograd.Function):
    @staticmethod
    def forward(ctx, x, bias, apply_elu, out_dtype):
        x = _check_fb('x', x)
        if x.ndim != 4: raise ValueError(f'expected (B,C,h,w), got {tuple(x.shape)}')
        B, C, h, w = x.shape
        if bias is not None: bias = _check('bias', bias, (C,))
        out = torch.empty((B, C, h + 2, w + 2), device=x.device, dtype=out_dtype)
        dt = (1 if x.dtype == _BF else 0) | (4 if out_dtype == _BF else 0)
        call('smd_elu_pad_fwd', x.data_ptr(), bias.data_ptr() if bias is not None else None, out.data_ptr(), B, C, h, w, int(apply_elu), dt, _stream())
        ctx.save_for_backward(x, bias); ctx.apply_elu, ctx.dt, ctx.out_dtype = int(apply_elu), dt, out_dtype
        return out

    @staticmethod
    def backward(ctx, g_out):
        x, bias = ctx.saved_tensors
        _on(x)
        B, C, h, w = x.shape
        g_x = torch.empty_like(x)
        g_b = torch.empty_like(bias) if (bias is not None and ctx.needs_input_grad[1]) else None
        ws, nbytes = _glue_ws(B, C, h, w, x.device) if g_b is not None else (None, 0)
        call('smd_elu_pad_bwd', x.data_ptr(), bias.data_ptr() if bias is not None else None, g_out.to(ctx.out_dtype).contiguous().data_ptr(),
             g_x.data_ptr(), g_b.data_ptr() if g_b is not None else None, ws.data_ptr() if ws is not None else None, nbytes, B, C, h, w,
             ctx.apply_elu, ctx.dt, _stream())
        return g_x, g_b, None, None


def elu_pad(x, bias=None, apply_elu: bool = True, out_dtype=None):
    return _EluPad.apply(x, bias, apply_elu, out_dtype or x.dtype)


class _Conv3x3Head(torch.autograd.Function):
    @staticmethod
    def forward(ctx, xp, weight, bias, act):
        xp = _check_fb('xp', xp)
        if xp.ndim != 4 or xp.shape[2] < 4 or xp.shape[3] < 4: raise ValueError(f'expected a padded (B,C,h+2,w+2) with h, w >= 2, got {tuple(xp.shape)}')
        B, C, H, W = xp.shape
        weight = _check('weight', weight, (1, C, 3, 3))
        if bias is not None: bias = _check('bias', bias, (1,))
        y = torch.empty((B, 1, H - 2, W - 2), device=xp.device, dtype=torch.float32)
        act = int(act) | (2 if xp.dtype == _BF else 0)
        call('smd_conv3x3_head_fwd', xp.data_ptr(), weight.data_ptr(), bias.data_ptr() if bias is not None else None, y.data_ptr(), B, C, H - 2, W - 2, act, _stream())
        ctx.save_for_backward(xp, weight, y); ctx.act, ctx.has_bias = act, bias is not None
        return y

    @staticmethod
    def backward(ctx, g_y):
        xp, weight, y = ctx.saved_tensors
        dev = _on(xp)
        B, C, H, W = xp.shape
        need_x, need_w, need_b = ctx.needs_input_grad[0], ctx.needs_input_grad[1], ctx.has_bias and ctx.needs_input_grad[2]
        g_y = _check('grad(y)', g_y.float(), (B, 1, H - 2, W - 2))
        g_xp = torch.empty_like(xp) if need_x else None
        g_w = torch.empty_like(weight) if (need_w or need_b) else None
        g_b = torch.empty(1, device=dev, dtype=torch.float32) if need_b else None
        nbytes = _lib.lib.smd_conv3x3_head_workspace_bytes(B, C, H - 2, W - 2) if g_w is not None else 0
        ws = torch.empty(max(nbytes, 256), device=dev, dtype=torch.uint8) if g_w is not None else None
        if g_xp is not None or g_w is not None:
            call('smd_conv3x3_head_bwd', xp.data_ptr(), weight.data_ptr(), y.data_ptr(), g_y.data_ptr(), g_xp.data_ptr() if g_xp is not None else None,
                 g_w.data_ptr() if g_w is not None else None, g_b.data_ptr() if g_b is not None else None, ws.data_ptr() if ws is not None else None, nbytes,
                 B, C, H - 2, W - 2, ctx.act, _stream())
        return g_xp, (g_w if need_w else None), g_b, None


def conv3x3_head(xp, weight, bias=None, act: str | None = 'sigmoid'):
    if act not in ('sigmoid', 'none', None): raise ValueError(f"act must be 'sigmoid' or None, got {act!r}")
    return _Conv3x3Head.apply(xp, weight, bias, 1 if act == 'sigmoid' else 0)


class _Conv3x3Thin(torch.autograd.Function):
    @staticmethod
    def forward(ctx, xp, weight):
        xp = _check('xp', xp)
        if xp.ndim != 4 or xp.shape[2] < 4 or xp.shape[3] < 4: raise ValueError(f'expected a padded (B,C,h+2,w+2) with h, w >= 2, got {tuple(xp.shape)}')
        B, C, H, W = xp.shape
        weight = _check('weight', weight, (16, C, 3, 3))
        y = torch.empty((B, 16, H - 2, W - 2), device=xp.device, dtype=torch.float32)
        call('smd_conv3x3_thin_fwd', xp.data_ptr(), weight.data_ptr(), y.data_ptr(), B, C, H - 2, W - 2, _stream())
        ctx.save_for_backward(xp, weight)
        return y

    @staticmethod
    def backward(ctx, g_y):
        xp, weight = ctx.saved_tensors
        dev = _on(xp)
        B, C, H, W = xp.shape
        need_x, need_w = ctx.needs_input_grad
        g_y = _check('grad(y)', g_y, (B, 16, H - 2, W - 2))
        g_xp = g_w = None
        if need_x: g_xp = torch.empty_like(xp)
        if need_w: g_w = torch.empty_like(weight)
        if need_x or need_w:
            nbytes = _lib.lib.smd_conv3x3_thin_workspace_bytes(B, C, H - 2, W - 2) if need_w else 0
            ws = torch.empty(max(nbytes, 256), device=dev, dtype=torch.uint8) if need_w else None
            call('smd_conv3x3_thin_bwd', xp.data_ptr(), weight.data_ptr(), g_y.data_ptr(), g_xp.data_ptr() if need_x else None, g_w.data_ptr() if need_w else None,
                 ws.data_ptr() if ws is not None else None, nbytes, B, C, H - 2, W - 2, _stream())
        return g_xp, g_w


def conv3x3_thin(xp, weight):
    return _Conv3x3Thin.apply(xp, weight)


_CONV_ROUTE_MODE = 'auto'
_CONV_ROUTES: dict = {}


def set_conv_route(mode: str = 'auto'):
    global _CONV_ROUTE_MODE
    if mode not in ('auto', 'mfma', 'miopen'): raise ValueError(mode)
    _CONV_ROUTE_MODE = mode
    _CONV_ROUTES.clear()


def conv_routes() -> dict:
    return dict(_CONV_ROUTES)


def _conv_static_rule(op, B, C, CO, h, w):
    px = B*h*w
    if op.endswith('_bf16'): return CO == 16
    if op.endswith('_z'): return _conv_static_rule_z(op[:-2], B, C, CO, h, w)
    if CO == 16: return op != 'wgt'
    if op == 'fwd': return px >= 20000 and C*CO <= 128*64
    if op == 'data': return px >= 5000 and C <= 256
    return px >= 20000 and CO <= 64


def _conv_static_rule_z(op, B, C, CO, h, w):
    px = B*h*w
    if op == 'wgt': return px >= 20000 and CO <= 128
    return px >= 40000 and C <= 128 and CO <= 128


def _conv_route(op, B, C, CO, h, w, run_mfma, run_ref):
    if _CONV_ROUTE_MODE != 'auto': return _CONV_ROUTE_MODE == 'mfma'
    key = (op, B, C, CO, h, w)
    r = _CONV_ROUTES.get(key)
    if r is None:
        if torch.cuda.is_current_stream_capturing(): return _conv_static_rule(op, B, C, CO, h, w)
        for _ in range(2): run_mfma(); run_ref()
        ev = [[torch.cuda.Event(enable_timing=True) for _ in range(3)] for _ in range(5)]
        for e in ev:
            e[0].record(); run_mfma(); e[1].record(); run_ref(); e[2].record()
        torch.cuda.synchronize()
        t_m = sorted(e[0].elapsed_time(e[1]) for e in ev)[2]*1e3
        t_r = sorted(e[1].elapsed_time(e[2]) for e in ev)[2]*1e3
        r = _CONV_ROUTES[key] = (t_m < 0.97*t_r, t_m, t_r)
    return r[0]


def _mfma_pack(weight, C, CO, pieces, want_fwd, want_bwd):
    nbytes = _lib.lib.smd_conv3x3_mfma_packed_bytes(C, CO, pieces)
    wf = torch.empty(max(nbytes, 256), device=weight.device, dtype=torch.uint8) if want_fwd else None
    wb = torch.empty(max(nbytes, 256), device=weight.device, dtype=torch.uint8) if want_bwd else None
    call('smd_conv3x3_mfma_pack', weight.data_ptr(), wf.data_ptr() if wf is not None else None, wb.data_ptr() if wb is not None else None, C, CO, pieces, _stream())
    return wf, wb


def _mfma_ws_bytes(B, C, CO, h, w, zpad):
    return (_lib.lib.smd_conv3x3z_mfma_workspace_bytes if zpad else _lib.lib.smd_conv3x3_mfma_workspace_bytes)(B, C, CO, h, w)


def _mfma_ws(B, C, CO, h, w, dev, zpad=False):
    nws = _mfma_ws_bytes(B, C, CO, h, w, zpad)
    return torch.empty(max(nws, 256), device=dev, dtype=torch.uint8), nws


def _routed(op, B, C, CO, h, w, force, run_mfma, run_ref):
    if force: return True
    try:
        return _conv_route(op, B, C, CO, h, w, run_mfma, run_ref)
    except (_lib.Unsupported, ValueError):
        _CONV_ROUTES[(op, B, C, CO, h, w)] = (False, float('nan'), float('nan'))
        return False


def _ran(force, run_mfma):
    if force: run_mfma(); return True
    try:
        run_mfma(); return True
    except (_lib.Unsupported, ValueError):
        return False


class _Conv3x3Wide(torch.autograd.Function):
    @staticmethod
    def forward(ctx, xp, weight, pieces, force, zpad=False):
        xp = _check_fb('xp', xp)
        if zpad and xp.dtype != torch.float32: raise TypeError(f'the zero-padded convolution takes float32 tensors, got {xp.dtype}')
        if xp.ndim != 4 or (not zpad and (xp.shape[2] < 3 or xp.shape[3] < 3)):
            raise ValueError(f'expected {"(B,C,h,w)" if zpad else "a padded (B,C,h+2,w+2)"}, got {tuple(xp.shape)}')
        B, C, H, W = xp.shape
        if weight.ndim != 4 or tuple(weight.shape[1:]) != (C, 3, 3): raise ValueError(f'weight: expected (CO,{C},3,3), got {tuple(weight.shape)}')
        CO = weight.shape[0]
        weight = _check('weight', weight, (CO, C, 3, 3))
        h, w, dev = (H, W, xp.device) if zpad else (H - 2, W - 2, xp.device)
        bf = xp.dtype == _BF
        if bf: pieces = 1
        thin = CO == 16 and C in (16, 32) and not zpad
        fwd_ok = (C % 16 == 0 and CO % 32 == 0) or thin
        if force and not fwd_ok:
            raise _lib.Unsupported(f'the MFMA forward serves C % 16 == 0 with CO % 32 == 0{"" if zpad else ", or CO = 16 with C = 16 | 32"}, not C={C} CO={CO}')
        if not force and _mfma_ws_bytes(B, C, CO, h, w, zpad) == 0: fwd_ok = False
        bwd_form = (CO % 16 == 0 and C % 32 == 0) or (C == 16 and CO == 16 and not zpad)
        y = torch.empty((B, CO, h, w), device=dev, dtype=xp.dtype)
        packed = {}

        def run_mfma():
            packed['wf'], packed['wb'] = _mfma_pack(weight, C, CO, pieces, True, bwd_form)
            ws, nws = _mfma_ws(B, C, CO, h, w, dev, zpad)
            call('smd_conv3x3z_mfma_fwd' if zpad else 'smd_conv3x3_mfma_fwd', xp.data_ptr(), packed['wf'].data_ptr(), y.data_ptr(), ws.data_ptr(), nws,
                 B, C, CO, h, w, pieces, _stream())

        def run_ref():
            if zpad: return torch.conv2d(xp, weight, None, 1, 1)
            if bf: return torch.conv2d(xp, weight.to(_BF))
            if thin: call('smd_conv3x3_thin_fwd', xp.data_ptr(), weight.data_ptr(), y.data_ptr(), B, C, h, w, _stream()); return y
            return torch.conv2d(xp, weight)
        op = 'fwd_z' if zpad else 'fwd_bf16' if bf else 'fwd'
        use = fwd_ok and _routed(op, B, C, CO, h, w, force, run_mfma, run_ref)
        if not (use and _ran(force, run_mfma)): y = run_ref()
        ctx.save_for_backward(xp, weight, packed.get('wb'))
        ctx.pieces, ctx.force, ctx.zpad, ctx.served = pieces, force, zpad, force or _mfma_ws_bytes(B, C, CO, h, w, zpad) > 0
        return y

    @staticmethod
    def backward(ctx, g_y):
        xp, weight, wp_bwd = ctx.saved_tensors
        dev = _on(xp)
        B, C, H, W = xp.shape
        zpad = ctx.zpad
        CO, pieces, force = weight.shape[0], ctx.pieces, ctx.force
        h, w = (H, W) if zpad else (H - 2, W - 2)
        need_x, need_w = ctx.needs_input_grad[0], ctx.needs_input_grad[1]
        bf = xp.dtype == _BF
        g_y = _check_fb('grad(y)', g_y.to(xp.dtype), (B, CO, h, w))
        g_xp = g_w = None
        thin = CO == 16 and C in (16, 32) and not zpad
        w_ref = weight.to(_BF) if bf else weight
        pad = [1, 1] if zpad else [0, 0]
        cb = lambda mask: torch.ops.aten.convolution_backward(g_y, xp, w_ref, None, [1, 1], pad, [1, 1], False, [0, 0], 1, mask)
        sfx = '_z' if zpad else '_bf16' if bf else ''

        def thin_bwd(want_x, want_w):
            gx_ = torch.empty_like(xp) if want_x else None
            gw_ = torch.empty_like(weight) if want_w else None
            nb = _lib.lib.smd_conv3x3_thin_workspace_bytes(B, C, h, w) if want_w else 0
            ws_ = torch.empty(max(nb, 256), device=dev, dtype=torch.uint8) if want_w else None
            call('smd_conv3x3_thin_bwd', xp.data_ptr(), weight.data_ptr(), g_y.data_ptr(), gx_.data_ptr() if want_x else None, gw_.data_ptr() if want_w else None,
                 ws_.data_ptr() if want_w else None, nb, B, C, h, w, _stream())
            return gx_, gw_
        if need_x:
            g_xp = torch.empty_like(xp)
            packed = {'wb': wp_bwd}

            def run_data():
                if packed['wb'] is None: packed['wb'] = _mfma_pack(weight, C, CO, pieces, False, True)[1]
                ws, nws = _mfma_ws(B, C, CO, h, w, dev, zpad)
                call('smd_conv3x3z_mfma_bwd_data' if zpad else 'smd_conv3x3_mfma_bwd_data', g_y.data_ptr(), packed['wb'].data_ptr(), g_xp.data_ptr(), ws.data_ptr(), nws,
                     B, C, CO, h, w, pieces, _stream())
            ok = ctx.served and ((CO % 16 == 0 and C % 32 == 0) or (C == 16 and CO == 16 and not zpad))
            ref_data = (lambda: thin_bwd(True, False)[0]) if (thin and not bf) else (lambda: cb([True, False, False])[0])
            if not (ok and _routed('data' + sfx, B, C, CO, h, w, force, run_data, ref_data) and _ran(force, run_data)):
                g_xp = ref_data()
        if need_w:
            g_w = torch.empty_like(weight)

            def run_wgt():
                ws, nws = _mfma_ws(B, C, CO, h, w, dev, zpad)
                call('smd_conv3x3z_mfma_bwd_weight' if zpad else 'smd_conv3x3_mfma_bwd_weight', xp.data_ptr(), g_y.data_ptr(), g_w.data_ptr(), ws.data_ptr(), nws,
                     B, C, CO, h, w, pieces, _stream())
            ok = ctx.served and (CO % 32 == 0 or thin)
            ref_wgt = (lambda: thin_bwd(False, True)[1]) if (thin and not bf) else (lambda: cb([False, True, False])[1].float())
            if not (ok and _routed('wgt' + sfx, B, C, CO, h, w, force, run_wgt, ref_wgt) and _ran(force, run_wgt)): g_w = ref_wgt()
        return g_xp, g_w, None, None, None


def conv3x3_mfma(xp, weight, pieces: int = 3):
    return _Conv3x3Wide.apply(xp, weight, int(pieces), True)


def conv3x3_wide(xp, weight):
    return _Conv3x3Wide.apply(xp, weight, 3, False)


def conv3x3_same(x, weight):
    return _Conv3x3Wide.apply(x, weight, 3, False, True)


class _EluUpCatPad(torch.autograd.Function):
    @staticmethod
    def forward(ctx, a, bias, skip, out_dtype):
        a = _check_fb('a', a)
        if a.ndim != 4: raise ValueError(f'expected (B,C,h,w), got {tuple(a.shape)}')
        B, Ca, h, w = a.shape
        if bias is not None: bias = _check('bias', bias, (Ca,))
        Cs = 0
        if skip is not None:
            Cs = skip.shape[1]
            skip = _check_fb('skip', skip, (B, Cs, 2*h, 2*w))
        out = torch.empty((B, Ca + Cs, 2*h + 2, 2*w + 2), device=a.device, dtype=out_dtype)
        dt = (1 if a.dtype == _BF else 0) | (2 if (skip is not None and skip.dtype == _BF) else 0) | (4 if out_dtype == _BF else 0)
        call('smd_elu_up_cat_pad_fwd', a.data_ptr(), bias.data_ptr() if bias is not None else None, skip.data_ptr() if skip is not None else None,
             out.data_ptr(), B, Ca, Cs, h, w, dt, _stream())
        ctx.save_for_backward(a, bias)
        ctx.Cs, ctx.dt, ctx.out_dtype, ctx.skip_dtype = Cs, dt, out_dtype, (skip.dtype if skip is not None else None)
        return out

    @staticmethod
    def backward(ctx, g_out):
        a, bias = ctx.saved_tensors
        _on(a)
        B, Ca, h, w = a.shape
        Cs = ctx.Cs
        g_b = torch.empty_like(bias) if (bias is not None and ctx.needs_input_grad[1]) else None
        g_a = torch.empty_like(a) if (ctx.needs_input_grad[0] or g_b is not None) else None
        g_skip = torch.empty((B, Cs, 2*h, 2*w), device=a.device, dtype=ctx.skip_dtype) if (Cs and ctx.needs_input_grad[2]) else None
        if g_a is None and g_skip is None: return None, None, None, None
        ws, nbytes = _glue_ws(B, Ca, h, w, a.device) if g_b is not None else (None, 0)
        call('smd_elu_up_cat_pad_bwd', a.data_ptr(), bias.data_ptr() if bias is not None else None, g_out.to(ctx.out_dtype).contiguous().data_ptr(),
             g_a.data_ptr() if g_a is not None else None, g_skip.data_ptr() if g_skip is not None else None,
             g_b.data_ptr() if g_b is not None else None, ws.data_ptr() if ws is not None else None, nbytes, B, Ca, Cs, h, w, ctx.dt, _stream())
        return g_a, g_b, g_skip, None


def elu_up_cat_pad(a, skip=None, bias=None, out_dtype=None):
    return _EluUpCatPad.apply(a, bias, skip, out_dtype or a.dtype)


class _BatchNormAct(torch.autograd.Function):

    @staticmethod
    def forward(ctx, x, residual, weight, bias, running_mean, running_var, momentum, eps, relu):
        x = _check('x', x)
        if x.ndim != 4: raise ValueError(f'expected (N,C,H,W), got {tuple(x.shape)}')
        N, C, H, W = x.shape
        if N*H*W < 2: raise ValueError('Expected more than 1 value per channel when training')
        if residual is not None: residual = _check('residual', residual, x.shape)
        weight = _check('weight', weight, (C,)); bias = _check('bias', bias, (C,))
        y = torch.empty_like(x)
        save = torch.empty((2, C), device=x.device, dtype=torch.float32)
        nbytes = _lib.lib.smd_bn_workspace_bytes(N, C, H*W)
        ws = torch.empty(nbytes, device=x.device, dtype=torch.uint8)
        call('smd_bn_fwd', x.data_ptr(), residual.data_ptr() if residual is not None else None, weight.data_ptr(), bias.data_ptr(),
             running_mean.data_ptr() if running_mean is not None else None, running_var.data_ptr() if running_var is not None else None,
             float(momentum), float(eps), int(relu), y.data_ptr(), save[0].data_ptr(), save[1].data_ptr(), ws.data_ptr(), nbytes, N, C, H*W, _stream())
        ctx.save_for_backward(x, y if relu else None, weight, save)
        ctx.relu, ctx.has_res = bool(relu), residual is not None
        return y

    @staticmethod
    def backward(ctx, g_y):
        x, y, weight, save = ctx.saved_tensors
        _on(x)
        N, C, H, W = x.shape
        g_y = g_y.contiguous()
        g_x = torch.empty_like(x)
        g_res = None
        if ctx.has_res and ctx.needs_input_grad[1]: g_res = torch.empty_like(x) if ctx.relu else g_y
        g_w = torch.empty_like(weight); g_b = torch.empty_like(weight)
        nbytes = _lib.lib.smd_bn_workspace_bytes(N, C, H*W)
        ws = torch.empty(nbytes, device=x.device, dtype=torch.uint8)
        call('smd_bn_bwd', x.data_ptr(), y.data_ptr() if y is not None else None, g_y.data_ptr(), weight.data_ptr(), save[0].data_ptr(),
             save[1].data_ptr(), int(ctx.relu), g_x.data_ptr(), g_res.data_ptr() if (g_res is not None and ctx.relu) else None,
             g_w.data_ptr(), g_b.data_ptr(), ws.data_ptr(), nbytes, N, C, H*W, _stream())
        return g_x, g_res, g_w, g_b, None, None, None, None, None


def batch_norm_act(x, weight, bias, running_mean=None, running_var=None, *, residual=None, momentum: float = 0.1, eps: float = 1e-5, relu: bool = False):
    return _BatchNormAct.apply(x, residual, weight, bias, running_mean, running_var, momentum, eps, relu)


class _MaxPool3x3s2(torch.autograd.Function):
    @staticmethod
    def forward(ctx, x):
        x = _check('x', x)
        if x.ndim != 4: raise ValueError(f'expected (N,C,H,W), got {tuple(x.shape)}')
        N, C, H, W = x.shape
        Ho, Wo = (H - 1)//2 + 1, (W - 1)//2 + 1
        y = torch.empty((N, C, Ho, Wo), device=x.device, dtype=torch.float32)
        idx = torch.empty((N, C, Ho, Wo), device=x.device, dtype=torch.uint8)
        call('smd_maxpool3x3s2_fwd', x.data_ptr(), y.data_ptr(), idx.data_ptr(), N, C, H, W, _stream())
        ctx.save_for_backward(idx); ctx.shape = (N, C, H, W)
        return y

    @staticmethod
    def backward(ctx, g_y):
        (idx,) = ctx.saved_tensors
        _on(idx)
        N, C, H, W = ctx.shape
        g_x = torch.empty((N, C, H, W), device=idx.device, dtype=torch.float32)
        call('smd_maxpool3x3s2_bwd', g_y.contiguous().data_ptr(), idx.data_ptr(), g_x.data_ptr(), N, C, H, W, _stream())
        return g_x


def max_pool3x3s2(x):
    return _MaxPool3x3s2.apply(x)


class _DwConv7x7(torch.autograd.Function):

    @staticmethod
    def forward(ctx, x, weight, bias):
        x = _check('x', x)
        if x.ndim != 4: raise ValueError(f'expected (N,C,H,W), got {tuple(x.shape)}')
        N, C, H, W = x.shape
        weight = _check('weight', weight, (C, 1, 7, 7))
        if bias is not None: bias = _check('bias', bias, (C,))
        y = torch.empty_like(x)
        call('smd_dwconv7x7_fwd', x.data_ptr(), weight.data_ptr(), bias.data_ptr() if bias is not None else None, y.data_ptr(), N, C, H, W, 0, _stream())
        ctx.save_for_backward(x, weight); ctx.has_bias = bias is not None
        return y

    @staticmethod
    def backward(ctx, g_y):
        x, weight = ctx.saved_tensors
        _on(x)
        N, C, H, W = x.shape
        g_y = g_y.contiguous()
        g_x = g_w = g_b = None
        if ctx.needs_input_grad[0]:
            g_x = torch.empty_like(x)
            call('smd_dwconv7x7_fwd', g_y.data_ptr(), weight.data_ptr(), None, g_x.data_ptr(), N, C, H, W, 1, _stream())
        if ctx.needs_input_grad[1] or (ctx.has_bias and ctx.needs_input_grad[2]):
            g_w = torch.empty_like(weight)
            g_b = torch.empty((C,), device=x.device, dtype=torch.float32) if ctx.has_bias else None
            nbytes = _lib.lib.smd_dwconv7x7_workspace_bytes(C, H, W)
            ws = torch.empty(nbytes, device=x.device, dtype=torch.uint8)
            call('smd_dwconv7x7_wrw', x.data_ptr(), g_y.data_ptr(), g_w.data_ptr(), g_b.data_ptr() if g_b is not None else None, ws.data_ptr(), nbytes,
                 N, C, H, W, _stream())
        return g_x, g_w, g_b


def dwconv7x7(x, weight, bias=None):
# ... 168 lines not shown
```

Baseline: 857.5.

## Add band tiling for small conv maps and multi-sample wgrad blocks

Adds a 'band' tile mode to the MFMA conv kernel for small spatial maps. It packs full-width rows, or several whole samples, into one LDS tile so that fewer lanes sit idle than with the fixed rectangular tiles. The DMA weight-gradient kernel can now walk several batch samples per block and skips the padding rows of zero-padded inputs, which reduces the number of partial sums. Static routing rules are widened so coarse, high-channel decoder and encoder layers go to the MFMA path during graph capture. This adds indexing complexity and changes workspace sizing.

```diff
diff --git a/slowtv_monodepth_amd/csrc/smd_api.hip b/slowtv_monodepth_amd/csrc/smd_api.hip
--- a/slowtv_monodepth_amd/csrc/smd_api.hip
+++ b/slowtv_monodepth_amd/csrc/smd_api.hip
@@ -820,7 +820,7 @@
   if (!mfma_sizes_ok(B, C, CO, h, w)) return 0;
   smd::set_conv_two_tiles(knob("conv_two_tiles", 0));
   size_t n = std::max((size_t)64, smd::conv_mfma_z_split_elems(B, C, CO, h, w));
-  if (CO % 32 == 0) n = std::max(n, smd::conv_mfma_wgrad_partials(B, C, CO, h, w));
+  if (CO % 32 == 0) n = std::max(n, smd::conv_mfma_z_wgrad_partials(B, C, CO, h, w));
   return align256(n*sizeof(float));
 }
 int smd_conv3x3z_mfma_fwd(const float* x, const void* wp_fwd, float* y, void* workspace, size_t workspace_bytes,
diff --git a/slowtv_monodepth_amd/csrc/smd_conv_mfma.hip b/slowtv_monodepth_amd/csrc/smd_conv_mfma.hip
--- a/slowtv_monodepth_amd/csrc/smd_conv_mfma.hip
+++ b/slowtv_monodepth_amd/csrc/smd_conv_mfma.hip
@@ -62,29 +62,50 @@
   static constexpr int TRB = (TC == 64) ? 4 : 8;
   static constexpr int PW = TC + 2, PH = TRB + 2, NPIX = PW*PH;
 };
+template <> struct ConvTile<0> {
+  static constexpr int TRB = 0, PW = 0, NPIX = 420;
+};
 
 template <int TC, int P, int OFF, typename TI, typename TO, int NM>
 __global__ __launch_bounds__(256*NM, 2/NM) void k_conv_mfma(const TI* __restrict__ in_, const uint4* __restrict__ wp, TO* __restrict__ out,
                                                    int CK, int M, int hi, int wi, int ho, int wo, int KS, int kc_per_split, size_t split_stride,
-                                                   unsigned gx, unsigned gy, unsigned gz) {
+                                                   unsigned gx, unsigned gy, unsigned gz, int S, int B) {
   using T = ConvTile<TC>;
-  constexpr int NPIX = T::NPIX, PW = T::PW, off = OFF, NPROD = n_products(P);
+  constexpr bool BAND = TC == 0;
+  constexpr int NPIX = T::NPIX, off = OFF, NPROD = n_products(P);
+  const int PW = BAND ? wo + 2 : T::PW;
   constexpr bool ZERO = OFF != 0;
   constexpr int kBuf = P*NPIX*2;
   __shared__ uint4 tile[2*kBuf];
   const int lane = threadIdx.x & 63, wall = __builtin_amdgcn_readfirstlane(threadIdx.x >> 6), wv = wall & 3, mt = wall >> 2, j = lane & 31, g = lane >> 5;
   constexpr int NT = 256*NM;
   const int MG = M/(32*NM);
-  const unsigned nblk = (unsigned)(MG*KS)*gx*gy*gz, per = (nblk + 7)/8;
+  const unsigned nblk = (unsigned)(MG*KS)*(BAND ? 1u : gx)*gy*gz, per = (nblk + 7)/8;
   const unsigned lid = (blockIdx.x & 7)*per + (blockIdx.x >> 3);
   if (lid >= nblk) return;
   const int mg = (int)(lid % MG)*NM + mt, ks = (lid/MG) % KS;
   const unsigned tl = lid/(MG*KS);
-  const int x0 = (int)(tl % gx)*TC, y0 = (int)((tl/gx) % gy)*T::TRB, b = (int)(tl/(gx*gy));
+  const int BR = BAND ? (int)gx : 0, SEGP = (BR + 2)*PW;
+  const int x0 = BAND ? 0 : (int)(tl % gx)*TC, y0 = BAND ? (int)(tl % gy)*BR : (int)((tl/gx) % gy)*T::TRB;
+  const int b = BAND ? (int)(tl/gy)*S : (int)(tl/(gx*gy));
   const int KC = CK >> 4, kc0 = ks*kc_per_split, kc1 = min(KC, kc0 + kc_per_split);
   const size_t plane = (size_t)hi*wi;
   typedef typename RawOf<TI>::type R;
   const R* src = reinterpret_cast<const R*>(in_) + (size_t)b*CK*plane;
+  auto band_pixel = [&](int nt, int& seg, int& ry, int& x) {
+    const int p = (2*wv + nt)*32 + j, spx = BR*wo;
+    seg = p/spx; const int q = p - seg*spx; ry = q/wo; x = q - ry*wo;
+    if (seg >= S || b + seg >= B || y0 + ry >= ho) seg = -1;
+  };
+  int lbase[2] = {0, 0};
+  if constexpr (BAND) {
+#pragma unroll
+    for (int nt = 0; nt < 2; ++nt) {
+      int seg, ry, x;
+      band_pixel(nt, seg, ry, x);
+      lbase[nt] = seg >= 0 ? (seg*(BR + 2) + ry)*PW + x : 0;
+    }
+  }
 
   constexpr int ITEMS = 2*NPIX, TRIPS = (ITEMS + NT - 1)/NT;
   int pofs[TRIPS];
@@ -92,10 +113,19 @@
   for (int t = 0; t < TRIPS; ++t) {
     const int item = min(t*NT + (int)threadIdx.x, ITEMS - 1);
     const int half = item >= NPIX ? 1 : 0, pix = item - half*NPIX;
-    const int r = pix/PW, cc = pix - r*PW;
-    const int yy = y0 + r - off, xx = x0 + cc - off;
-    if (ZERO) pofs[t] = (yy >= 0 && yy < hi && xx >= 0 && xx < wi) ? yy*wi + xx : -1;
-    else pofs[t] = min(yy, hi - 1)*wi + min(xx, wi - 1);
+    if constexpr (BAND) {
+      const int seg = pix/SEGP, rp = pix - seg*SEGP, r = rp/PW, cc = rp - r*PW;
+      const int yy = y0 + r - off, xx = cc - off;
+      const bool in_b = seg < S && b + seg < B;
+      const int sofs = min(seg, B - 1 - b)*CK*(int)plane;
+      if (ZERO) pofs[t] = (in_b && yy >= 0 && yy < hi && xx >= 0 && xx < wi) ? sofs + yy*wi + xx : -1;
+      else pofs[t] = sofs + min(yy, hi - 1)*wi + min(xx, wi - 1);
+    } else {
+      const int r = pix/PW, cc = pix - r*PW;
+      const int yy = y0 + r - off, xx = x0 + cc - off;
+      if (ZERO) pofs[t] = (yy >= 0 && yy < hi && xx >= 0 && xx < wi) ? yy*wi + xx : -1;
+      else pofs[t] = min(yy, hi - 1)*wi + min(xx, wi - 1);
+    }
   }
   R v[TRIPS][8];
   auto request = [&](int kc) {
@@ -144,7 +174,7 @@
 #pragma unroll
     for (int nt = 0; nt < 2; ++nt) {
       const int r = (TC == 64) ? wv : 2*wv + nt, cb = (TC == 64) ? nt*32 : 0;
-      const int pix = (r + ky)*PW + cb + j + kx;
+      const int pix = BAND ? lbase[nt] + ky*PW + kx : (r + ky)*PW + cb + j + kx;
       const int slot = pix*2 + (g ^ ((pix >> 3) & 1));
 #pragma unroll
       for (int p = 0; p < P; ++p) dst[nt][p] = as_frag(tile[buf*kBuf + p*NPIX*2 + slot]);
@@ -197,13 +227,21 @@
   float* dstf = reinterpret_cast<float*>(out) + (size_t)ks*split_stride;
 #pragma unroll
   for (int nt = 0; nt < 2; ++nt) {
-    const int r = (TC == 64) ? wv : 2*wv + nt, cb = (TC == 64) ? nt*32 : 0;
-    const int y = y0 + r, x = x0 + cb + j;
-    if (y < ho && x < wo) {
+    int y, x, bo = b;
+    bool ok;
+    if constexpr (BAND) {
+      int seg, ry;
+      band_pixel(nt, seg, ry, x);
+      ok = seg >= 0; y = y0 + ry; bo = b + seg;
+    } else {
+      const int r = (TC == 64) ? wv : 2*wv + nt, cb = (TC == 64) ? nt*32 : 0;
+      y = y0 + r; x = x0 + cb + j; ok = y < ho && x < wo;
+    }
+    if (ok) {
 #pragma unroll
       for (int rr = 0; rr < 16; ++rr) {
         const int m = mg*32 + (rr & 3) + 8*(rr >> 2) + 4*g;
-        const size_t o = (((size_t)b*M + m)*ho + y)*wo + x;
+        const size_t o = (((size_t)bo*M + m)*ho + y)*wo + x;
         if (KS > 1) dstf[o] = acc[nt][rr] + lo[nt][rr];
         else store_out<TO>(out, o, acc[nt][rr] + lo[nt][rr]);
       }
@@ -503,7 +541,7 @@
 
 template <int P, bool ZP>
 __global__ __launch_bounds__(256, 2) void k_conv_wgrad_dma(const float* __restrict__ xp, const float* __restrict__ gy, float* __restrict__ partial,
-                                                        int C, int CO, int h, int w, int rows_per_block) {
+                                                        int B, int C, int CO, int h, int w, int rows_per_block, int spb) {
   constexpr int COB = 32, CB = 64, NW = 4, NPROD = n_products(P), CS = 36, D = 4;
   constexpr int XDW = CB*CS, GDW = COB*CS, NPX = XDW/64, NPG = GDW/64, NX = (NPX + NW - 1)/NW, NG = (NPG + NW - 1)/NW, NDMA = NX + NG, SLOT = XDW + GDW + 64;
   static_assert(XDW % 64 == 0 && GDW % 64 == 0 && (D - 2)*NDMA < 64 && D == 4, "DMA pieces and waits");
@@ -512,11 +550,13 @@
   const int lane = threadIdx.x & 63, wv = __builtin_amdgcn_readfirstlane(threadIdx.x >> 6), j = lane & 31, g = lane >> 5;
   const int ct = wv & 1, ks = wv >> 1;
   const int CGRP = (C + CB - 1)/CB, COGRP = CO/COB;
-  const int cg = blockIdx.z % CGRP, cog = (blockIdx.z/CGRP) % COGRP, b = blockIdx.z/(CGRP*COGRP);
-  const int x0 = blockIdx.x*32, ybeg = blockIdx.y*rows_per_block, nrows = min(rows_per_block, h - ybeg), nsteps = nrows + 2;
+  const int cg = blockIdx.z % CGRP, cog = (blockIdx.z/CGRP) % COGRP, sg = blockIdx.z/(CGRP*COGRP);
+  const int x0 = blockIdx.x*32, ybeg = blockIdx.y*rows_per_block, nrows = min(rows_per_block, h - ybeg);
+  const bool skip0 = ZP && ybeg == 0;
+  const int nsteps = nrows + 2 - ((ZP && ybeg + nrows == h) ? 1 : 0);
+  const int b0 = sg*spb, nsteps_all = min(spb, B - b0)*nsteps;
   const int W = w + 2, H = h + 2;
-  const rsrc_t rs_x = ZP ? make_rsrc(xp + (size_t)b*C*h*w, (size_t)C*h*w*4) : make_rsrc(xp + (size_t)b*C*H*W, (size_t)C*H*W*4);
-  const rsrc_t rs_g = make_rsrc(gy + ((size_t)b*CO + (size_t)cog*COB)*h*w, (size_t)COB*h*w*4);
+  const size_t xsample = ZP ? (size_t)C*h*w : (size_t)C*H*W;
   [[maybe_unused]] const rsrc_t rs_0 = make_rsrc(xp, 0);
   const unsigned lds0 = (unsigned)__builtin_amdgcn_readfirstlane((int)(unsigned)(unsigned long long)(__attribute__((address_space(3))) unsigned*)lds);
   auto dma = [&](const rsrc_t& rs, unsigned v, unsigned so, unsigned dst) {
@@ -536,8 +576,13 @@
     const int k = n*NW + wv, d = k*64 + lane, co = d/CS, col = d - co*CS;
     tab[(NX + n)*64] = (k < NPG && col < 32 && x0 + col < w) ? (unsigned)((co*h)*w + x0 + col)*4u : 0x80000000u;
   }
-  auto issue = [&](int r) {
-    const unsigned base = lds0 + (unsigned)((r % D)*SLOT*4);
+  int is_b = b0, is_r = 0;
+  auto issue = [&](int q) {
+    const int r = is_r, b = is_b;
+    if (++is_r == nsteps) { is_r = 0; ++is_b; }
+    const unsigned base = lds0 + (unsigned)((q % D)*SLOT*4);
+    const rsrc_t rs_x = make_rsrc(xp + (size_t)b*xsample, xsample*4);
+    const rsrc_t rs_g = make_rsrc(gy + ((size_t)b*CO + (size_t)cog*COB)*h*w, (size_t)COB*h*w*4);
     rsrc_t rx = rs_x;
     unsigned sx;
     if constexpr (ZP) {
@@ -566,14 +611,17 @@
 #pragma unroll
     for (int p = 0; p < P; ++p) A[r][p] = as_frag(uint4{0u, 0u, 0u, 0u});
 
+  int st_r = 0;
   auto step = [&](int i, bf16x8 (&a0)[P], const bf16x8 (&a1)[P], const bf16x8 (&a2)[P]) {
-    const int after = min(D - 2, nsteps - 1 - i);
+    const int il = st_r;
+    if (++st_r == nsteps) st_r = 0;
+    const int after = min(D - 2, nsteps_all - 1 - i);
     if (after >= 2) asm volatile("s_waitcnt vmcnt(%0)" :: "n"(2*NDMA) : "memory");
     else if (after == 1) asm volatile("s_waitcnt vmcnt(%0)" :: "n"(NDMA) : "memory");
     else asm volatile("s_waitcnt vmcnt(0)" ::: "memory");
     __builtin_amdgcn_s_barrier();
     asm volatile("" ::: "memory");
-    if (i + D - 1 < nsteps) issue(i + D - 1);
+    if (i + D - 1 < nsteps_all) issue(i + D - 1);
     const float* slot = reinterpret_cast<const float*>(lds) + (i % D)*SLOT;
     const float* xr = slot + (ct*32 + j)*CS + ks*16 + g*8;
     const float* gr = slot + XDW + j*CS + ks*16 + g*8;
@@ -590,8 +638,9 @@
       Bx[1][p] = as_frag(uint4{__builtin_amdgcn_alignbit(px[1][p], px[0][p], 16), __builtin_amdgcn_alignbit(px[2][p], px[1][p], 16),
                                __builtin_amdgcn_alignbit(px[3][p], px[2][p], 16), __builtin_amdgcn_alignbit(px[4][p], px[3][p], 16)});
       Bx[2][p] = as_frag(uint4{px[1][p], px[2][p], px[3][p], px[4][p]});
-      a0[p] = as_frag(i < nrows ? uint4{pg[0][p], pg[1][p], pg[2][p], pg[3][p]} : uint4{0u, 0u, 0u, 0u});
-    }
+      a0[p] = as_frag(il < nrows ? uint4{pg[0][p], pg[1][p], pg[2][p], pg[3][p]} : uint4{0u, 0u, 0u, 0u});
+    }
+    if (skip0 && il == 0) return;
 #pragma unroll
     for (int ky = 0; ky < 3; ++ky) {
       const bf16x8 (&a)[P] = ky == 0 ? a0 : ky == 1 ? a1 : a2;
@@ -602,11 +651,11 @@
     }
   };
 #pragma unroll
-  for (int r = 0; r < D - 1; ++r) issue(r);
-  for (int i = 0; i < nsteps; i += 3) {
+  for (int r = 0; r < D - 1; ++r) if (r < nsteps_all) issue(r);
+  for (int i = 0; i < nsteps_all; i += 3) {
     step(i, A[0], A[2], A[1]);
-    if (i + 1 < nsteps) step(i + 1, A[1], A[0], A[2]);
-    if (i + 2 < nsteps) step(i + 2, A[2], A[1], A[0]);
+    if (i + 1 < nsteps_all) step(i + 1, A[1], A[0], A[2]);
+    if (i + 2 < nsteps_all) step(i + 2, A[2], A[1], A[0]);
   }
   __syncthreads();
   float* red = reinterpret_cast<float*>(lds);
@@ -622,7 +671,7 @@
     for (int t = 0; t < 9; ++t)
 #pragma unroll
       for (int r = 0; r < 16; ++r) acc[t][r] += red[(ct*144 + t*16 + r)*64 + lane];
-    const size_t blk = ((size_t)b*gridDim.y + blockIdx.y)*gridDim.x + blockIdx.x;
+    const size_t blk = ((size_t)sg*gridDim.y + blockIdx.y)*gridDim.x + blockIdx.x;
     const int c = (cg*2 + ct)*32 + j;
     if (c < C) {
 #pragma unroll
@@ -908,12 +957,23 @@
 }
 static unsigned wgrad_slices(unsigned T) { return T < 64 ? 1u : std::min(32u, T/16); }
 
-static void wgrad_shape(int B, int C, int CO, int h, int w, dim3& grid, int& rows) {
-  const int strips = ceil_div(w, 32), base = strips*B*ceil_div(C, 64)*(CO/32);
+static void wgrad_shape(int B, int C, int CO, int h, int w, dim3& grid, int& rows, int& spb, bool multi) {
+  const int cgs = ceil_div(C, 64)*(CO/32), strips = ceil_div(w, 32), base = strips*B*cgs;
   const int groups = std::max(1, std::min(512/std::max(base, 1), ceil_div(h, 12)));
   rows = ceil_div(h, groups);
-  grid = dim3(strips, ceil_div(h, rows), B*ceil_div(C, 64)*(CO/32));
-}
+  spb = 1;
+  if (multi && rows == h && base > 512) {
+    const long long per = (long long)strips*cgs;
+    long long best = -1;
+    for (int s = 1; s <= B; ++s) {
+      const long long nsg = ceil_div(B, s), cost = ceil_div(nsg*per, 256ll)*(s*(h + 2) + 4);
+      if (s > 1 && nsg*per < 512) break;
+      if (best < 0 || cost < best) { best = cost; spb = s; }
+    }
+  }
+  grid = dim3(strips, ceil_div(h, rows), ceil_div(B, spb)*cgs);
+}
+static void wgrad_shape(int B, int C, int CO, int h, int w, dim3& grid, int& rows) { int spb; wgrad_shape(B, C, CO, h, w, grid, rows, spb, false); }
 static void wgrad16_shape(int B, int C, int h, int w, dim3& grid, int& rows) {
   const int strips = ceil_div(w, 64);
   const long long units = (long long)strips*B, slots = C == 16 ? 1024 : 768;
@@ -921,12 +981,18 @@
   rows = ceil_div(h, groups);
   grid = dim3(strips, ceil_div(h, rows), B);
 }
-size_t conv_mfma_wgrad_partials(int B, int C, int CO, int h, int w) {
-  dim3 grid; int rows;
-  if (CO == 16) wgrad16_shape(B, C, h, w, grid, rows); else wgrad_shape(B, C, CO, h, w, grid, rows);
-  const size_t T = (size_t)grid.x*grid.y*B, n = (size_t)9*CO*C;
-  return T*n + 2*(size_t)wgrad_slices((unsigned)T)*n;
-}
+static unsigned wgrad_sets(int B, int C, int CO, int h, int w, bool multi) {
+  dim3 grid; int rows, spb = 1;
+  if (CO == 16) wgrad16_shape(B, C, h, w, grid, rows); else wgrad_shape(B, C, CO, h, w, grid, rows, spb, multi);
+  return grid.x*grid.y*(unsigned)ceil_div(B, spb);
+}
+static size_t wgrad_floats(unsigned T, int C, int CO) {
+  const size_t n = (size_t)9*CO*C;
+  const unsigned G = wgrad_slices(T);
+  return (size_t)T*n + (G > 1 ? 2*(size_t)G*n : 0);
+}
+size_t conv_mfma_wgrad_partials(int B, int C, int CO, int h, int w) { return wgrad_floats(wgrad_sets(B, C, CO, h, w, false), C, CO); }
+size_t conv_mfma_z_wgrad_partials(int B, int C, int CO, int h, int w) { return wgrad_floats(wgrad_sets(B, C, CO, h, w, true), C, CO); }
 static size_t thin_packed_elems(int C, int pieces) { return (size_t)(C >> 4)*5*pieces*512; }
 size_t conv_mfma_packed_elems(int C, int CO, int pieces) { return std::max((size_t)CO*C*9*pieces, CO == 16 ? thin_packed_elems(C, pieces) : (size_t)0); }
 
@@ -965,14 +1031,48 @@
 static int g_conv_two_tiles = 0;
 void set_conv_two_tiles(int v) { g_conv_two_tiles = v; }
 static bool conv_two_tiles() { return g_conv_two_tiles != 0; }
-struct ConvShape { int TC, TRB, NM, KS, kcs; unsigned gx, gy, gz; dim3 grid; size_t out_elems; };
+struct ConvShape { int TC, TRB, NM, KS, kcs, S; unsigned gx, gy, gz; dim3 grid; size_t out_elems; };
+static double band_shape(int B, int CK, int ho, int wo, int& BR, int& S) {
+  constexpr int NP = ConvTile<0>::NPIX;
+  const int PW = wo + 2;
+  if (3*PW > NP || (long long)B*CK*(ho + 2)*PW >= (1ll << 31)) return 0.0;
+  if (ho*wo <= 128) {
+    BR = ho; S = std::min(256/(ho*wo), B);
+    while (S > 1 && S*(ho + 2)*PW > NP) --S;
+  } else {
+    S = 1; BR = std::min(ho, 256/wo);
+    while (BR > 0 && (BR + 2)*PW > NP) --BR;
+    if (BR == 0) return 0.0;
+  }
+  return (double)B*ho*wo/((double)ceil_div(ho, BR)*ceil_div(B, S)*256.0);
+}
 static ConvShape conv_shape(int B, int CK, int M, int ho, int wo) {
   ConvShape s;
-  s.TC = wo >= 48 ? 64 : 32; s.TRB = wo >= 48 ? 4 : 8;
+  s.TC = wo >= 48 ? 64 : 32; s.TRB = wo >= 48 ? 4 : 8; s.S = 1;
+  const int KC = CK >> 4;
+  {
+    const double rect = (double)B*ho*wo/((double)ceil_div(wo, s.TC)*s.TC*ceil_div(ho, s.TRB)*s.TRB*B);
+    int BR = 0, S = 1;
+    const double band = rect < 0.9 ? band_shape(B, CK, ho, wo, BR, S) : 0.0;
+    if (band > rect + 0.05) {
+      s.TC = 0; s.TRB = BR; s.S = S; s.NM = 1;
+      s.gx = BR; s.gy = ceil_div(ho, BR); s.gz = ceil_div(B, S);
+      s.out_elems = (size_t)B*M*ho*wo;
+      const long long base = (long long)s.gy*s.gz*(M/32);
+      double best = -1.0;
+      for (int kcs = std::min(2, KC); kcs <= KC; ++kcs) {
+        const int KS = ceil_div(KC, kcs);
+        if (ceil_div(KC, KS) != kcs) continue;
+        const double cost = (double)ceil_div(base*KS, 512ll)*(kcs + 1) + (KS > 1 ? (2.0*KS + 1.0)*s.out_elems*4.0/25e6 : 0.0);
+        if (best < 0.0 || cost < best - 1e-9) { best = cost; s.kcs = kcs; s.KS = KS; }
+      }
+      s.grid = dim3(8*(unsigned)ceil_div(base*s.KS, 8ll));
+      return s;
+    }
+  }
   const long long tiles = (long long)ceil_div(wo, s.TC)*ceil_div(ho, s.TRB)*B;
   s.NM = (M % 64 == 0 && tiles*(M/64) >= 256 && conv_two_tiles()) ? 2 : 1;
   const long long base = tiles*(M/(32*s.NM));
-  const int KC = CK >> 4;
   int ks = 1;
   if (base < 384) ks = (int)std::min<long long>(std::max(KC/2, 1), (512 + base - 1)/base);
   s.kcs = ceil_div(KC, ks); s.KS = ceil_div(KC, s.kcs);
@@ -992,11 +1092,12 @@
   const uint4* wq = (const uint4*)wp;
   const T* i_ = (const T*)in;
   T* dst = s.KS > 1 ? reinterpret_cast<T*>(split_ws) : (T*)out;
-  if (s.NM == 2) {
-    if (s.TC == 64) hipLaunchKernelGGL((k_conv_mfma<64, P, OFF, T, T, 2>), s.grid, dim3(512), 0, st, i_, wq, dst, CK, M, hi, wi, ho, wo, s.KS, s.kcs, s.out_elems, s.gx, s.gy, s.gz);
-    else hipLaunchKernelGGL((k_conv_mfma<32, P, OFF, T, T, 2>), s.grid, dim3(512), 0, st, i_, wq, dst, CK, M, hi, wi, ho, wo, s.KS, s.kcs, s.out_elems, s.gx, s.gy, s.gz);
-  } else if (s.TC == 64) hipLaunchKernelGGL((k_conv_mfma<64, P, OFF, T, T, 1>), s.grid, dim3(256), 0, st, i_, wq, dst, CK, M, hi, wi, ho, wo, s.KS, s.kcs, s.out_elems, s.gx, s.gy, s.gz);
-  else hipLaunchKernelGGL((k_conv_mfma<32, P, OFF, T, T, 1>), s.grid, dim3(256), 0, st, i_, wq, dst, CK, M, hi, wi, ho, wo, s.KS, s.kcs, s.out_elems, s.gx, s.gy, s.gz);
+  if (s.TC == 0) hipLaunchKernelGGL((k_conv_mfma<0, P, OFF, T, T, 1>), s.grid, dim3(256), 0, st, i_, wq, dst, CK, M, hi, wi, ho, wo, s.KS, s.kcs, s.out_elems, s.gx, s.gy, s.gz, s.S, B);
+  else if (s.NM == 2) {
+    if (s.TC == 64) hipLaunchKernelGGL((k_conv_mfma<64, P, OFF, T, T, 2>), s.grid, dim3(512), 0, st, i_, wq, dst, CK, M, hi, wi, ho, wo, s.KS, s.kcs, s.out_elems, s.gx, s.gy, s.gz, 1, B);
+    else hipLaunchKernelGGL((k_conv_mfma<32, P, OFF, T, T, 2>), s.grid, dim3(512), 0, st, i_, wq, dst, CK, M, hi, wi, ho, wo, s.KS, s.kcs, s.out_elems, s.gx, s.gy, s.gz, 1, B);
+  } else if (s.TC == 64) hipLaunchKernelGGL((k_conv_mfma<64, P, OFF, T, T, 1>), s.grid, dim3(256), 0, st, i_, wq, dst, CK, M, hi, wi, ho, wo, s.KS, s.kcs, s.out_elems, s.gx, s.gy, s.gz, 1, B);
+  else hipLaunchKernelGGL((k_conv_mfma<32, P, OFF, T, T, 1>), s.grid, dim3(256), 0, st, i_, wq, dst, CK, M, hi, wi, ho, wo, s.KS, s.kcs, s.out_elems, s.gx, s.gy, s.gz, 1, B);
   if (s.KS > 1) {
     const size_t n4 = s.out_elems/4;
     hipLaunchKernelGGL((k_conv_split_sum<T>), dim3((unsigned)((n4 + 255)/256)), dim3(256), 0, st, split_ws, (T*)out, n4, s.KS);
@@ -1044,14 +1145,13 @@
     }
     return;
   }
-  wgrad_shape(B, C, CO, h, w, grid, rows);
-  if constexpr (std::is_same<T, float>::value) hipLaunchKernelGGL((k_conv_wgrad_dma<P, false>), grid, dim3(256), 0, st, xp, gy, partial, C, CO, h, w, rows);
+  int spb;
+  wgrad_shape(B, C, CO, h, w, grid, rows, spb, std::is_same<T, float>::value);
+  if constexpr (std::is_same<T, float>::value) hipLaunchKernelGGL((k_conv_wgrad_dma<P, false>), grid, dim3(256), 0, st, xp, gy, partial, B, C, CO, h, w, rows, spb);
   else hipLaunchKernelGGL((k_conv_wgrad_mfma<P, T>), grid, dim3(256), 0, st, xp, gy, partial, C, CO, h, w, rows);
 }
-static hipError_t wgrad_finalize(float* g_w, float* partial, int B, int C, int CO, int h, int w, hipStream_t st) {
-  dim3 grid; int rows;
-  if (CO == 16) wgrad16_shape(B, C, h, w, grid, rows); else wgrad_shape(B, C, CO, h, w, grid, rows);
-  const unsigned T = grid.x*grid.y*(unsigned)B, G = wgrad_slices(T);
+static hipError_t wgrad_finalize(float* g_w, float* partial, int B, int C, int CO, int h, int w, bool multi, hipStream_t st) {
+  const unsigned T = wgrad_sets(B, C, CO, h, w, multi), G = wgrad_slices(T);
   const int n = CO*C*9;
   double* slice = reinterpret_cast<double*>(partial + (size_t)T*n);
   if (G == 1) hipLaunchKernelGGL(k_conv_wgrad_finalize<true>, dim3(ceil_div(n, 64), 1), dim3(256), 0, st, partial, T, 1u, CO, C, slice, g_w);
@@ -1065,7 +1165,7 @@
 #define SMD_CALL(P, T) launch_wgrad<P, T>(xp, gy, partial, B, C, CO, h, w, st)
   SMD_BY_PIECES(pieces, SMD_CALL);
 #undef SMD_CALL
-  return wgrad_finalize(g_w, partial, B, C, CO, h, w, st);
+  return wgrad_finalize(g_w, partial, B, C, CO, h, w, pieces != 1, st);
 }
 
 #define SMD_BY_PIECES_F32(pieces, CALL) do { if ((pieces) == 3) { CALL(3); } else { CALL(2); } } while (0)
@@ -1088,12 +1188,12 @@
   return hipGetLastError();
 }
 hipError_t launch_conv_mfma_z_bwd_wgt(const float* x, const float* gy, float* g_w, float* partial, int B, int C, int CO, int h, int w, int pieces, hipStream_t st) {
-  dim3 grid; int rows;
-  wgrad_shape(B, C, CO, h, w, grid, rows);
-#define SMD_CALL(P) hipLaunchKernelGGL((k_conv_wgrad_dma<P, true>), grid, dim3(256), 0, st, x, gy, partial, C, CO, h, w, rows)
+  dim3 grid; int rows, spb;
+  wgrad_shape(B, C, CO, h, w, grid, rows, spb, true);
+#define SMD_CALL(P) hipLaunchKernelGGL((k_conv_wgrad_dma<P, true>), grid, dim3(256), 0, st, x, gy, partial, B, C, CO, h, w, rows, spb)
   SMD_BY_PIECES_F32(pieces, SMD_CALL);
 #undef SMD_CALL
-  return wgrad_finalize(g_w, partial, B, C, CO, h, w, st);
+  return wgrad_finalize(g_w, partial, B, C, CO, h, w, true, st);
 }
 
 }
diff --git a/slowtv_monodepth_amd/csrc/smd_kernels.h b/slowtv_monodepth_amd/csrc/smd_kernels.h
--- a/slowtv_monodepth_amd/csrc/smd_kernels.h
+++ b/slowtv_monodepth_amd/csrc/smd_kernels.h
@@ -226,6 +226,7 @@
 size_t conv_mfma_packed_elems(int C, int CO, int pieces);
 void set_conv_two_tiles(int v);
 size_t conv_mfma_wgrad_partials(int B, int C, int CO, int h, int w);
+size_t conv_mfma_z_wgrad_partials(int B, int C, int CO, int h, int w);
 hipError_t launch_conv_mfma_pack(const float* w, void* wp_fwd, void* wp_bwd, int C, int CO, int pieces, hipStream_t st);
 size_t conv_mfma_fwd_split_elems(int B, int C, int CO, int h, int w);
 size_t conv_mfma_bwd_split_elems(int B, int C, int CO, int h, int w);
diff --git a/slowtv_monodepth_amd/functional.py b/slowtv_monodepth_amd/functional.py
--- a/slowtv_monodepth_amd/functional.py
+++ b/slowtv_monodepth_amd/functional.py
@@ -816,15 +816,16 @@
     if op.endswith('_bf16'): return CO == 16
     if op.endswith('_z'): return _conv_static_rule_z(op[:-2], B, C, CO, h, w)
     if CO == 16: return op != 'wgt'
-    if op == 'fwd': return px >= 20000 and C*CO <= 128*64
-    if op == 'data': return px >= 5000 and C <= 256
-    return px >= 20000 and CO <= 64
+    coarse = w <= 80 and C >= 256
+    if op == 'fwd': return (px >= 20000 and C*CO <= 128*64) or (coarse and px >= 1000)
+    if op == 'data': return (px >= 5000 and C <= 256) or (coarse and px >= 1000)
+    return (px >= 20000 and CO <= 64) or (coarse and px >= 2400)
 
 
 def _conv_static_rule_z(op, B, C, CO, h, w):
     px = B*h*w
-    if op == 'wgt': return px >= 20000 and CO <= 128
-    return px >= 40000 and C <= 128 and CO <= 128
+    if op == 'data': return px >= 1000
+    return px >= (2400 if max(C, CO) >= 512 else 1000)
 
 
 def _conv_route(op, B, C, CO, h, w, run_mfma, run_ref):
```

Measured after the change: 923.3, median of 6. 7.7% higher.
